# jjery2243542/adaptive_voice_conversion

Measured on AMD Instinct MI355X. Metric: mel-segments/sec (80x128) train step, higher is better.
Workload: dtype f32; 1 GPU; BASELINE configs[1]: recon+KL train step (fwd, loss, bwd, clip, Adam-amsgrad), 80-mel x 128-frame segments, batch 256/GPU, fp32; global_batch=256, parallelism=dp1, world_size=1

## Files before the change

### adaptive_voice_conversion_amd/_lib.py

```python
import ctypes
import os

_HERE = os.path.dirname(os.path.abspath(__file__))
LIB_PATH = os.path.join(_HERE, "csrc", "libavc_hip.so")
_lib = None

MAX_BLOCKS = 8
PLAN_INFERENCE, PLAN_SPEAKER_ONLY = 1, 2
GRADS_ALL, GRADS_DECODER, GRADS_ENCODERS, GRADS_SPEAKER, GRADS_CONTENT = 0, 1, 2, 3, 4


class EncoderCfg(ctypes.Structure):
    _fields_ = [(n, ctypes.c_int) for n in ("c_in", "c_h", "c_out", "kernel_size", "bank_size", "bank_scale", "c_bank",
                                            "n_conv_blocks", "n_dense_blocks")] + [("subsample", ctypes.c_int * MAX_BLOCKS), ("act", ctypes.c_int)]


class DecoderCfg(ctypes.Structure):
    _fields_ = [(n, ctypes.c_int) for n in ("c_in", "c_cond", "c_h", "c_out", "kernel_size", "n_conv_blocks")] + \
               [("upsample", ctypes.c_int * MAX_BLOCKS), ("act", ctypes.c_int)]


class ModelCfg(ctypes.Structure):
    _fields_ = [("spk", EncoderCfg), ("enc", EncoderCfg), ("dec", DecoderCfg)]

# ... 46 lines not shown
    lib.avc_tuning_init.argtypes = [ctypes.POINTER(Tuning)]
    lib.avc_tuning_init.restype = None
    lib.avc_get_op_tuning.argtypes = [ctypes.POINTER(Tuning)]
    lib.avc_get_op_tuning.restype = None
    lib.avc_plan_create_tuned.argtypes = [ctypes.POINTER(ModelCfg), c_int, c_int, c_int, c_int, ctypes.POINTER(Tuning), ctypes.POINTER(c_void_p)]
    lib.avc_plan_set_single_stream.argtypes = [c_void_p, c_int]
    lib.avc_plan_create_ragged.argtypes = [ctypes.POINTER(ModelCfg), c_int, ctypes.POINTER(c_int), ctypes.POINTER(c_int), ctypes.POINTER(Tuning),
                                           ctypes.POINTER(c_void_p)]
    lib.avc_plan_ragged_out.argtypes = [c_void_p, ctypes.POINTER(c_int), ctypes.POINTER(c_long)]
    lib.avc_forward_ragged.argtypes = [c_void_p, c_void_p, c_void_p, c_void_p, c_void_p, c_void_p]
    if hasattr(lib, "avc_plan_create_ragged_ex"):
        lib.avc_plan_create_ragged_ex.argtypes = [ctypes.POINTER(ModelCfg), c_int, ctypes.POINTER(c_int), ctypes.POINTER(c_int), c_int,
                                                  ctypes.POINTER(Tuning), ctypes.POINTER(c_void_p)]
        lib.avc_forward_ragged_emb.argtypes = [c_void_p, c_void_p, c_void_p, c_void_p, c_long, c_long, c_void_p, c_void_p]
    if hasattr(lib, "avc_plan_create_ragged_fanout"):
        lib.avc_plan_create_ragged_fanout.argtypes = [ctypes.POINTER(ModelCfg), c_int, ctypes.POINTER(c_int), c_int, ctypes.POINTER(c_int), c_int,
                                                      ctypes.POINTER(Tuning), ctypes.POINTER(c_void_p)]
        lib.avc_plan_ragged_latents.argtypes = [c_void_p, ctypes.POINTER(c_int), ctypes.POINTER(c_long)]
        lib.avc_decoder_forward_ragged.argtypes = [c_void_p, c_void_p, c_void_p, c_int, c_void_p, c_long, c_long, c_void_p, c_void_p]
    if hasattr(lib, "avc_backward_ragged"):
        lib.avc_backward_ragged.argtypes = [c_void_p, c_void_p, c_void_p, c_void_p, c_long, c_long, c_void_p, c_void_p]
    if hasattr(lib, "avc_plan_create_ragged_content_grads"):
        lib.avc_plan_create_ragged_content_grads.argtypes = [ctypes.POINTER(ModelCfg), c_int, ctypes.POINTER(c_int), ctypes.POINTER(Tuning),
                                                             ctypes.POINTER(c_void_p)]
        lib.avc_content_backward_ragged.argtypes = [c_void_p, c_void_p, c_void_p, c_void_p, c_void_p, c_void_p]
    lib.avc_gather_segments.argtypes = [c_void_p, c_long, c_int, c_void_p, c_int, c_int, c_void_p, c_void_p]
    lib.avc_plan_destroy.argtypes = [c_void_p]
    lib.avc_plan_destroy.restype = None
    lib.avc_plan_num_params.argtypes = [c_void_p]
    lib.avc_plan_param_floats.argtypes = [c_void_p]
    lib.avc_plan_param_floats.restype = c_long
    lib.avc_plan_param_info.argtypes = [c_void_p, c_int, ctypes.POINTER(c_long), ctypes.POINTER(c_long), ctypes.POINTER(c_int * 3)]
    lib.avc_plan_workspace_floats.argtypes = [c_void_p]
    lib.avc_plan_workspace_floats.restype = c_long
    lib.avc_plan_buffer.argtypes = [c_void_p, ctypes.c_char_p]
    lib.avc_plan_buffer.restype = c_long
    lib.avc_plan_num_relu_sites.argtypes = [c_void_p]
    lib.avc_plan_relu_site.argtypes = [c_void_p, c_int, ctypes.POINTER(ReluSite)]
    lib.avc_plan_set_compute_dtype.argtypes = [c_void_p, c_int]
    lib.avc_plan_compute_dtype.argtypes = [c_void_p]
    lib.avc_plan_out_len.argtypes = [c_void_p]
    lib.avc_plan_latent_len.argtypes = [c_void_p]
    lib.avc_forward.argtypes = [c_void_p, c_void_p, c_void_p, c_long, c_long, c_int, c_void_p, c_long, c_long, c_int,
                                c_void_p, c_void_p, c_void_p]
    lib.avc_forward_ex.argtypes = [c_void_p, c_void_p, c_void_p, c_long, c_long, c_int, c_void_p, c_long, c_long, c_int,
                                   c_void_p, c_void_p, c_int, c_void_p]
    lib.avc_plan_pack_weights.argtypes = [c_void_p, c_void_p, c_void_p, c_void_p]
    if hasattr(lib, "avc_decoder_forward"):
        lib.avc_decoder_forward.argtypes = [c_void_p, c_void_p, c_void_p, c_long, c_long, c_int, c_void_p, c_long, c_long, c_void_p, c_int, c_void_p]
        lib.avc_decoder_backward.argtypes = [c_void_p, c_void_p, c_void_p, c_long, c_long, c_int, c_void_p, c_long, c_long, c_void_p, c_void_p,
                                             c_void_p, c_void_p]
    lib.avc_loss.argtypes = [c_void_p, c_void_p, c_long, c_long, c_int, c_float, c_void_p, c_void_p]
    lib.avc_backward.argtypes = [c_void_p, c_void_p, c_void_p, c_long, c_long, c_int, c_void_p, c_long, c_long, c_int,
                                 c_void_p, c_void_p, c_void_p, c_void_p, c_float, c_void_p, c_void_p, c_void_p]
    lib.avc_clip_adam_ws_floats.argtypes = [c_long]
    lib.avc_clip_adam_ws_floats.restype = c_long
    lib.avc_clip_adam_step.argtypes = [c_void_p] * 5 + [c_long, c_int] + [c_float] * 5 + [c_int, c_float, c_float, c_int,
                                                                                        c_void_p, c_void_p, c_void_p]
    lib.avc_packed_weight_floats.argtypes = [c_int] * 4
    lib.avc_packed_weight_floats.restype = c_long
    lib.avc_packed_weight_floats_x3.argtypes = [c_int] * 4
    lib.avc_packed_weight_floats_x3.restype = c_long
    lib.avc_pack_weight_x3.argtypes = [c_void_p, c_int, c_int, c_int, c_int, c_void_p, c_void_p]
    lib.avc_pack_weight.argtypes = [c_void_p, c_int, c_int, c_int, c_int, c_int, c_int, c_void_p, c_void_p]
    lib.avc_conv1d_fwd.argtypes = [c_void_p, c_long, c_long, c_int, c_int, c_int, c_int, c_void_p, c_void_p, c_int, c_int,
                                   c_int, c_int, c_void_p, c_long, c_long, c_int, c_int, c_void_p, c_int, c_long, c_long,
                                   c_int, c_int, c_void_p, c_int, c_void_p]
    lib.avc_conv1d_dgrad.argtypes = [c_void_p, c_long, c_long, c_int, c_int, c_int, c_int, c_int, c_void_p, c_int, c_int,
                                     c_int, c_int, c_void_p, c_long, c_long, c_int, c_void_p, c_int, c_long, c_long, c_int,
                                     c_int, c_void_p, c_void_p, c_int, c_void_p]
    lib.avc_conv1d_wgrad_ws_floats.argtypes = [c_int] * 5
    lib.avc_conv1d_wgrad_ws_floats.restype = c_long
    lib.avc_conv1d_wgrad.argtypes = [c_void_p, c_long, c_long, c_int, c_void_p, c_long, c_long, c_int, c_int, c_int, c_int,
                                     c_int, c_int, c_int, c_int, c_int, c_void_p, c_void_p, c_void_p, c_void_p]
    lib.avc_instnorm_fwd.argtypes = [c_void_p, c_int, c_int, c_int, c_void_p, c_long, c_int, c_int, c_void_p, c_int, c_int,
                                     c_void_p, c_void_p, c_void_p, c_void_p]
    lib.avc_instnorm_bwd.argtypes = [c_void_p, c_void_p, c_void_p, c_void_p, c_int, c_int, c_int, c_void_p, c_long, c_int,
                                     c_int, c_void_p, c_void_p, c_long, c_int, c_void_p]
    lib.avc_conv1d_in_fwd.argtypes = [c_void_p, c_long, c_long, c_int, c_int, c_int, c_int, c_void_p, c_void_p, c_int, c_int, c_int, c_int,
                                      c_void_p, c_void_p, c_long, c_int, c_int, c_void_p, c_int, c_int, c_void_p, c_void_p, c_void_p, c_void_p, c_void_p]
    lib.avc_conv1d_dgrad_in_bwd.argtypes = [c_void_p, c_long, c_long, c_int, c_int, c_int, c_int, c_int, c_void_p, c_int, c_int, c_int, c_int,
                                            c_void_p, c_void_p, c_int, c_int, c_void_p, c_void_p, c_void_p, c_void_p, c_long, c_int, c_int,
                                            c_void_p, c_void_p, c_long, c_int, c_void_p, c_void_p]
    lib.avc_instnorm_fwd_pairs.argtypes = [c_void_p, c_int, c_int, c_int, c_void_p, c_long, c_int, c_int, c_void_p, c_int, c_int, c_int,
                                           c_void_p, c_void_p, c_void_p, c_void_p]
    lib.avc_instnorm_bwd_pairs.argtypes = [c_void_p, c_void_p, c_void_p, c_void_p, c_int, c_int, c_int, c_void_p, c_long, c_int, c_int, c_int,
                                           c_void_p, c_void_p, c_long, c_int, c_void_p]
    lib.avc_to_pairs.argtypes = [c_void_p, c_long, c_long, c_long, c_int, c_int, c_int, c_void_p, c_void_p]
    lib.avc_dsp_num_frames.argtypes = [c_long, c_int]
    lib.avc_dsp_basis_floats.argtypes = [c_int, c_int, c_int]
    lib.avc_dsp_basis_floats.restype = c_long
    lib.avc_dsp_basis_scratch_floats.argtypes = [c_int, c_int]
    lib.avc_dsp_basis_scratch_floats.restype = c_long
    lib.avc_dsp_make_basis.argtypes = [c_int, c_int, c_int, c_int, c_void_p, c_void_p, c_void_p]
    lib.avc_dsp_stft.argtypes = [c_void_p, c_long, c_int, c_int, c_int, c_void_p, c_void_p, c_void_p, c_void_p]
    lib.avc_dsp_istft.argtypes = [c_void_p, c_int, c_int, c_int, c_int, c_void_p, c_void_p, c_void_p, c_void_p]
    lib.avc_dsp_griffin_lim_ws_floats.argtypes = [c_int, c_int, c_int, c_int]
    lib.avc_dsp_griffin_lim_ws_floats.restype = c_long
    lib.avc_dsp_griffin_lim.argtypes = [c_void_p, c_int, c_int, c_int, c_int, c_int, c_void_p, c_void_p, c_void_p, c_void_p, c_void_p]
    lib.avc_dsp_stft_batch.argtypes = [c_void_p, c_long, c_int, c_int, c_int, c_int, c_void_p, c_void_p, c_void_p, c_void_p]
    lib.avc_dsp_istft_batch.argtypes = [c_void_p, c_int, c_int, c_int, c_int, c_int, c_void_p, c_void_p, c_void_p, c_void_p]
    lib.avc_dsp_griffin_lim_batch.argtypes = [c_void_p, c_int, c_int, c_int, c_int, c_int, c_int, c_void_p, c_void_p, c_void_p, c_void_p, c_void_p]
    lib.avc_dsp_griffin_lim_ragged.argtypes = [c_void_p, c_void_p, c_void_p, c_int, c_int, c_int, c_int, c_int, c_int, c_void_p, c_void_p, c_void_p, c_void_p, c_void_p]
    lib.avc_dsp_magnitude.argtypes = [c_void_p, c_int, c_int, c_void_p, c_void_p]
    lib.avc_dsp_db_normalize.argtypes = [c_void_p, c_int, c_int, c_float, c_float, c_void_p, c_void_p]
    lib.avc_dsp_denormalize_amp.argtypes = [c_void_p, c_int, c_int, c_float, c_float, c_void_p, c_void_p]
    lib.avc_dsp_preemphasis.argtypes = [c_void_p, c_long, c_float, c_void_p, c_void_p]
    lib.avc_dsp_deemphasis.argtypes = [c_void_p, c_long, c_float, c_void_p, c_void_p]
    lib.avc_dsp_frame_power.argtypes = [c_void_p, c_long, c_int, c_int, c_void_p, c_void_p]
    lib.avc_prof_end.argtypes = [c_void_p, c_void_p, c_void_p, c_void_p]
    lib.avc_prof_class_name.argtypes = [c_int]
    lib.avc_prof_class_name.restype = ctypes.c_char_p
    return lib


def load():
    global _lib, LIB_PATH
    if _lib is None:
        LIB_PATH = os.environ.get("AVC_HIP_LIB", LIB_PATH)
        if not os.path.exists(LIB_PATH):
            raise RuntimeError(
                f"{LIB_PATH} is missing: build the HIP extension first "
                "(python -c 'import __graft_entry__ as g; g.build()' or adaptive_voice_conversion_amd/csrc/build.sh)")
        import torch
        try:
            _lib = declare(ctypes.CDLL(LIB_PATH))
        except OSError as e:
            raise RuntimeError(f"cannot load {LIB_PATH}: {e}") from e
    return _lib
```

### adaptive_voice_conversion_amd/csrc/conv_gemm.hip

```cpp
#include <hip/hip_runtime.h>
#include <stdlib.h>

#include "avc_common.h"
#include "avc_internal.h"

#include "conv_shared.h"
#include "conv_x3_shared.h"

#ifndef AVC_CONV_STAGES
#define AVC_CONV_STAGES 2
#endif
#ifndef AVC_CONV_STAGES_BH
#define AVC_CONV_STAGES_BH 2
#endif

static __device__ __forceinline__ void conv_wait_dma(int n) {
#define AVC_WAIT_VM(k) __builtin_amdgcn_s_waitcnt(((k) & 15) | (((k) >> 4) << 14) | (7 << 4) | (15 << 8))
    switch (n) {
        case 0: AVC_WAIT_VM(0); break;
        case 1: AVC_WAIT_VM(1); break;
        case 2: AVC_WAIT_VM(2); break;
        case 3: AVC_WAIT_VM(3); break;
        case 4: AVC_WAIT_VM(4); break;
        case 5: AVC_WAIT_VM(5); break;
// ... 323 lines not shown
        load_a(kg + KG, 1);
        load_x(xtile, kg + KG, 1);
    }
    __syncthreads();

    const int a_lane4 = (wave_m * (32 * WM) + li) * 4;
    const int nit = (nchunk + KG - 1) / KG;
    int st = 0;
    for (int wk = 0; wk < walk_n; ++wk) {
    f32x16 acc[WM][WN];
#pragma unroll
    for (int wm = 0; wm < WM; ++wm)
#pragma unroll
        for (int wn = 0; wn < WN; ++wn)
#pragma unroll
            for (int r = 0; r < 16; ++r) acc[wm][wn][r] = 0.f;
    const bool walk_more = WALK && wk + 1 < walk_n;
    for (int it = 0; it < nit; ++it) {
        const int chunk = it * KG + kg;
        const bool more = (chunk + DIST * KG < nchunk) && !((a.dbg & 1) && (DIST == 2 || it >= 1));
        const bool last_of_tile = walk_more && it == nit - 1;
        int issued = 0;
        if (more) {
            const int stn = (st + DIST) % NS;
            load_a(chunk + DIST * KG, stn);
            load_x(xtile, chunk + DIST * KG, stn);
            if (DIST == 2) issued = dma_count(chunk + DIST * KG);
        } else if (last_of_tile && !(a.dbg & 1)) {
            const int stn = (st + 1) % NS;
            load_a(0, stn);
            load_x(xtile + walk_dx, 0, stn);
        }
        const float* Ab = As + st * AS;
        const float* Xb = Xs + st * XS;
        if ((a.dbg & 2) || chunk >= nchunk) {
        } else if constexpr (PAR) {
            if (wave_n == 0) {
                if (MIRROR && use_mirror && one_window) conv_chunk_mma<WM, WN, 1, KSC, GRC, BF, 1>(acc, Ab, Xb, KS, CK, ROW, h, a_lane4, cb4, cbl4, cbr4);
                else if (MIRROR && use_mirror) conv_chunk_mma<WM, WN, 2, KSC, GRC, BF, 1>(acc, Ab, Xb, KS, CK, ROW, h, a_lane4, cb4, cbl4, cbr4);
                else conv_chunk_mma<WM, WN, 0, KSC, GRC, BF, 1>(acc, Ab, Xb, KS, CK, ROW, h, a_lane4, cb4, cbl4, cbr4);
            } else {
                if (MIRROR && use_mirror && one_window) conv_chunk_mma<WM, WN, 1, KSC, GRC, BF, 2>(acc, Ab, Xb, KS, CK, ROW, h, a_lane4, cb4, cbl4, cbr4);
                else if (MIRROR && use_mirror) conv_chunk_mma<WM, WN, 2, KSC, GRC, BF, 2>(acc, Ab, Xb, KS, CK, ROW, h, a_lane4, cb4, cbl4, cbr4);
                else conv_chunk_mma<WM, WN, 0, KSC, GRC, BF, 2>(acc, Ab, Xb, KS, CK, ROW, h, a_lane4, cb4, cbl4, cbr4);
            }
        } else if (MIRROR && use_mirror && one_window)
            conv_chunk_mma<WM, WN, 1, KSC, GRC, BF>(acc, Ab, Xb, KS, CK, ROW, h, a_lane4, cb4, cbl4, cbr4);
        else if (MIRROR && use_mirror)
            conv_chunk_mma<WM, WN, 2, KSC, GRC, BF>(acc, Ab, Xb, KS, CK, ROW, h, a_lane4, cb4, cbl4, cbr4);
        else if constexpr (KSC < 0) {
            switch (KS * 8 + GR) {
                case 1 * 8 + 4: conv_chunk_mma<WM, WN, 0, 1, 4, BF>(acc, Ab, Xb, KS, CK, ROW, h, a_lane4, cb4, cbl4, cbr4); break;
                case 2 * 8 + 2: conv_chunk_mma<WM, WN, 0, 2, 2, BF>(acc, Ab, Xb, KS, CK, ROW, h, a_lane4, cb4, cbl4, cbr4); break;
                case 3 * 8 + 2: conv_chunk_mma<WM, WN, 0, 3, 2, BF>(acc, Ab, Xb, KS, CK, ROW, h, a_lane4, cb4, cbl4, cbr4); break;
                case 4 * 8 + 1: conv_chunk_mma<WM, WN, 0, 4, 1, BF>(acc, Ab, Xb, KS, CK, ROW, h, a_lane4, cb4, cbl4, cbr4); break;
                case 5 * 8 + 1: conv_chunk_mma<WM, WN, 0, 5, 1, BF>(acc, Ab, Xb, KS, CK, ROW, h, a_lane4, cb4, cbl4, cbr4); break;
                case 6 * 8 + 1: conv_chunk_mma<WM, WN, 0, 6, 1, BF>(acc, Ab, Xb, KS, CK, ROW, h, a_lane4, cb4, cbl4, cbr4); break;
                case 7 * 8 + 1: conv_chunk_mma<WM, WN, 0, 7, 1, BF>(acc, Ab, Xb, KS, CK, ROW, h, a_lane4, cb4, cbl4, cbr4); break;
                case 8 * 8 + 1: conv_chunk_mma<WM, WN, 0, 8, 1, BF>(acc, Ab, Xb, KS, CK, ROW, h, a_lane4, cb4, cbl4, cbr4); break;
                default: conv_chunk_mma<WM, WN, 0, 0, 0, BF>(acc, Ab, Xb, KS, CK, ROW, h, a_lane4, cb4, cbl4, cbr4);
            }
        } else
            conv_chunk_mma<WM, WN, 0, KSC, GRC, BF>(acc, Ab, Xb, KS, CK, ROW, h, a_lane4, cb4, cbl4, cbr4);
        if (last_of_tile) {
            conv_wait_dma(0);
        } else if (!(a.dbg & 4)) {
            conv_wait_dma(issued);
            conv_bare_barrier();
        }
        st = st == NS - 1 ? 0 : st + 1;
    }

    if (KG > 1) {
        float* red = smem + ((kg > 0 ? kg - 1 : 0) * 4 + wave) * (WM * WN * 16 * 64) + lane;
        if (kg > 0) {
#pragma unroll
            for (int wm = 0; wm < WM; ++wm)
#pragma unroll
                for (int wn = 0; wn < WN; ++wn)
#pragma unroll
                    for (int r = 0; r < 16; ++r) red[((wm * WN + wn) * 16 + r) * 64] = acc[wm][wn][r];
        }
        __syncthreads();
        if (kg > 0) return;
#pragma unroll
        for (int k2 = 1; k2 < KG; ++k2) {
            const float* rk = smem + ((k2 - 1) * 4 + wave) * (WM * WN * 16 * 64) + lane;
#pragma unroll
            for (int wm = 0; wm < WM; ++wm)
#pragma unroll
                for (int wn = 0; wn < WN; ++wn)
#pragma unroll
                    for (int r = 0; r < 16; ++r) acc[wm][wn][r] += rk[((wm * WN + wn) * 16 + r) * 64];
        }
    }

    if constexpr (INF) {
        static_assert(WM == 1 && WN == 1 && (BF == 0 || BF == 2) && !PAR && !RAG && !WALK && !MIRROR, "fused InstanceNorm epilogue: forward, 64 x 64 tiles, fp32 or bf16 pairs");
        if (KG > 1) __syncthreads();
        if constexpr (BF == 2) conv_epilogue_in_pairs(a, g, acc[0][0], smem, tid, wave_m, wave_n, li, h, m_tile0, q.b0);
        else conv_epilogue_in(a, g, acc[0][0], smem, tid, wave_m, wave_n, li, h, m_tile0, q.b0);
        return;
    }
    if constexpr (INB) {
        static_assert(WM == 1 && WN == 1 && (BF == 0 || BF == 2) && !RAG && !WALK && !INF, "fused InstanceNorm-backward epilogue: input gradient on 64 x 64 tiles, fp32 or bf16 pairs");
        if (KG > 1) __syncthreads();
        if constexpr (BF == 2) conv_epilogue_in_bwd_pairs(a, g, acc[0][0], smem, tid, wave_m, h, m_tile0, q.b0, q.t0, colb[0] - q.b0, colt[0], colv[0]);
        else conv_epilogue_in_bwd(a, g, acc[0][0], smem, tid, wave_m, h, m_tile0, q.b0, q.t0, colb[0] - q.b0, colt[0], colv[0]);
        return;
    }
    if (!(a.dbg & 8)) {
        if constexpr (WALK) {
            ConvEpi epi_t;
            ConvGroup g_t;
#ifdef AVC_EMU
            const ConvArgs* ka = &a;
#else
            const __attribute__((address_space(4))) ConvArgs* ka = (const __attribute__((address_space(4))) ConvArgs*)__builtin_amdgcn_kernarg_segment_ptr();
            asm volatile("" : "+s"(ka));
#endif
            epi_t.ob = ka->ob; epi_t.oc = ka->oc; epi_t.rb = ka->rb; epi_t.rc = ka->rc; epi_t.obase = 0; epi_t.rbase = 0;
            epi_t.ot = ka->ot; epi_t.ops = ka->ops; epi_t.rt = ka->rt; epi_t.Tres = ka->Tres; epi_t.Tout = ka->Tout; epi_t.M = ka->M;
            epi_t.act = ka->act; epi_t.res_mode = ka->res_mode; epi_t.res_to_primary = ka->res_to_primary; epi_t.slope = ka->slope;
            epi_t.pairs = ka->pairs;
            const int z = blockIdx.z;
            g_t.wp = nullptr; g_t.bias = ka->g[z].bias; g_t.out = ka->g[z].out; g_t.out2 = ka->g[z].out2; g_t.res = ka->g[z].res;
            g_t.mask = ka->g[z].mask; g_t.KS = 0; g_t.padL = 0; g_t.padR = 0; g_t.nchunk = 0; g_t.CK = 0; g_t.out_c0 = 0;
#pragma unroll
            for (int wn = 0; wn < WN; ++wn) {
                if (!colv[wn]) continue;
#pragma unroll
                for (int wm = 0; wm < WM; ++wm) {
                    int tcol = colt[wn], bcol = b0_cur + colb[wn], mb = m_tile0 + wave_m * (32 * WM) + wm * 32;
#ifndef AVC_EMU
                    asm volatile("" : "+v"(tcol), "+v"(bcol));
                    asm volatile("" : "+s"(mb));
#endif
                    if (BF == 2 && epi_t.pairs) conv_store_frag_pairs(epi_t, g_t, acc[wm][wn], mb, h, bcol, tcol);
                    else conv_store_frag(epi_t, g_t, acc[wm][wn], mb, h, bcol, tcol);
                }
            }
        } else {
#pragma unroll
            for (int wn = 0; wn < WN; ++wn) {
                if (!colv[wn]) continue;
#pragma unroll
                for (int wm = 0; wm < WM; ++wm) {
                    if (BF == 2 && epi.pairs) conv_store_frag_pairs(epi, g, acc[wm][wn], m_tile0 + wave_m * (32 * WM) + wm * 32, h, colb[wn], colt[wn]);
                    else conv_store_frag(epi, g, acc[wm][wn], m_tile0 + wave_m * (32 * WM) + wm * 32, h, colb[wn], colt[wn]);
                }
            }
        }
    }
    if (walk_more) {
        conv_bare_barrier();
        xtile += walk_dx;
        b0_cur += a.walk_db;
    }
    }
}


struct PackBatch {
    PackArgs a[AVC_PACK_BATCH];
};

static __device__ __forceinline__ void pack_one(const PackArgs& p, long first, long stride, long limit = (1L << 62));

__global__ void __launch_bounds__(AVC_THREADS) pack_weight_batch_kernel(const PackBatch b) {
    pack_one(b.a[blockIdx.y], (long)blockIdx.x * AVC_THREADS + threadIdx.x, (long)gridDim.x * AVC_THREADS);
}

static __device__ __forceinline__ void pack_staged(const PackArgs* __restrict__ gp, const float* __restrict__ params, float* __restrict__ ws, int piece, float* stage) {
    const int tid = threadIdx.x;
    const int MB = gp->mb, Mp = gp->Mp, M = gp->M, KS = gp->KS, CK = gp->CK, Cin = gp->Cin, Cout = gp->Cout, img = gp->img;
    const int nsrc = gp->nsrc, rows_per_src = gp->rows_per_src;
    const bool dgrad = gp->dgrad != 0;
    float* dst = (float*)((char*)ws + (size_t)gp->dst);
    const char* pbase = (const char*)params;
    const int nmb = (Mp + MB - 1) / MB;
    const int chunk = piece / nmb, m0 = (piece - chunk * nmb) * MB;
    const bool pairs = img == AVC_IMG_K4H;
    const int CKr = pairs ? 2 * CK : CK, c0 = chunk * CKr;
    const int seglen = dgrad ? MB * KS : CKr * KS, nseg = dgrad ? CKr : MB;
    const int pitch = seglen | 1;
    const int n = nseg * seglen;
    const float inv_seglen = 1.0f / (float)seglen, inv_rows = 1.0f / (float)rows_per_src;
    const int row0 = dgrad ? c0 : m0, col0 = dgrad ? m0 : c0;
    const int row_end = dgrad ? Cout : M, off_end = ((dgrad ? M : Cin) - col0) * KS;
    constexpr int U = 16;
    for (int e0 = tid; e0 < n; e0 += U * AVC_THREADS) {
// ... 210 lines not shown
    return ck;
}

static size_t conv_lds_bytes(const ConvArgs& a, int BM, int BN) {
    size_t worst = 0;
    for (int gi = 0; gi < a.ngroups; ++gi) {
        ConvGeom q = conv_geom(a.mode, a.stride, a.Tout, a.g[gi].KS, BN, 0);
        size_t AS = (size_t)a.g[gi].KS * a.g[gi].CK * BM, XS = (size_t)a.g[gi].CK * q.ROW;
        size_t bytes = (size_t)(a.bf16 == AVC_COMPUTE_BF16S ? AVC_CONV_STAGES_BH : AVC_CONV_STAGES) * (AS + XS) * 4;
        worst = bytes > worst ? bytes : worst;
    }
    return worst + 16;
}

static int conv_ntiles_n(const ConvArgs& a, int BN) {
    if (a.Tout >= BN) return a.B * avc_cdiv(a.Tout, BN);
    int worst = 1;
    for (int gi = 0; gi < a.ngroups; ++gi) {
        const int n = avc_cdiv(a.B, conv_geom(a.mode, a.stride, a.Tout, a.g[gi].KS, BN, 0).SPT);
        worst = n > worst ? n : worst;
    }
    return worst;
}

template <int WM, int BF>
static void conv_launch_rag(const ConvArgs& a, int fast, dim3 grid, dim3 block, size_t lds, hipStream_t stream) {
    if (fast == 1) hipLaunchKernelGGL((conv_gemm_kernel<WM, 1, false, 5, 1, 1, BF, false, true>), grid, block, lds, stream, a);
    else if (fast == -1) hipLaunchKernelGGL((conv_gemm_kernel<WM, 1, false, -1, 0, 1, BF, false, true>), grid, block, lds, stream, a);
    else if (fast == 14) hipLaunchKernelGGL((conv_gemm_kernel<WM, 1, false, 1, 4, 1, BF, false, true>), grid, block, lds, stream, a);
    else hipLaunchKernelGGL((conv_gemm_kernel<WM, 1, false, 0, 0, 1, BF, false, true>), grid, block, lds, stream, a);
}

static void conv_launch_rag_dgrad(const ConvArgs& a, int fast, dim3 grid, dim3 block, size_t lds, hipStream_t stream) {
    if (a.par && fast == 1) hipLaunchKernelGGL((conv_gemm_kernel<1, 1, true, 5, 1, 1, 0, true, true>), grid, block, lds, stream, a);
    else if (fast == 1) hipLaunchKernelGGL((conv_gemm_kernel<1, 1, true, 5, 1, 1, 0, false, true>), grid, block, lds, stream, a);
    else hipLaunchKernelGGL((conv_gemm_kernel<1, 1, true, 0, 0, 1, 0, false, true>), grid, block, lds, stream, a);
}

template <int WM, int KG, int BF>
static void conv_launch_variant(const ConvArgs& a, bool mir, int fast, dim3 grid, dim3 block, size_t lds, hipStream_t stream) {
    if (mir && fast == 1) hipLaunchKernelGGL((conv_gemm_kernel<WM, 1, true, 5, 1, KG, BF>), grid, block, lds, stream, a);
    else if (mir && fast == 2) hipLaunchKernelGGL((conv_gemm_kernel<WM, 1, true, 5, 2, KG, BF>), grid, block, lds, stream, a);
    else if (mir) hipLaunchKernelGGL((conv_gemm_kernel<WM, 1, true, 0, 0, KG, BF>), grid, block, lds, stream, a);
    else if (fast == 1) hipLaunchKernelGGL((conv_gemm_kernel<WM, 1, false, 5, 1, KG, BF>), grid, block, lds, stream, a);
    else if (fast == 2) hipLaunchKernelGGL((conv_gemm_kernel<WM, 1, false, 5, 2, KG, BF>), grid, block, lds, stream, a);
    else if (fast == 4 && KG == 1) hipLaunchKernelGGL((conv_gemm_kernel<WM, 1, false, 5, 4, 1, BF>), grid, block, lds, stream, a);
    else if (fast == -1 && KG == 1) hipLaunchKernelGGL((conv_gemm_kernel<WM, 1, false, -1, 0, 1, BF>), grid, block, lds, stream, a);
    else if (fast == 14) hipLaunchKernelGGL((conv_gemm_kernel<WM, 1, false, 1, 4, KG, BF>), grid, block, lds, stream, a);
    else hipLaunchKernelGGL((conv_gemm_kernel<WM, 1, false, 0, 0, KG, BF>), grid, block, lds, stream, a);
}

static bool conv_launch_walk(const ConvArgs& a, int tile, bool mir, int fast, dim3 grid, dim3 block, size_t lds, hipStream_t stream) {
    if (tile == 11 && fast == 1 && mir) hipLaunchKernelGGL((conv_gemm_kernel<1, 1, true, 5, 1, 1, 0, false, false, true>), grid, block, lds, stream, a);
    else if (tile == 11 && fast == 1) hipLaunchKernelGGL((conv_gemm_kernel<1, 1, false, 5, 1, 1, 0, false, false, true>), grid, block, lds, stream, a);
    else if (tile == 11 && fast == -1 && !mir) hipLaunchKernelGGL((conv_gemm_kernel<1, 1, false, -1, 0, 1, 0, false, false, true>), grid, block, lds, stream, a);
    else if (tile == 11 && fast == 14 && !mir) hipLaunchKernelGGL((conv_gemm_kernel<1, 1, false, 1, 4, 1, 0, false, false, true>), grid, block, lds, stream, a);
    else if (tile == 21 && fast == 14 && !mir) hipLaunchKernelGGL((conv_gemm_kernel<2, 1, false, 1, 4, 1, 0, false, false, true>), grid, block, lds, stream, a);
    else return false;
    return true;
}
template <int KG, int BF>
static void conv_launch_inf(const ConvArgs& a, int fast, dim3 grid, dim3 block, size_t lds, hipStream_t stream) {
    if (fast == 1) hipLaunchKernelGGL((conv_gemm_kernel<1, 1, false, 5, 1, KG, BF, false, false, false, true>), grid, block, lds, stream, a);
    else if (fast == 2) hipLaunchKernelGGL((conv_gemm_kernel<1, 1, false, 5, 2, KG, BF, false, false, false, true>), grid, block, lds, stream, a);
    else if (fast == 14) hipLaunchKernelGGL((conv_gemm_kernel<1, 1, false, 1, 4, KG, BF, false, false, false, true>), grid, block, lds, stream, a);
    else hipLaunchKernelGGL((conv_gemm_kernel<1, 1, false, 0, 0, KG, BF, false, false, false, true>), grid, block, lds, stream, a);
}
template <int KG, int BF>
static void conv_launch_inb(const ConvArgs& a, bool mir, int fast, dim3 grid, dim3 block, size_t lds, hipStream_t stream) {
    if (a.par && mir && fast == 1) hipLaunchKernelGGL((conv_gemm_kernel<1, 1, true, 5, 1, KG, BF, true, false, false, false, true>), grid, block, lds, stream, a);
    else if (a.par && mir) hipLaunchKernelGGL((conv_gemm_kernel<1, 1, true, 5, 2, KG, BF, true, false, false, false, true>), grid, block, lds, stream, a);
    else if (a.par && fast == 1) hipLaunchKernelGGL((conv_gemm_kernel<1, 1, false, 5, 1, KG, BF, true, false, false, false, true>), grid, block, lds, stream, a);
    else if (a.par) hipLaunchKernelGGL((conv_gemm_kernel<1, 1, false, 5, 2, KG, BF, true, false, false, false, true>), grid, block, lds, stream, a);
    else if (mir && fast == 1) hipLaunchKernelGGL((conv_gemm_kernel<1, 1, true, 5, 1, KG, BF, false, false, false, false, true>), grid, block, lds, stream, a);
    else if (mir && fast == 2) hipLaunchKernelGGL((conv_gemm_kernel<1, 1, true, 5, 2, KG, BF, false, false, false, false, true>), grid, block, lds, stream, a);
    else if (mir) hipLaunchKernelGGL((conv_gemm_kernel<1, 1, true, 0, 0, KG, BF, false, false, false, false, true>), grid, block, lds, stream, a);
    else if (fast == 14) hipLaunchKernelGGL((conv_gemm_kernel<1, 1, false, 1, 4, KG, BF, false, false, false, false, true>), grid, block, lds, stream, a);
    else hipLaunchKernelGGL((conv_gemm_kernel<1, 1, false, 0, 0, KG, BF, false, false, false, false, true>), grid, block, lds, stream, a);
}
static bool conv_walk_instance(int tile, bool mir, int fast) {
    return (tile == 11 && (fast == 1 || ((fast == -1 || fast == 14) && !mir))) || (tile == 21 && fast == 14 && !mir);
}

template <int BF>
static void conv_launch_wide(const ConvArgs& a, bool mir, dim3 grid, dim3 block, size_t lds, hipStream_t stream) {
    if (mir) hipLaunchKernelGGL((conv_gemm_kernel<1, 2, true, 5, 1, 1, BF>), grid, block, lds, stream, a);
    else hipLaunchKernelGGL((conv_gemm_kernel<1, 2, false, 5, 1, 1, BF>), grid, block, lds, stream, a);
}

template <int KG, int BF>
static void conv_launch_par(const ConvArgs& a, bool mir, int fast, dim3 grid, dim3 block, size_t lds, hipStream_t stream) {
    if (mir && fast == 1) hipLaunchKernelGGL((conv_gemm_kernel<1, 1, true, 5, 1, KG, BF, true>), grid, block, lds, stream, a);
    else if (mir) hipLaunchKernelGGL((conv_gemm_kernel<1, 1, true, 5, 2, KG, BF, true>), grid, block, lds, stream, a);
    else if (fast == 1) hipLaunchKernelGGL((conv_gemm_kernel<1, 1, false, 5, 1, KG, BF, true>), grid, block, lds, stream, a);
    else hipLaunchKernelGGL((conv_gemm_kernel<1, 1, false, 5, 2, KG, BF, true>), grid, block, lds, stream, a);
}

bool avc_conv_in_fusable(const ConvArgs& a, const avc_tuning& tun, int res_mode, int Tres) {
    const int Tn_ = a.Tout * a.ops;
    if (res_mode != AVC_RES_NONE && !((res_mode == AVC_RES_IDENTITY && Tres == Tn_) || (res_mode == AVC_RES_UP2 && 2 * Tres == Tn_) ||
                                      (res_mode == AVC_RES_AVGPOOL2 && Tres == 2 * Tn_))) return false;
    if (!tun.conv_in_fuse || a.mode != 0 || a.ngroups != 1 || a.rag.tile) return false;
    const bool bh = a.bf16 == AVC_COMPUTE_BF16S;
    if (bh ? (a.img != AVC_IMG_K4H || !a.pairs || a.ops != 1 || (a.M & 1) || a.x.ps != 1 || a.x.st != 1) : (a.bf16 != AVC_COMPUTE_F32 || a.img != AVC_IMG_K4 || a.pairs)) return false;
    if (a.Tout != 16 && a.Tout != 32 && a.Tout != 64) return false;
    if (a.ops != 1 && a.ops != 2) return false;
    if (a.ops == 2 && (a.M & 1)) return false;
    if (a.act || a.res_mode != AVC_RES_NONE || a.g[0].out2 || a.g[0].mask) return false;
    const int C = (bh ? a.M / 2 : a.M) / a.ops, Tn = a.Tout * a.ops;
    if (a.ot != 1 || a.oc != Tn || a.ob != (long)C * Tn) return false;
    if (conv_geom(0, a.stride, a.Tout, a.g[0].KS, 64, 0).SPT != 64 / a.Tout) return false;
    return avc_conv_pick_tile(tun, a.Mp, a.B, a.Tout, 1, a.Cred * a.g[0].KS * (bh ? 2 : 1)) == 11;
}

bool avc_conv_inb_fusable(const ConvArgs& a, const avc_tuning& tun) {
    if (!tun.conv_in_fuse || a.mode != 1 || a.ngroups != 1 || a.rag.tile) return false;
    const bool bh = a.bf16 == AVC_COMPUTE_BF16S;
    if (bh ? (a.img != AVC_IMG_K4H || !a.pairs || (a.M & 1) || a.x.ps != 1 || a.x.st != 1) : (a.bf16 != AVC_COMPUTE_F32 || a.img != AVC_IMG_K4 || a.pairs)) return false;
    if (a.Tout != 16 && a.Tout != 32 && a.Tout != 64) return false;
    if (a.ops != 1 || a.act || a.g[0].out2 || a.g[0].mask || a.g[0].bias) return false;
    const long Mr = bh ? a.M / 2 : a.M;
    if (a.ot != 1 || a.oc != a.Tout || a.ob != Mr * a.Tout) return false;
    if (a.res_mode != AVC_RES_NONE) {
        if (!a.res_to_primary || a.rt != 1 || a.rc != a.Tres || a.rb != Mr * a.Tres) return false;
        if (!((a.res_mode == AVC_RES_IDENTITY && a.Tres == a.Tout) || (a.res_mode == AVC_RES_POOLT && 2 * a.Tres == a.Tout) ||
              (a.res_mode == AVC_RES_UPT && a.Tres == 2 * a.Tout))) return false;
    }
    if (conv_geom(1, a.stride, a.Tout, a.g[0].KS, 64, 0).SPT != 64 / a.Tout) return false;
    return avc_conv_pick_tile(tun, a.Mp, a.B, a.Tout, 1, a.Cred * a.g[0].KS * (bh ? 2 : 1)) == 11;
}

int avc_launch_conv(const ConvArgs& a_in, hipStream_t stream, int force_tile, const avc_tuning& tun) {
    if (a_in.img == AVC_IMG_X3 || force_tile == 97) return avc_launch_conv_x3(a_in, stream, tun);
    ConvArgs a = a_in;
    a.dbg = tun.conv_ablation;
    if (a.ngroups < 1 || a.ngroups > AVC_MAX_GROUPS) return -1;
    if (a.Mp % 128 != 0) return -2;
    if (a.x.ps != 1 && a.x.ps != 2) return -2;
    for (int gi = 0; gi < a.ngroups; ++gi)
        if (a.mode == 0 && (a.g[gi].padL >= a.Tsrc || a.g[gi].padR >= a.Tsrc)) return -6;
    int tile = force_tile == 22 ? 21 : force_tile;
    if (tile == 98) return -8;
    const bool wide_ok = a.ngroups == 1 && a.g[0].KS == 5 && a.g[0].CK == 8 && a.stride == 1 && a.Tout >= 64 && !a.rag.tile && a.x.ps == 1;
    if (tile == 0) {
        tile = avc_conv_pick_tile(tun, a.Mp, a.B, a.Tout, a.ngroups, a.Cred * a.g[0].KS * (a.bf16 == AVC_COMPUTE_BF16S ? 2 : 1));
        if (tile == 11 && wide_ok && tun.tile12_wgs > 0 && !a.in.out && !a.inb.dy) {
            const long ntn = a.Tout >= 128 ? (long)a.B * avc_cdiv(a.Tout, 128) : (long)avc_cdiv(a.B, 128 / a.Tout);
            if ((long)(a.Mp / 64) * ntn >= tun.tile12_wgs) tile = 12;
        }
    }
    if (a.in.out) {
        if (!avc_conv_in_fusable(a, tun, a.in.res ? a.in.res_mode : AVC_RES_NONE, a.in.Tres) || (force_tile != 0 && force_tile != 11) || tile != 11) return -2;
        if (!a.in.mean || !a.in.rstd || a.in.C != a.M / a.ops) return -2;
    }
    if (a.inb.dy) {
        if (a.in.out || !avc_conv_inb_fusable(a, tun) || (force_tile != 0 && force_tile != 11) || tile != 11) return -2;
        if (!a.inb.y || !a.inb.mean || !a.inb.rstd || a.inb.C != a.M) return -2;
    }
    if (tile == 12 && !wide_ok) return -2;
    if (tile != 11 && tile != 21 && tile != 12) return -2;
    const int BM = (tile == 21) ? 128 : 64, BN = (tile == 12) ? 128 : 64;
    for (int gi = 0; gi < a.ngroups; ++gi) {
        ConvGeom q = conv_geom(a.mode, a.stride, a.Tout, a.g[gi].KS, BN, 0);
        if (a.g[gi].CK % 8 != 0) return -2;
        if (q.ROW > 16 * AVC_CONV_NJ4) return -3;
    }
    size_t lds = conv_lds_bytes(a, BM, BN);
    const bool rag = a.rag.tile != nullptr;
    if (rag && (a.Tout < BN || a.rag.ntiles < 1)) return -2;
    if (rag && a.mode == 1 && (a.bf16 != AVC_COMPUTE_F32 || tile == 12 || a.ngroups != 1)) return -2;
    dim3 grid(rag ? a.rag.ntiles : conv_ntiles_n(a, BN), a.Mp / BM, a.ngroups);
    int kgroups = 1;
    if (!rag && a.bf16 != AVC_COMPUTE_BF16S && tile == 11 && a.ngroups == 1 && (long)grid.x * grid.y <= tun.kg_wgs && a.g[0].nchunk >= 4 && 2 * lds <= 160 * 1024 && !a.dbg) kgroups = 2;
    lds *= kgroups;
    if ((a.in.out || a.inb.dy) && lds < AVC_IN_LDS_BYTES) lds = AVC_IN_LDS_BYTES;
    if (lds > 160 * 1024) return -5;
    if (tun.conv_min_lds > 0 && (size_t)tun.conv_min_lds > lds && tun.conv_min_lds <= 160 * 1024) lds = (size_t)tun.conv_min_lds;
    dim3 block(AVC_THREADS * kgroups);
    double flops = 0;
    for (int gi = 0; gi < a.ngroups; ++gi)
        flops += 2.0 * a.M * a.Cred * (a.bf16 == AVC_COMPUTE_BF16S ? 2 : 1) * a.g[gi].KS * (double)a.B * (a.mode == 0 ? a.Tout : a.Tsrc);
    ProfScope ps(a.mode == 0 ? AVC_K_CONV_FWD : AVC_K_CONV_DGRAD, flops, 0.0, stream);
    const bool mir = a.mode == 1 && a.mirror;
    const int fast = (a.ngroups == 1 && a.g[0].KS == 5) ? (a.g[0].CK == 8 ? 1 : (a.g[0].CK == 16 ? 2 : (a.g[0].CK == 32 ? 4 : 0)))
                     : ((a.ngroups > 1 && a.mode == 0 && tun.bank_switch) ? -1
                        : ((a.ngroups == 1 && a.g[0].KS == 1 && a.g[0].CK == 32 && tun.bank_switch) ? 14 : 0));
    const int bf = a.bf16 == AVC_COMPUTE_BF16 ? 1 : (a.bf16 == AVC_COMPUTE_BF16S ? 2 : 0);
    if (bf == 2 && (a.img != AVC_IMG_K4H || a.x.ps != 1 || a.x.st != 1)) return -2;
    if (a.pairs && (bf != 2 || a.ops != 1 || a.ot != 1 || (a.M & 1) || (a.res_mode != AVC_RES_NONE && a.rt != 1))) return -2;
    a.par = tun.dgrad_par && a.mode == 1 && a.stride == 2 && tile == 11 && a.ngroups == 1 && (fast == 1 || fast == 2) && !a.dbg &&
            a.g[0].padL == 2 && (a.Tout >= 64 || (a.Tout % 2 == 0 && 64 % a.Tout == 0)) && !(rag && fast != 1);
    a.walk_n = 1;
    a.walk_rem = (int)grid.x;
    a.walk_db = 0;
    bool walk = false;
    if (tun.conv_walk != 0 && !a.in.out && !a.inb.dy && !rag && !a.par && bf == 0 && kgroups == 1 && AVC_CONV_STAGES == 2 && conv_walk_instance(tile, mir, fast)) {
        const int ntn = (int)grid.x;
        const int tps = a.Tout >= BN ? avc_cdiv(a.Tout, BN) : 1;
        const int SPT = a.Tout >= BN ? 1 : conv_geom(a.mode, a.stride, a.Tout, a.g[0].KS, BN, 0).SPT;
        const bool geom_ok = a.Tout >= BN || (a.ngroups == 1 && a.B % SPT == 0);
        long per_cu = (long)(160 * 1024) / (long)lds;
        const long reg_cu = BM == 128 ? 3 : 4;
        per_cu = per_cu < reg_cu ? per_cu : reg_cu;
        per_cu = per_cu < tun.conv_walk ? per_cu : tun.conv_walk;
        long W = 256 * per_cu / ((long)grid.y * grid.z);
        const bool forced = tun.conv_walk < 0;
        if (forced) W = -tun.conv_walk < tps ? tps : -tun.conv_walk;
        W = W / tps * tps;
        if (geom_ok && W >= tps && W < ntn && (forced || (long)ntn >= (tun.conv_walk_min > 1 ? tun.conv_walk_min : 2) * W)) {
            a.walk_n = avc_cdiv(ntn, (int)W);
            a.walk_rem = ntn - (a.walk_n - 1) * (int)W;
            a.walk_db = a.Tout >= BN ? (int)W / tps : (int)W * SPT;
            grid.x = (unsigned)W;
            walk = true;
        }
    }
#define AVC_BF3(CALL_)                       \
    do {                                     \
        if (bf == 2) { CALL_(2); }           \
        else if (bf == 1) { CALL_(1); }      \
        else { CALL_(0); }                   \
    } while (0)
    if (a.inb.dy) {
        if (bf == 2) conv_launch_inb<1, 2>(a, mir, fast, grid, block, lds, stream);
        else if (kgroups == 2) conv_launch_inb<2, 0>(a, mir, fast, grid, block, lds, stream);
        else conv_launch_inb<1, 0>(a, mir, fast, grid, block, lds, stream);
    } else if (a.in.out) {
        const int f = (fast == 1 || fast == 2 || fast == 14) ? fast : 0;
        if (bf == 2) conv_launch_inf<1, 2>(a, f, grid, block, lds, stream);
        else if (kgroups == 2) conv_launch_inf<2, 0>(a, f, grid, block, lds, stream);
        else conv_launch_inf<1, 0>(a, f, grid, block, lds, stream);
    } else if (walk) {
        if (!conv_launch_walk(a, tile, mir, fast, grid, block, lds, stream)) return -2;
    } else if (rag) {
        if (bf == 2) return -2;
        if (mir) {
            if (tile != 11) return -2;
            conv_launch_rag_dgrad(a, fast, grid, block, lds, stream);
            return (int)hipGetLastError();
        }
        const int f = (fast == 1 || fast == -1 || fast == 14) ? fast : 0;
#define AVC_C_RAG2(BF_) conv_launch_rag<2, BF_>(a, f, grid, block, lds, stream)
#define AVC_C_RAG1(BF_) conv_launch_rag<1, BF_>(a, f, grid, block, lds, stream)
        if (tile == 21) { if (bf) AVC_C_RAG2(1); else AVC_C_RAG2(0); }
        else { if (bf) AVC_C_RAG1(1); else AVC_C_RAG1(0); }
    } else if (a.par) {
#define AVC_C_PAR2(BF_) conv_launch_par<2, BF_>(a, mir, fast, grid, block, lds, stream)
#define AVC_C_PAR1(BF_) conv_launch_par<1, BF_>(a, mir, fast, grid, block, lds, stream)
        if (kgroups == 2) AVC_BF3(AVC_C_PAR2);
        else AVC_BF3(AVC_C_PAR1);
    } else if (tile == 12) {
#define AVC_C_WIDE(BF_) conv_launch_wide<BF_>(a, mir, grid, block, lds, stream)
        AVC_BF3(AVC_C_WIDE);
    } else if (tile == 21) {
#define AVC_C_V21(BF_) conv_launch_variant<2, 1, BF_>(a, mir, fast, grid, block, lds, stream)
        AVC_BF3(AVC_C_V21);
    } else if (kgroups == 2) {
#define AVC_C_V12(BF_) conv_launch_variant<1, 2, BF_>(a, mir, fast, grid, block, lds, stream)
        AVC_BF3(AVC_C_V12);
    } else {
#define AVC_C_V11(BF_) conv_launch_variant<1, 1, BF_>(a, mir, fast, grid, block, lds, stream)
        AVC_BF3(AVC_C_V11);
    }
#undef AVC_BF3
    return (int)hipGetLastError();
}

long avc_pack_total(const PackArgs& p) {
    if (p.img == AVC_IMG_X3) return (long)p.nchunk * x3_arows(p.KS) * p.Mp * 4;
    return (long)p.nchunk * p.KS * p.CK * p.Mp;
}

int avc_launch_pack_batch(const PackArgs* ps, int n, hipStream_t stream) {
    for (int i = 0; i < n; i += AVC_PACK_BATCH) {
        PackBatch b;
        int m = n - i < AVC_PACK_BATCH ? n - i : AVC_PACK_BATCH;
        long maxtotal = 1, bytes = 0;
        for (int k = 0; k < m; ++k) {
            b.a[k] = ps[i + k];
            long t = avc_pack_total(ps[i + k]);
            maxtotal = t > maxtotal ? t : maxtotal;
            bytes += 8 * t;
        }
        int blocks = (int)((maxtotal + AVC_THREADS * 4 - 1) / (AVC_THREADS * 4));
        if (blocks > 256) blocks = 256;
        ProfScope ps_(AVC_K_PACK, 0.0, (double)bytes, stream);
        hipLaunchKernelGGL(pack_weight_batch_kernel, dim3(blocks, m), dim3(AVC_THREADS), 0, stream, b);
    }
    return (int)hipGetLastError();
}

int avc_launch_pack_table(const PackArgs* dev_tab, const void* dev_blk, int nblk, double bytes, const float* params, float* ws, hipStream_t stream) {
    ProfScope ps_(AVC_K_PACK, 0.0, bytes, stream);
    hipLaunchKernelGGL(pack_weight_table_kernel, dim3(nblk), dim3(AVC_THREADS), 0, stream, dev_tab, (const int2*)dev_blk, params, ws);
    return (int)hipGetLastError();
}

int avc_launch_pack(const PackArgs& p, hipStream_t stream) {
    long total = avc_pack_total(p);
    int blocks = (int)((total + AVC_THREADS * 4 - 1) / (AVC_THREADS * 4));
    if (blocks < 1) blocks = 1;
    if (blocks > 4096) blocks = 4096;
    ProfScope ps(AVC_K_PACK, 0.0, 8.0 * total, stream);
    hipLaunchKernelGGL(pack_weight_kernel, dim3(blocks), dim3(AVC_THREADS), 0, stream, p);
    return (int)hipGetLastError();
}
// ... 1 lines not shown
```

### adaptive_voice_conversion_amd/csrc/conv_shared.h

```cpp
#pragma once
#include "avc_common.h"
#include "bf16_pairs.h"

#define AVC_CONV_NJ 6
#define AVC_CONV_NJ4 10
#define AVC_CONV_MAXROW4 (16 * AVC_CONV_NJ4)

struct ConvGeom {
    int b0, t0, SPT, ncols, SEG, seg_p0, ROWDATA, ROW;
};

static inline __host__ __device__ ConvGeom conv_geom(int mode, int stride, int Tout, int KS, int BN, int tile) {
    ConvGeom q;
    if (Tout >= BN) {
        int tps = avc_cdiv(Tout, BN);
        q.b0 = tile / tps;
        q.t0 = (tile % tps) * BN;
        q.SPT = 1;
        q.ncols = BN;
    } else {
        q.SPT = BN / Tout;
        if (BN == 64) {
            const int seg = (mode == 0) ? (Tout - 1) * stride + KS : Tout + 3 * (KS - 1);
            const int fit = (AVC_CONV_MAXROW4 - KS) / seg;
// ... 61 lines not shown
        case AVC_RES_POOLT: i0 = (long)(t >> 1) * a.rt; break;
        case AVC_RES_UPT: i0 = (long)(2 * t) * a.rt; i1 = (long)(2 * t + 1) * a.rt; break;
        default: i0 = 0;
    }
}
static inline __device__ float conv_load_res(const ConvEpi& a, const float* res, int b, int m, int t) {
    const float* base = res + a.rbase + (long)b * a.rb + (long)m * a.rc;
    long i0, i1;
    conv_res_index(a, t, i0, i1);
    return conv_res_value(a, base[i0], i1 >= 0 ? base[i1] : 0.f, t);
}


static __device__ __forceinline__ void conv_store_frag(const ConvEpi& a, const ConvGroup& g, const f32x16& acc, int m_base, int h,
                                                       int b, int t) {
    const bool has_res = a.res_mode != AVC_RES_NONE;
    const bool has_mask = g.out2 && g.mask;
    const bool res_two = a.res_mode == AVC_RES_AVGPOOL2 || a.res_mode == AVC_RES_UPT;
    long ri0 = 0, ri1 = -1;
    if (has_res) conv_res_index(a, t, ri0, ri1);
#pragma unroll
    for (int half = 0; half < 2; ++half) {
        float bs[8], q0[8], q1[8], mk[8];
        long o[8];
#pragma unroll
        for (int e = 0; e < 8; ++e) {
            const int r = 8 * half + e;
            const int m = m_base + (r & 3) + 8 * (r >> 2) + 4 * h;
            const int mc = m < a.M ? m : a.M - 1;
            if (a.ops == 1)
                o[e] = a.obase + (long)b * a.ob + (long)mc * a.oc + (long)t * a.ot;
            else
                o[e] = a.obase + (long)b * a.ob + (long)(mc / a.ops) * a.oc + (long)(t * a.ops + (mc % a.ops)) * a.ot;
            bs[e] = q0[e] = q1[e] = mk[e] = 0.f;
        }
        if (g.bias) {
#pragma unroll
            for (int e = 0; e < 8; ++e) {
                const int r = 8 * half + e;
                const int m = m_base + (r & 3) + 8 * (r >> 2) + 4 * h;
                bs[e] = g.bias[m < a.M ? m : a.M - 1];
            }
        }
        if (has_res) {
#pragma unroll
            for (int e = 0; e < 8; ++e) {
                const int r = 8 * half + e;
                const int m = m_base + (r & 3) + 8 * (r >> 2) + 4 * h;
                const float* base = g.res + a.rbase + (long)b * a.rb + (long)(m < a.M ? m : a.M - 1) * a.rc;
                q0[e] = base[ri0];
                if (res_two) q1[e] = base[ri1];
            }
        }
        if (has_mask) {
#pragma unroll
            for (int e = 0; e < 8; ++e) mk[e] = g.mask[o[e]];
        }
        float v[8], v2[8];
#pragma unroll
        for (int e = 0; e < 8; ++e) {
            float x = g.bias ? acc[8 * half + e] + bs[e] : acc[8 * half + e];
            if (a.act == 1) x = avc_act(x, a.slope);
            const float rr = has_res ? conv_res_value(a, q0[e], q1[e], t) : 0.f;
            if (a.res_to_primary) x += rr;
            float y = a.res_to_primary ? x : x + rr;
            if (has_mask) y = avc_act_grad(y, mk[e] > 0.f, a.slope);
            v[e] = x;
            v2[e] = y;
        }
#pragma unroll
        for (int e = 0; e < 8; ++e) {
            const int r = 8 * half + e;
            const int m = m_base + (r & 3) + 8 * (r >> 2) + 4 * h;
            if (m < a.M) {
                if (g.out) g.out[o[e]] = v[e];
                if (g.out2) g.out2[o[e]] = v2[e];
            }
        }
    }
}

#define AVC_IN_LDT 68
#define AVC_IN_LDS_BYTES (64 * AVC_IN_LDT * 4)
static __device__ __forceinline__ float4 conv_in_res4(const float* rrow, int mode, int t, int Tres) {
    float4 r = make_float4(0.f, 0.f, 0.f, 0.f);
    if (mode == AVC_RES_IDENTITY) {
        r = *(const float4*)(rrow + t);
    } else if (mode == AVC_RES_UP2) {
        float2 ab = *(const float2*)(rrow + (t >> 1));
        r = make_float4(ab.x, ab.x, ab.y, ab.y);
    } else if (mode == AVC_RES_AVGPOOL2) {
        float4 p = *(const float4*)(rrow + 2 * t), q = *(const float4*)(rrow + 2 * t + 4);
        r = make_float4((p.x + p.y) * 0.5f, (p.z + p.w) * 0.5f, (q.x + q.y) * 0.5f, (q.z + q.w) * 0.5f);
    }
    return r;
}
static __device__ void conv_epilogue_in(const ConvArgs& a, const ConvGroup& g, const f32x16& acc, float* tile, int tid, int wave_m, int wave_n,
                                        int li, int h, int m_tile0, int b0) {
    const ConvINFuse& f = a.in;
    const int col = wave_n * 32 + li;
#pragma unroll
    for (int r = 0; r < 16; ++r) {
        const int row = wave_m * 32 + (r & 3) + 8 * (r >> 2) + 4 * h;
        const int m = m_tile0 + row;
        const float bs = g.bias ? g.bias[m < a.M ? m : a.M - 1] : 0.f;
        tile[row * AVC_IN_LDT + col] = acc[r] + bs;
    }
    __syncthreads();
    const int r = tid >> 2, qd = tid & 3;
    const int m = m_tile0 + r;
    const int Tout = a.Tout, lpr = Tout >> 4;
    const int bl = (16 * qd) / Tout, t0 = 16 * qd - bl * Tout;
    const int b = b0 + bl;
    const bool valid = m < a.M && b < a.B;
    float v[16];
#pragma unroll
    for (int k = 0; k < 4; ++k) {
        const float4 x = *(const float4*)(tile + r * AVC_IN_LDT + 16 * qd + 4 * k);
        v[4 * k] = x.x; v[4 * k + 1] = x.y; v[4 * k + 2] = x.z; v[4 * k + 3] = x.w;
    }
    const int ops = a.ops;
    const int c = ops == 2 ? m >> 1 : m, j = ops == 2 ? (m & 1) : 0;
    const int Tn = Tout * ops;
    const float invT = 1.0f / (float)Tn;
    float s = 0.f;
#pragma unroll
    for (int k = 0; k < 4; ++k) s += (v[4 * k] + v[4 * k + 1]) + (v[4 * k + 2] + v[4 * k + 3]);
    for (int o = 1; o < lpr; o <<= 1) s += __shfl_xor(s, o);
    if (ops == 2) s += __shfl_xor(s, 4);
    const float mean = s * invT;
    float ss = 0.f;
#pragma unroll
    for (int k = 0; k < 4; ++k) {
        const float dx = v[4 * k] - mean, dy = v[4 * k + 1] - mean, dz = v[4 * k + 2] - mean, dw = v[4 * k + 3] - mean;
        ss += (dx * dx + dy * dy) + (dz * dz + dw * dw);
    }
    for (int o = 1; o < lpr; o <<= 1) ss += __shfl_xor(ss, o);
    if (ops == 2) ss += __shfl_xor(ss, 4);
    const float rstd = 1.0f / sqrtf(ss * invT + AVC_IN_EPS);
    int fbase = t0;
    if (ops == 2) {
        float w[16];
#pragma unroll
        for (int i = 0; i < 8; ++i) {
            const float rcv = __shfl_xor(j ? v[i] : v[8 + i], 4);
            w[2 * i] = j ? rcv : v[i];
            w[2 * i + 1] = j ? v[8 + i] : rcv;
        }
#pragma unroll
        for (int i = 0; i < 16; ++i) v[i] = w[i];
        fbase = 2 * t0 + 16 * j;
    }
    if (!valid) return;
    const long rowi = (long)b * f.C + c;
    if (qd % lpr == 0 && j == 0) {
        f.mean[rowi] = mean;
        f.rstd[rowi] = rstd;
    }
    float gamma = 1.f, beta = 0.f;
    if (f.cond) {
        const float* cr = f.cond + (long)b * f.cond_sb + f.cond_off;
        beta = cr[c];
        gamma = cr[f.C + c];
    }
    float4 rv[4];
    const float* rrow = f.res ? f.res + rowi * f.Tres : nullptr;
#pragma unroll
    for (int k = 0; k < 4; ++k) rv[k] = rrow ? conv_in_res4(rrow, f.res_mode, fbase + 4 * k, f.Tres) : make_float4(0.f, 0.f, 0.f, 0.f);
    float* yrow = g.out + rowi * Tn + fbase;
    float* orow = f.out + rowi * Tn + fbase;
#pragma unroll
    for (int k = 0; k < 4; ++k) *(float4*)(yrow + 4 * k) = make_float4(v[4 * k], v[4 * k + 1], v[4 * k + 2], v[4 * k + 3]);
#pragma unroll
    for (int k = 0; k < 4; ++k) {
        float o[4];
#pragma unroll
        for (int e = 0; e < 4; ++e) {
            const float w = in_preact(in_xhat(v[4 * k + e], mean, rstd), gamma, beta);
            o[e] = f.relu ? avc_act(w, a.slope) : w;
        }
        *(float4*)(orow + 4 * k) = make_float4(o[0] + rv[k].x, o[1] + rv[k].y, o[2] + rv[k].z, o[3] + rv[k].w);
    }
}

static __device__ void conv_epilogue_in_bwd(const ConvArgs& a, const ConvGroup& g, const f32x16& acc, float* tile, int tid, int wave_m, int h,
                                            int m_tile0, int b0, int t0_tile, int bl_lane, int t_lane, bool col_valid) {
    const ConvINBwd& f = a.inb;
    const int Tout = a.Tout, lpr = Tout >> 4;
    if (col_valid) {
        const int col = bl_lane * Tout + (t_lane - t0_tile);
#pragma unroll
        for (int r = 0; r < 16; ++r) {
            const int row = wave_m * 32 + (r & 3) + 8 * (r >> 2) + 4 * h;
            tile[row * AVC_IN_LDT + col] = acc[r];
        }
    }
    __syncthreads();
    const int r = tid >> 2, qd = tid & 3;
    const int m = m_tile0 + r;
    const int bl = (16 * qd) / Tout, t0 = 16 * qd - bl * Tout;
    const int b = b0 + bl;
    const bool valid = m < a.M && b < a.B;
    const int mc = m < a.M ? m : a.M - 1, bc = b < a.B ? b : a.B - 1;
    float gv[16];
#pragma unroll
    for (int k = 0; k < 4; ++k) {
        const float4 x = *(const float4*)(tile + r * AVC_IN_LDT + 16 * qd + 4 * k);
        gv[4 * k] = x.x; gv[4 * k + 1] = x.y; gv[4 * k + 2] = x.z; gv[4 * k + 3] = x.w;
    }
    const long rowi = (long)bc * f.C + mc;
    float yv[16];
    const float* yrow = f.y + rowi * Tout + t0;
#pragma unroll
    for (int k = 0; k < 4; ++k) {
        const float4 x = *(const float4*)(yrow + 4 * k);
        yv[4 * k] = x.x; yv[4 * k + 1] = x.y; yv[4 * k + 2] = x.z; yv[4 * k + 3] = x.w;
    }
    const float mean = f.mean[rowi], rstd = f.rstd[rowi];
    float gamma = 1.f, beta = 0.f;
    if (f.cond) {
        const float* cr = f.cond + (long)bc * f.cond_sb + f.cond_off;
        beta = cr[mc];
        gamma = cr[f.C + mc];
    }
    if (a.res_mode != AVC_RES_NONE) {
        const float* rrow = g.res + ((long)bc * a.M + mc) * a.Tres;
        if (a.res_mode == AVC_RES_IDENTITY) {
#pragma unroll
            for (int k = 0; k < 4; ++k) {
                const float4 x = *(const float4*)(rrow + t0 + 4 * k);
                gv[4 * k] += x.x; gv[4 * k + 1] += x.y; gv[4 * k + 2] += x.z; gv[4 * k + 3] += x.w;
            }
        } else if (a.res_mode == AVC_RES_POOLT) {
#pragma unroll
            for (int k = 0; k < 2; ++k) {
                const float4 x = *(const float4*)(rrow + (t0 >> 1) + 4 * k);
                gv[8 * k] += x.x * 0.5f; gv[8 * k + 1] += x.x * 0.5f; gv[8 * k + 2] += x.y * 0.5f; gv[8 * k + 3] += x.y * 0.5f;
                gv[8 * k + 4] += x.z * 0.5f; gv[8 * k + 5] += x.z * 0.5f; gv[8 * k + 6] += x.w * 0.5f; gv[8 * k + 7] += x.w * 0.5f;
            }
        } else {
#pragma unroll
            for (int k = 0; k < 8; ++k) {
                const float4 x = *(const float4*)(rrow + 2 * t0 + 4 * k);
                gv[2 * k] += x.x + x.y;
                gv[2 * k + 1] += x.z + x.w;
            }
        }
    }
    if (valid && g.out) {
        float* grow = g.out + ((long)b * a.M + m) * Tout + t0;
#pragma unroll
        for (int k = 0; k < 4; ++k) *(float4*)(grow + 4 * k) = make_float4(gv[4 * k], gv[4 * k + 1], gv[4 * k + 2], gv[4 * k + 3]);
    }
    float xh[16], s1 = 0.f, s2 = 0.f;
#pragma unroll
    for (int i = 0; i < 16; ++i) {
        const float hh = in_xhat(yv[i], mean, rstd);
        const float w = in_preact(hh, gamma, beta);
        const float gme = avc_act_grad(gv[i], !f.relu || w > 0.f, a.slope);
        xh[i] = hh;
        gv[i] = gme;
        s1 += gme;
        s2 += gme * hh;
    }
    for (int o = 1; o < lpr; o <<= 1) {
        s1 += __shfl_xor(s1, o);
        s2 += __shfl_xor(s2, o);
    }
    if (!valid) return;
    if (f.dcond && qd % lpr == 0) {
        float* dc = f.dcond + (long)b * f.dcond_sb + f.dcond_off;
        dc[m] = s1;
        dc[f.C + m] = s2;
    }
    const float invT = 1.0f / (float)Tout;
    const float m1 = gamma * s1 * invT, m2 = gamma * s2 * invT;
    float* drow = f.dy + rowi * Tout + t0;
#pragma unroll
    for (int k = 0; k < 4; ++k) {
        float4 o;
        o.x = rstd * (gv[4 * k] * gamma - m1 - xh[4 * k] * m2);
        o.y = rstd * (gv[4 * k + 1] * gamma - m1 - xh[4 * k + 1] * m2);
        o.z = rstd * (gv[4 * k + 2] * gamma - m1 - xh[4 * k + 2] * m2);
        o.w = rstd * (gv[4 * k + 3] * gamma - m1 - xh[4 * k + 3] * m2);
        *(float4*)(drow + 4 * k) = o;
    }
}

typedef unsigned conv_u32x4 __attribute__((ext_vector_type(4)));
typedef unsigned conv_u32x2 __attribute__((ext_vector_type(2)));
static __device__ __forceinline__ void conv_in_res_pairs4(const unsigned* rrow, int mode, int t, float (&lo)[4], float (&hi)[4]) {
    if (mode == AVC_RES_IDENTITY) {
        const conv_u32x4 v = *(const conv_u32x4*)(rrow + t);
#pragma unroll
        for (int k = 0; k < 4; ++k) { lo[k] = bh_lo(v[k]); hi[k] = bh_hi(v[k]); }
    } else if (mode == AVC_RES_UP2) {
        const conv_u32x2 v = *(const conv_u32x2*)(rrow + (t >> 1));
        lo[0] = lo[1] = bh_lo(v[0]); hi[0] = hi[1] = bh_hi(v[0]);
        lo[2] = lo[3] = bh_lo(v[1]); hi[2] = hi[3] = bh_hi(v[1]);
    } else if (mode == AVC_RES_AVGPOOL2) {
        const conv_u32x4 p = *(const conv_u32x4*)(rrow + 2 * t), q = *(const conv_u32x4*)(rrow + 2 * t + 4);
        lo[0] = (bh_lo(p[0]) + bh_lo(p[1])) * 0.5f; hi[0] = (bh_hi(p[0]) + bh_hi(p[1])) * 0.5f;
        lo[1] = (bh_lo(p[2]) + bh_lo(p[3])) * 0.5f; hi[1] = (bh_hi(p[2]) + bh_hi(p[3])) * 0.5f;
        lo[2] = (bh_lo(q[0]) + bh_lo(q[1])) * 0.5f; hi[2] = (bh_hi(q[0]) + bh_hi(q[1])) * 0.5f;
        lo[3] = (bh_lo(q[2]) + bh_lo(q[3])) * 0.5f; hi[3] = (bh_hi(q[2]) + bh_hi(q[3])) * 0.5f;
    } else {
#pragma unroll
        for (int k = 0; k < 4; ++k) lo[k] = hi[k] = 0.f;
    }
}
static __device__ void conv_epilogue_in_pairs(const ConvArgs& a, const ConvGroup& g, const f32x16& acc, float* tile, int tid, int wave_m, int wave_n,
                                              int li, int h, int m_tile0, int b0) {
    const ConvINFuse& f = a.in;
    const int col = wave_n * 32 + li;
#pragma unroll
    for (int r = 0; r < 16; ++r) {
        const int row = wave_m * 32 + (r & 3) + 8 * (r >> 2) + 4 * h;
        const int m = m_tile0 + row;
        const float bs = g.bias ? g.bias[m < a.M ? m : a.M - 1] : 0.f;
        tile[row * AVC_IN_LDT + col] = acc[r] + bs;
    }
    __syncthreads();
    const int r = tid >> 2, qd = tid & 3;
    const int m = m_tile0 + r, odd = m & 1;
    const int Tout = a.Tout, lpr = Tout >> 4;
    const int bl = (16 * qd) / Tout, t0 = 16 * qd - bl * Tout;
    const int b = b0 + bl;
    const bool valid = m < a.M && b < a.B;
    float v[16];
#pragma unroll
    for (int k = 0; k < 4; ++k) {
        const float4 x = *(const float4*)(tile + r * AVC_IN_LDT + 16 * qd + 4 * k);
        v[4 * k] = bh_lo(bh_pack(x.x, 0.f)); v[4 * k + 1] = bh_lo(bh_pack(x.y, 0.f));
        v[4 * k + 2] = bh_lo(bh_pack(x.z, 0.f)); v[4 * k + 3] = bh_lo(bh_pack(x.w, 0.f));
    }
    const float invT = 1.0f / (float)Tout;
    float s = 0.f;
#pragma unroll
    for (int k = 0; k < 4; ++k) s += (v[4 * k] + v[4 * k + 1]) + (v[4 * k + 2] + v[4 * k + 3]);
    for (int o = 1; o < lpr; o <<= 1) s += __shfl_xor(s, o);
    const float mean = s * invT;
    float ss = 0.f;
#pragma unroll
    for (int i = 0; i < 16; ++i) {
        const float d = v[i] - mean;
        ss += d * d;
    }
    for (int o = 1; o < lpr; o <<= 1) ss += __shfl_xor(ss, o);
    const float rstd = 1.0f / sqrtf(ss * invT + AVC_IN_EPS);
    const int mc = m < a.M ? m : a.M - 1;
    float gamma = 1.f, beta = 0.f;
    if (f.cond) {
        const float* cr = f.cond + (long)(b < a.B ? b : a.B - 1) * f.cond_sb + f.cond_off;
        beta = cr[mc];
        gamma = cr[f.C + mc];
    }
    if (valid && qd % lpr == 0) {
        f.mean[(long)b * f.C + m] = mean;
        f.rstd[(long)b * f.C + m] = rstd;
    }
    float lo[8], hi[8];
#pragma unroll
    for (int i = 0; i < 8; ++i) {
        const float rcv = __shfl_xor(odd ? v[i] : v[8 + i], 4);
        lo[i] = odd ? rcv : v[i];
        hi[i] = odd ? v[8 + i] : rcv;
    }
    const float pmean = __shfl_xor(mean, 4), prstd = __shfl_xor(rstd, 4), pgamma = __shfl_xor(gamma, 4), pbeta = __shfl_xor(beta, 4);
    const float mean0 = odd ? pmean : mean, mean1 = odd ? mean : pmean, rstd0 = odd ? prstd : rstd, rstd1 = odd ? rstd : prstd;
    const float g0 = odd ? pgamma : gamma, g1 = odd ? gamma : pgamma, be0 = odd ? pbeta : beta, be1 = odd ? beta : pbeta;
    if (!valid) return;
    const int fb = t0 + 8 * odd;
    const long prow = (long)b * (f.C >> 1) + (m >> 1);
    unsigned* yrow = (unsigned*)g.out + prow * Tout + fb;
    unsigned* orow = (unsigned*)f.out + prow * Tout + fb;
    const unsigned* rrow = f.res ? (const unsigned*)f.res + prow * f.Tres : nullptr;
#pragma unroll
    for (int k = 0; k < 2; ++k) {
        float rl[4], rh[4];
        if (rrow) conv_in_res_pairs4(rrow, f.res_mode, fb + 4 * k, rl, rh);
        else { rl[0] = rl[1] = rl[2] = rl[3] = rh[0] = rh[1] = rh[2] = rh[3] = 0.f; }
        conv_u32x4 yv, ov;
#pragma unroll
        for (int e = 0; e < 4; ++e) {
            const float y0 = lo[4 * k + e], y1 = hi[4 * k + e];
            yv[e] = bh_pack(y0, y1);
            const float w0 = in_preact(in_xhat(y0, mean0, rstd0), g0, be0), w1 = in_preact(in_xhat(y1, mean1, rstd1), g1, be1);
            ov[e] = bh_pack((f.relu ? avc_act(w0, a.slope) : w0) + rl[e], (f.relu ? avc_act(w1, a.slope) : w1) + rh[e]);
        }
        *(conv_u32x4*)(yrow + 4 * k) = yv;
        *(conv_u32x4*)(orow + 4 * k) = ov;
    }
}

static __device__ void conv_epilogue_in_bwd_pairs(const ConvArgs& a, const ConvGroup& g, const f32x16& acc, float* tile, int tid, int wave_m, int h,
                                                  int m_tile0, int b0, int t0_tile, int bl_lane, int t_lane, bool col_valid) {
    const ConvINBwd& f = a.inb;
    const int Tout = a.Tout, lpr = Tout >> 4;
    if (col_valid) {
        const int col = bl_lane * Tout + (t_lane - t0_tile);
#pragma unroll
        for (int r = 0; r < 16; ++r) {
            const int row = wave_m * 32 + (r & 3) + 8 * (r >> 2) + 4 * h;
            tile[row * AVC_IN_LDT + col] = acc[r];
        }
    }
    __syncthreads();
    const int r = tid >> 2, qd = tid & 3;
    const int m = m_tile0 + r, odd = m & 1;
    const int bl = (16 * qd) / Tout, t0 = 16 * qd - bl * Tout;
    const int b = b0 + bl;
    const bool valid = m < a.M && b < a.B;
    const int mc = m < a.M ? m : a.M - 1, bc = b < a.B ? b : a.B - 1;
    float gv[16];
#pragma unroll
    for (int k = 0; k < 4; ++k) {
        const float4 x = *(const float4*)(tile + r * AVC_IN_LDT + 16 * qd + 4 * k);
        gv[4 * k] = x.x; gv[4 * k + 1] = x.y; gv[4 * k + 2] = x.z; gv[4 * k + 3] = x.w;
    }
    const int C2 = f.C >> 1;
    const long prow = (long)bc * C2 + (mc >> 1);
    const long rowi = (long)bc * f.C + mc;
    float yv[16];
    const unsigned* yrow = (const unsigned*)f.y + prow * Tout + t0;
#pragma unroll
    for (int k = 0; k < 4; ++k) {
        const conv_u32x4 v = *(const conv_u32x4*)(yrow + 4 * k);
#pragma unroll
        for (int e = 0; e < 4; ++e) yv[4 * k + e] = odd ? bh_hi(v[e]) : bh_lo(v[e]);
    }
    const float mean = f.mean[rowi], rstd = f.rstd[rowi];
    float gamma = 1.f, beta = 0.f;
    if (f.cond) {
        const float* cr = f.cond + (long)bc * f.cond_sb + f.cond_off;
        beta = cr[mc];
        gamma = cr[f.C + mc];
    }
    if (a.res_mode != AVC_RES_NONE) {
        const unsigned* rrow = (const unsigned*)g.res + ((long)bc * (a.M >> 1) + (mc >> 1)) * a.Tres;
        if (a.res_mode == AVC_RES_IDENTITY) {
#pragma unroll
            for (int k = 0; k < 4; ++k) {
                const conv_u32x4 v = *(const conv_u32x4*)(rrow + t0 + 4 * k);
#pragma unroll
                for (int e = 0; e < 4; ++e) gv[4 * k + e] += odd ? bh_hi(v[e]) : bh_lo(v[e]);
            }
        } else if (a.res_mode == AVC_RES_POOLT) {
#pragma unroll
            for (int k = 0; k < 2; ++k) {
                const conv_u32x4 v = *(const conv_u32x4*)(rrow + (t0 >> 1) + 4 * k);
#pragma unroll
                for (int e = 0; e < 4; ++e) {
                    const float x = (odd ? bh_hi(v[e]) : bh_lo(v[e])) * 0.5f;
                    gv[8 * k + 2 * e] += x;
                    gv[8 * k + 2 * e + 1] += x;
                }
            }
        } else {
#pragma unroll
            for (int k = 0; k < 8; ++k) {
                const conv_u32x4 v = *(const conv_u32x4*)(rrow + 2 * t0 + 4 * k);
                gv[2 * k] += odd ? bh_hi(v[0]) + bh_hi(v[1]) : bh_lo(v[0]) + bh_lo(v[1]);
                gv[2 * k + 1] += odd ? bh_hi(v[2]) + bh_hi(v[3]) : bh_lo(v[2]) + bh_lo(v[3]);
            }
        }
    }
#pragma unroll
    for (int i = 0; i < 16; ++i) gv[i] = bh_lo(bh_pack(gv[i], 0.f));
    auto store_pairs = [&](unsigned* base, const float (&v)[16]) {
        float lo[8], hi[8];
#pragma unroll
        for (int i = 0; i < 8; ++i) {
            const float rcv = __shfl_xor(odd ? v[i] : v[8 + i], 4);
            lo[i] = odd ? rcv : v[i];
            hi[i] = odd ? v[8 + i] : rcv;
        }
        if (!valid) return;
        unsigned* drow = base + prow * Tout + t0 + 8 * odd;
#pragma unroll
        for (int k = 0; k < 2; ++k) {
            conv_u32x4 w;
#pragma unroll
            for (int e = 0; e < 4; ++e) w[e] = bh_pack(lo[4 * k + e], hi[4 * k + e]);
            *(conv_u32x4*)(drow + 4 * k) = w;
        }
    };
    if (g.out) store_pairs((unsigned*)g.out, gv);
    float xh[16], s1 = 0.f, s2 = 0.f;
#pragma unroll
    for (int i = 0; i < 16; ++i) {
        const float hh = in_xhat(yv[i], mean, rstd);
        const float w = in_preact(hh, gamma, beta);
        const float gme = avc_act_grad(gv[i], !f.relu || w > 0.f, a.slope);
        xh[i] = hh;
        gv[i] = gme;
        s1 += gme;
        s2 += gme * hh;
    }
    for (int o = 1; o < lpr; o <<= 1) {
        s1 += __shfl_xor(s1, o);
        s2 += __shfl_xor(s2, o);
    }
    if (valid && f.dcond && qd % lpr == 0) {
        float* dc = f.dcond + (long)b * f.dcond_sb + f.dcond_off;
        dc[m] = s1;
        dc[f.C + m] = s2;
    }
    const float invT = 1.0f / (float)Tout;
    const float m1 = gamma * s1 * invT, m2 = gamma * s2 * invT;
    float dv[16];
#pragma unroll
    for (int i = 0; i < 16; ++i) dv[i] = rstd * (gv[i] * gamma - m1 - xh[i] * m2);
    store_pairs((unsigned*)f.dy, dv);
}

static __device__ __forceinline__ void conv_res_index_pair(const ConvEpi& a, int t, int& i0, int& i1) {
    i1 = -1;
    switch (a.res_mode) {
        case AVC_RES_IDENTITY: i0 = t; break;
        case AVC_RES_AVGPOOL2: i0 = 2 * t; i1 = (2 * t + 1 < a.Tres) ? 2 * t + 1 : 2 * t; break;
        case AVC_RES_POOLT: i0 = t >> 1; break;
        case AVC_RES_UPT: i0 = 2 * t; i1 = 2 * t + 1; break;
        default: i0 = 0;
    }
}
static inline __device__ void conv_load_res_pair(const ConvEpi& a, const float* res, int b, int m, int t, float& r0, float& r1) {
    const unsigned* base = (const unsigned*)res + a.rbase + (long)b * a.rb + (long)(m >> 1) * a.rc;
    int i0, i1;
    conv_res_index_pair(a, t, i0, i1);
    const unsigned d0 = base[i0], d1 = i1 >= 0 ? base[i1] : 0u;
    r0 = conv_res_value(a, bh_lo(d0), bh_lo(d1), t);
    r1 = conv_res_value(a, bh_hi(d0), bh_hi(d1), t);
}

static __device__ __forceinline__ void conv_store_frag_pairs(const ConvEpi& a, const ConvGroup& g, const f32x16& acc, int m_base, int h,
                                                             int b, int t) {
    unsigned* out = (unsigned*)g.out;
    unsigned* out2 = (unsigned*)g.out2;
    const unsigned* mask = (const unsigned*)g.mask;
    const bool has_res = a.res_mode != AVC_RES_NONE;
    const bool has_mask = out2 && mask;
    const bool res_two = a.res_mode == AVC_RES_AVGPOOL2 || a.res_mode == AVC_RES_UPT;
    int ri0 = 0, ri1 = -1;
    if (has_res) conv_res_index_pair(a, t, ri0, ri1);
#pragma unroll
    for (int half = 0; half < 2; ++half) {
        float b0[4], b1[4];
        unsigned d0[4], d1[4], md[4];
        long o[4];
#pragma unroll
        for (int e = 0; e < 4; ++e) {
            const int r = 2 * (4 * half + e);
            const int m = m_base + (r & 3) + 8 * (r >> 2) + 4 * h;
            const int mc = m < a.M ? m : a.M - 2;
            o[e] = a.obase + (long)b * a.ob + (long)(mc >> 1) * a.oc + t;
            b0[e] = b1[e] = 0.f;
            d0[e] = d1[e] = md[e] = 0u;
        }
        if (g.bias) {
#pragma unroll
            for (int e = 0; e < 4; ++e) {
                const int r = 2 * (4 * half + e);
                const int m = m_base + (r & 3) + 8 * (r >> 2) + 4 * h;
                const int mc = m < a.M ? m : a.M - 2;
                b0[e] = g.bias[mc];
                b1[e] = g.bias[mc + 1];
            }
        }
        if (has_res) {
#pragma unroll
            for (int e = 0; e < 4; ++e) {
                const int r = 2 * (4 * half + e);
                const int m = m_base + (r & 3) + 8 * (r >> 2) + 4 * h;
                const int mc = m < a.M ? m : a.M - 2;
                const unsigned* base = (const unsigned*)g.res + a.rbase + (long)b * a.rb + (long)(mc >> 1) * a.rc;
                d0[e] = base[ri0];
                if (res_two) d1[e] = base[ri1];
            }
        }
        if (has_mask) {
#pragma unroll
            for (int e = 0; e < 4; ++e) md[e] = mask[o[e]];
        }
        unsigned w[4], w2[4];
#pragma unroll
        for (int e = 0; e < 4; ++e) {
            const int r = 2 * (4 * half + e);
            float v0 = acc[r], v1 = acc[r + 1];
            if (g.bias) { v0 += b0[e]; v1 += b1[e]; }
            if (a.act == 1) { v0 = avc_act(v0, a.slope); v1 = avc_act(v1, a.slope); }
            float r0 = 0.f, r1 = 0.f;
            if (has_res) {
                r0 = conv_res_value(a, bh_lo(d0[e]), bh_lo(d1[e]), t);
                r1 = conv_res_value(a, bh_hi(d0[e]), bh_hi(d1[e]), t);
            }
            if (a.res_to_primary) { v0 += r0; v1 += r1; }
// ... 20 lines not shown
```

### adaptive_voice_conversion_amd/csrc/engine.hip

```cpp
#include <hip/hip_runtime.h>
#include <math.h>
#include <stdio.h>
#include <stdlib.h>

#include <algorithm>
#include <map>
#include <string>
#include <vector>

#include "avc_common.h"
#include "avc_hip.h"
#include "avc_internal.h"

static thread_local std::string g_err;
static int fail(int rc, const char* what) {
    char buf[256];
    snprintf(buf, sizeof(buf), "%s (rc=%d)", what, rc);
    g_err = buf;
    return rc;
}
#define RUN(expr)                                  \
    do {                                           \
        int _rc = (expr);                          \
        if (_rc != 0) return fail(_rc, #expr);     \
// ... 935 lines not shown
    return avc_launch_wgrad_batch(L.data(), n, ls, c.p->tun.wgrad_ablation);
}

static int wgrad_layer(BwdCtx& c, const LayerP& L, const float* x, long xsb, long xsc, int xst, const float* dy, long ysb,
                       long ysc, int yst, int yps, int Bn, int Tin, int Tout) {
    BwdCtx::PendW pw;
    WgradArgs& a = pw.a;
    memset(&a, 0, sizeof(a));
    a.x.ptr = x; a.x.sb = xsb; a.x.sc = xsc; a.x.st = xst; a.x.ps = 1;
    a.dy.ptr = dy; a.dy.sb = ysb; a.dy.sc = ysc; a.dy.st = yst; a.dy.ps = yps;
    a.B = Bn; a.Cin = L.Cin; a.Cout = L.Cout; a.Tin = Tin; a.Tout = Tout;
    a.KS = L.KS; a.padL = L.KS / 2; a.stride = L.stride;
    a.bf16 = (L.bf16 == AVC_COMPUTE_F32 && c.p->tun.wgrad_x3) ? AVC_COMPUTE_F32X3 : L.bf16;
    a.cw8 = c.p->tun.wgrad_cw8 ? 1 : 0;
    pw.L = &L;
    avc_wgrad_geometry(a);
    c.pend_units += (long)a.tiles * a.total_chunks;
    c.pend.push_back(pw);
    if (!c.hold && ((int)c.pend.size() >= c.p->tun.wgrad_batch || c.pend_units >= c.p->tun.wgrad_batch_units)) return flush_wgrads(c);
    return 0;
}

static void pack_layer(const avc_plan* p, const LayerP& L, const float* params, float* ws, std::vector<PackArgs>& out) {
    PackArgs a;
    memset(&a, 0, sizeof(a));
    for (int i = 0; i < L.nsrc; ++i) a.src[i] = p->par(params, L.w[i]);
    a.src[0] += L.src_off;
    a.nsrc = L.nsrc; a.rows_per_src = L.rows;
    a.Cout = L.Cout; a.Cin = L.Cin; a.KS = L.KS;
    a.dgrad = 0; a.CK = L.CK; a.nchunk = L.nchunk_f; a.M = L.Cout; a.Mp = L.Mp_f;
    a.dst = ws + L.wpf;
    a.img = L.conv_path ? (L.bh ? AVC_IMG_K4H : AVC_IMG_K4) : AVC_IMG_PLAIN;
    if (L.wpf < 0) {
    } else if (L.x3_f) {
        PackArgs r;
        avc_pack_x3_args(r, p->par(params, L.w[0]), L.Cout, L.Cin, L.KS, 0, ws + L.wrs_f);
        out.push_back(r);
    } else {
        out.push_back(a);
    }
    if (L.wplain >= 0) {
        PackArgs b = a;
        b.img = AVC_IMG_PLAIN;
        b.dst = ws + L.wplain;
        out.push_back(b);
    }
    if (L.need_dgrad && L.x3_d) {
        PackArgs r;
        avc_pack_x3_args(r, p->par(params, L.w[0]), L.Cout, L.Cin, L.KS, 1, ws + L.wrs_d, L.dgM);
        out.push_back(r);
    } else if (L.need_dgrad) {
        a.dgrad = 1; a.CK = L.CKd; a.nchunk = L.nchunk_d; a.M = L.dgM; a.Mp = L.Mp_d;
        a.dst = ws + L.wpd;
        out.push_back(a);
    }
    if (L.nsrc > 1) {
        PackArgs b;
        memset(&b, 0, sizeof(b));
        for (int i = 0; i < L.nsrc; ++i) b.src[i] = p->par(params, L.b[i]);
        b.nsrc = L.nsrc; b.rows_per_src = L.rows;
        b.Cout = L.Cout; b.Cin = 1; b.KS = 1;
        b.dgrad = 0; b.CK = 32; b.nchunk = 1; b.M = L.Cout; b.Mp = L.Mp_f;
        b.dst = ws + L.bpk;
        b.img = AVC_IMG_PLAIN;
        out.push_back(b);
    }
}

static int in_fwd(float slope, const float* y, int Bn, int C, int T, const float* cond, long cond_sb, int cond_off, const float* res,
                  int res_mode, int Tres, float* out, float* stats, hipStream_t s, int Bfull = 0, int b0 = 0, bool pairs = false, int planar = 0, int nv = 0) {
    if (Bfull == 0) Bfull = Bn;
    INFwdArgs a;
    a.y = y; a.out = out; a.mean = stats + (long)b0 * C; a.rstd = stats + (long)Bfull * C + (long)b0 * C;
    a.cond = cond; a.cond_sb = cond_sb; a.cond_off = cond_off;
    a.res = res; a.res_mode = res ? res_mode : 0; a.Tres = Tres;
    a.R = Bn * C; a.C = C; a.T = T; a.relu = 1; a.slope = slope; a.planar = planar; a.nv_hint = nv;
    if (pairs) {
        a.R = Bn * (C / 2);
        return avc_launch_in_fwd_pairs(a, s);
    }
    return avc_launch_in_fwd(a, s);
}

static int conv_in_fwd(const avc_plan* p, ConvArgs& a, float slope, int Bn, int C, int T, const float* cond, long cond_sb, int cond_off,
                       const float* res, int res_mode, int Tres, float* out, float* stats, hipStream_t s, int Bfull = 0, int b0 = 0,
                       bool pairs = false, int planar = 0, int nv = 0) {
    if (Bfull == 0) Bfull = Bn;
    if (!planar && avc_conv_in_fusable(a, p->tun, res ? res_mode : AVC_RES_NONE, Tres)) {
        a.in.out = out;
        a.in.mean = stats + (long)b0 * C;
        a.in.rstd = stats + (long)Bfull * C + (long)b0 * C;
        a.in.cond = cond; a.in.cond_sb = cond_sb; a.in.cond_off = cond_off;
        a.in.res = res; a.in.res_mode = res ? res_mode : 0; a.in.Tres = Tres;
        a.in.C = C; a.in.relu = 1;
        return avc_launch_conv(a, s, 0, p->tun);
    }
    int rc = avc_launch_conv(a, s, 0, p->tun);
    if (rc) return rc;
    return in_fwd(slope, a.g[0].out, Bn, C, T, cond, cond_sb, cond_off, res, res_mode, Tres, out, stats, s, Bfull, b0, pairs, planar, nv);
}

static int in_bwd(float slope, const float* g, const float* y, const float* stats, int Bn, int C, int T, const float* cond,
                  long cond_sb, int cond_off, float* dy, float* dcond, hipStream_t s, bool pairs = false, int nv = 0) {
    INBwdArgs a;
    a.g = g; a.y = y; a.mean = stats; a.rstd = stats + (long)Bn * C;
    a.cond = cond; a.cond_sb = cond_sb; a.cond_off = cond_off;
    a.dy = dy; a.dcond = dcond; a.dcond_sb = cond_sb; a.dcond_off = cond_off;
    a.R = Bn * C; a.C = C; a.T = T; a.relu = 1; a.slope = slope; a.planar = 0; a.nv_hint = nv;
    if (pairs) {
        a.R = Bn * (C / 2);
        return avc_launch_in_bwd_pairs(a, s);
    }
    return avc_launch_in_bwd(a, s);
}

static int enc_front(const avc_plan* p, const EncNet& e, const float* params, float* ws, const float* x, long sxb,
                     long sxc, int sxt, hipStream_t s) {
    const int B = p->B, T0 = e.T[0];
    const float SL = e.slope;
    const bool bh = p->bh;
    const long CCr = bh ? e.CC / 2 : e.CC, Cbr = bh ? e.c.c_bank / 2 : e.c.c_bank;
    float* tail = ws + e.cat + (long)e.nb * Cbr * T0;
    if (bh) RUN(avc_launch_to_pairs(x, sxb, sxc, sxt, B, e.c.c_in, T0, tail, CCr * T0, T0, s));
    ConvArgs a;
    memset(&a, 0, sizeof(a));
    a.x.ptr = x; a.x.sb = sxb; a.x.sc = sxc; a.x.st = sxt; a.x.ps = 1;
    if (bh) { a.x.ptr = tail; a.x.sb = CCr * T0; a.x.sc = T0; a.x.st = 1; }
    a.B = B; a.Cred = bh ? e.c.c_in / 2 : e.c.c_in; a.Tsrc = T0;
    a.mode = 0; a.stride = 1; a.bf16 = p->compute;
    a.M = e.c.c_bank; a.Mp = avc_cdiv(e.c.c_bank, 128) * 128; a.Tout = T0;
    a.ob = CCr * T0; a.oc = T0; a.ot = 1; a.ops = 1;
    a.act = 1;
    a.slope = SL;
    a.ngroups = e.nb;
    a.img = bh ? AVC_IMG_K4H : AVC_IMG_K4;
    a.pairs = bh ? 1 : 0;
    for (int g = 0; g < e.nb; ++g) {
        const LayerP& L = p->layers[e.bank[g]];
        set_group(a.g[g], ws + L.wpf, p->par(params, L.b[0]), L.KS, L.CK, L.nchunk_f);
        a.g[g].out = ws + e.cat + (long)g * Cbr * T0;
    }
    RUN(avc_launch_conv(a, s, 0, p->tun));
    if (!bh) RUN(avc_launch_copy_rows(x, sxb, sxc, sxt, B, e.c.c_in, T0, tail, (long)e.CC * T0, T0, s));
    return 0;
}

static bool side_ready(const avc_plan* p);
static int pack_all(const avc_plan* p, const float* params, float* ws, hipStream_t s) {
    if (p->pack_tab_dev && !(p->tun.dbg_streams & 16)) {
        return avc_launch_pack_table(p->pack_tab_dev, p->pack_blk_dev, p->pack_nblk, p->pack_tab_bytes, params, ws, s);
    }
    std::vector<PackArgs> all;
    for (size_t i = 0; i < p->layers.size(); ++i)
        if (p->layers[i].wpf >= 0 || p->layers[i].wpd >= 0) pack_layer(p, p->layers[i], params, ws, all);
    return avc_launch_pack_batch(all.data(), (int)all.size(), s);
}

extern "C" int avc_plan_pack_weights(const avc_plan* p, const float* params, float* ws, void* stream) {
    if (!p || !params || !ws) return fail(-1, "avc_plan_pack_weights: null argument");
    RUN(pack_all(p, params, ws, (hipStream_t)stream));
    return 0;
}

static int forward_impl(const avc_plan* p, const float* params, const float* x, long sxb, long sxc, int sxt,
                        const float* xc, long scb, long scc, int sct, const float* eps, float* ws, hipStream_t s, bool packed = false,
                        const DecIn* din = nullptr) {
    const int B = p->B;
    const bool bh = p->bh;
    const int NV = (int)p->tun.in_pairs_nv;
    if (!packed) RUN(pack_all(p, params, ws, s));

    const bool do_spk = has_spk(p->flags), do_enc = has_enc(p->flags), do_dec = has_dec(p->flags);
    auto content_front = [&]() -> int {
        if (!do_enc) return 0;
        const EncNet& e = p->enc;
        const float SL = e.slope;
        const int Cc = e.c.c_h;
        const long C = bh ? Cc / 2 : Cc, CCr = bh ? e.CC / 2 : e.CC;
        RUN(enc_front(p, e, params, ws, x, sxb, sxc, sxt, s));
        ConvArgs a = mk_fwd(p, SL, p->layers[e.in_conv], params, ws, ws + e.cat, CCr * e.T[0], e.T[0], 1, B, e.T[0], ws + e.h0, (long)C * e.T[0], e.T[0], 1, 0);
        RUN(conv_in_fwd(p, a, SL, B, Cc, e.T[0], nullptr, 0, 0, nullptr, 0, 0, ws + e.out[0], ws + e.st0, s, 0, 0, bh, 0, NV));
        return 0;
    };
    const hipStream_t mainS = s;
    const hipStream_t sideS = do_spk ? fork_side(p, mainS) : mainS;
    if (!do_spk) RUN(content_front());
    if (do_spk) {
        const hipStream_t s = sideS;
        const EncNet& e = p->spk;
        const float SL = e.slope;
        const int Cc = e.c.c_h;
        const long C = bh ? Cc / 2 : Cc;
        const long CCr = bh ? e.CC / 2 : e.CC;
        RUN(enc_front(p, e, params, ws, xc, scb, scc, sct, s));
        RUN(content_front());
        {
            const LayerP& L = p->layers[e.in_conv];
            ConvArgs a = mk_fwd(p, SL, L, params, ws, ws + e.cat, CCr * e.T[0], e.T[0], 1, B, e.T[0], ws + e.h0, (long)C * e.T[0], e.T[0], 1, 1);
            RUN(avc_launch_conv(a, s, 0, p->tun));
        }
        for (int l = 0; l < e.n; ++l) {
            const int Ti = e.T[l], To = e.T[l + 1];
            ConvArgs a = mk_fwd(p, SL, p->layers[e.c1[l]], params, ws, ws + e.out[l], (long)C * Ti, Ti, 1, B, Ti, ws + e.a1[l], (long)C * Ti, Ti, 1, 1);
            RUN(avc_launch_conv(a, s, 0, p->tun));
            ConvArgs b = mk_fwd(p, SL, p->layers[e.c2[l]], params, ws, ws + e.a1[l], (long)C * Ti, Ti, 1, B, Ti, ws + e.a2[l], (long)C * To, To, 1, 1);
            b.g[0].out2 = ws + e.out[l + 1];
            set_res(b, ws + e.out[l], e.c.subsample[l] > 1 ? AVC_RES_AVGPOOL2 : AVC_RES_IDENTITY, (long)C * Ti, Ti, 1, Ti);
            RUN(avc_launch_conv(b, s, 0, p->tun));
        }
        const int Tn = e.T[e.n];
        if (bh) RUN(avc_launch_timepool_fwd_pairs(ws + e.out[e.n], B, Cc, Tn, ws + e.pooled, s));
        else RUN(avc_launch_timepool_fwd(ws + e.out[e.n], B, Cc, Tn, ws + e.pooled, s));
        {
            DenseArgs da;
            memset(&da, 0, sizeof(da));
            da.nlayers = 2 * e.nd + 1;
            da.B = B; da.C = Cc; da.slope = SL;
            da.in = ws + e.hd[0];
            da.emb = ws + p->emb;
            for (int l = 0; l < da.nlayers; ++l) {
                const bool last = (l == da.nlayers - 1);
                const LayerP& L = p->layers[last ? e.outl : ((l & 1) ? e.dn2[l / 2] : e.dn1[l / 2])];
                DenseLayer& D = da.layer[l];
                D.wp = ws + L.wpf;
                D.bias = p->par(params, L.b[0]);
                D.Cin = L.Cin; D.Cout = L.Cout; D.Kp = L.nchunk_f * L.CK; D.Mp = L.Mp_f;
                if (!last) {
                    D.act = ws + ((l & 1) ? e.d2[l / 2] : e.d1[l / 2]);
                    D.out2 = (l & 1) ? ws + e.hd[l / 2 + 1] : nullptr;
                }
                da.Kmax = D.Kp > da.Kmax ? D.Kp : da.Kmax;
                da.Wmax = D.Kp * D.Mp > da.Wmax ? D.Kp * D.Mp : da.Wmax;
            }
            RUN(avc_launch_dense(da, 0, s));
        }
    }

    if (do_enc) {
        const EncNet& e = p->enc;
        const float SL = e.slope;
        const int Cc = e.c.c_h;
        const long C = bh ? Cc / 2 : Cc, CCr = bh ? e.CC / 2 : e.CC;
        for (int l = 0; l < e.n; ++l) {
            const int Ti = e.T[l], To = e.T[l + 1];
            ConvArgs a = mk_fwd(p, SL, p->layers[e.c1[l]], params, ws, ws + e.out[l], (long)C * Ti, Ti, 1, B, Ti, ws + e.y1[l], (long)C * Ti, Ti, 1, 0);
            RUN(conv_in_fwd(p, a, SL, B, Cc, Ti, nullptr, 0, 0, nullptr, 0, 0, ws + e.a1[l], ws + e.st1[l], s, 0, 0, bh, 0, NV));
            ConvArgs b = mk_fwd(p, SL, p->layers[e.c2[l]], params, ws, ws + e.a1[l], (long)C * Ti, Ti, 1, B, Ti, ws + e.y2[l], (long)C * To, To, 1, 0);
            const int rmode = e.c.subsample[l] > 1 ? AVC_RES_AVGPOOL2 : AVC_RES_IDENTITY;
            RUN(conv_in_fwd(p, b, SL, B, Cc, To, nullptr, 0, 0, ws + e.out[l], rmode, Ti, ws + e.out[l + 1], ws + e.st2[l], s, 0, 0, bh, 0, NV));
        }
        const int Tb = p->Tb;
        ConvArgs h = mk_fwd(p, SL, p->layers[e.heads], params, ws, ws + e.out[e.n], (long)C * Tb, Tb, 1, B, Tb, ws + p->muls, (long)2 * e.c.c_out * Tb, Tb, 1, 0);
        h.pairs = 0;
        RUN(avc_launch_conv(h, s, 0, p->tun));
    }

    join_side(p, mainS, sideS);
    if (do_dec) {
        const DecNet& d = p->dec;
        const float SL = d.slope;
        const int Cc = d.c.c_h, Czc = d.c.c_in, Tb = p->Tb;
        const long C = bh ? Cc / 2 : Cc, Cz = bh ? Czc / 2 : Czc;
        const float* zs = ws + d.z;
        long zsb = Cz * Tb, zsc = Tb;
        int zst = 1;
        if (din && !bh) {
            zs = din->z; zsb = din->szb; zsc = din->szc; zst = din->szt;
        } else if (din) {
            RUN(avc_launch_to_pairs(din->z, din->szb, din->szc, din->szt, B, Czc, Tb, ws + d.z, Cz * Tb, Tb, s));
        } else if (bh) {
            RUN(avc_launch_reparam_fwd_pairs(ws + p->muls, eps, B, Czc, Tb, ws + d.z, s));
        } else {
            RUN(avc_launch_reparam_fwd(ws + p->muls, eps, B, Czc, Tb, ws + d.z, s));
        }
        const float* es = din ? din->emb : ws + p->emb;
        const long esb = din ? din->seb : d.c.c_cond, esc = din ? din->sec : 1;
        const long csb = (long)2 * d.n * 2 * Cc;
        {
            ConvArgs a = mk_fwd(p, SL, p->layers[d.affine], params, ws, es, 0, esc, (int)esb, 1, B, ws + d.cond, 0, 1, (int)csb, 0);
            RUN(avc_launch_conv(a, s, 0, p->tun));
        }
        auto dec_phase = [&](int b0, int Bn, hipStream_t s, int ph) -> int {
            const long ob0 = (long)b0 * C * Tb;
            const float* cond = ws + d.cond + (long)b0 * csb;
            if (ph == 0) {
                ConvArgs a = mk_fwd(p, SL, p->layers[d.in_conv], params, ws, zs + (long)b0 * zsb, zsb, zsc, zst, Bn, Tb, ws + d.y0 + ob0, (long)C * Tb, Tb, 1, 0);
                RUN(conv_in_fwd(p, a, SL, Bn, Cc, Tb, nullptr, 0, 0, nullptr, 0, 0, ws + d.out[0] + ob0, ws + d.st0, s, B, b0, bh, 0, NV));
                return 0;
            }
            if (ph == 2 * d.n + 1) {
                const int To = p->Tout;
                ConvArgs o = mk_fwd(p, SL, p->layers[d.out_conv], params, ws, ws + d.out[d.n] + (long)b0 * C * To, (long)C * To, To, 1, Bn, To,
                                    ws + p->decb + (long)b0 * p->M * To, (long)p->M * To, To, 1, 0);
                o.pairs = 0;
                RUN(avc_launch_conv(o, s, 0, p->tun));
                return 0;
            }
            const int l = (ph - 1) / 2;
            const int Ti = d.T[l], To = d.T[l + 1], up = d.c.upsample[l];
            const long oi = (long)b0 * C * Ti, oo = (long)b0 * C * To;
            if ((ph - 1) % 2 == 0) {
                ConvArgs a = mk_fwd(p, SL, p->layers[d.c1[l]], params, ws, ws + d.out[l] + oi, (long)C * Ti, Ti, 1, Bn, Ti, ws + d.y1[l] + oi, (long)C * Ti, Ti, 1, 0);
                RUN(conv_in_fwd(p, a, SL, Bn, Cc, Ti, cond, csb, (2 * l) * 2 * Cc, nullptr, 0, 0, ws + d.a1[l] + oi, ws + d.st1[l], s, B, b0, bh, 0, NV));
                return 0;
            }
            ConvArgs b = mk_fwd(p, SL, p->layers[d.c2[l]], params, ws, ws + d.a1[l] + oi, (long)C * Ti, Ti, 1, Bn, Ti, ws + d.y2[l] + oo, (long)C * To, To, 1, 0);
            b.ops = up;
            if (bh) {
                b.ops = 1;
                b.ob = (long)C * To; b.oc = Ti;
            }
            RUN(conv_in_fwd(p, b, SL, Bn, Cc, To, cond, csb, (2 * l + 1) * 2 * Cc, ws + d.out[l] + oi, up > 1 ? AVC_RES_UP2 : AVC_RES_IDENTITY, Ti,
                            ws + d.out[l + 1] + oo, ws + d.st2[l], s, B, b0, bh, (bh && up > 1) ? 1 : 0, NV));
            return 0;
        };
        const int nph = 2 * d.n + 2;
        if (B >= p->tun.dec_split_min && side_ready(p)) {
            const int Bh = B / 2;
            const hipStream_t s2 = fork_side(p, s);
            for (int ph = 0; ph < nph; ++ph) {
                RUN(dec_phase(0, Bh, s, ph));
                RUN(dec_phase(Bh, B - Bh, s2, ph));
            }
            join_side(p, s, s2);
        } else {
            for (int ph = 0; ph < nph; ++ph) RUN(dec_phase(0, B, s, ph));
        }
    }
    return 0;
}

extern "C" int avc_forward(const avc_plan* p, const float* params, const float* x, long sxb, long sxc, int sxt,
                           const float* x_cond, long scb, long scc, int sct, const float* eps, float* ws, void* stream) {
    if (!p || !params || !x || !ws) return fail(-1, "avc_forward: null argument");
    if (p->flags & AVC_PLAN_RAGGED) return fail(-8, "avc_forward: ragged plans run through avc_forward_ragged");
    if (p->flags & AVC_PLAN_DECODER_ONLY) return fail(-8, "avc_forward: decoder part plans run through avc_decoder_forward");
    if (!x_cond) {
        x_cond = x; scb = sxb; scc = sxc; sct = sxt;
    }
    return forward_impl(p, params, x, sxb, sxc, sxt, x_cond, scb, scc, sct, eps, ws, (hipStream_t)stream);
}

extern "C" int avc_forward_ex(const avc_plan* p, const float* params, const float* x, long sxb, long sxc, int sxt,
                              const float* x_cond, long scb, long scc, int sct, const float* eps, float* ws, int flags, void* stream) {
    if (!p || !params || !x || !ws) return fail(-1, "avc_forward_ex: null argument");
    if (p->flags & AVC_PLAN_RAGGED) return fail(-8, "avc_forward_ex: ragged plans run through avc_forward_ragged");
    if (p->flags & AVC_PLAN_DECODER_ONLY) return fail(-8, "avc_forward_ex: decoder part plans run through avc_decoder_forward");
    if (flags & ~AVC_FWD_WEIGHTS_PACKED) return fail(-1, "avc_forward_ex: unknown flag");
    if (!x_cond) {
        x_cond = x; scb = sxb; scc = sxc; sct = sxt;
    }
    return forward_impl(p, params, x, sxb, sxc, sxt, x_cond, scb, scc, sct, eps, ws, (hipStream_t)stream, (flags & AVC_FWD_WEIGHTS_PACKED) != 0);
}

extern "C" int avc_decoder_forward(const avc_plan* p, const float* params, const float* z, long szb, long szc, int szt, const float* emb,
                                   long seb, long sec, float* ws, int flags, void* stream) {
    if (!p || !params || !z || !emb || !ws) return fail(-1, "avc_decoder_forward: null argument");
    if (!(p->flags & AVC_PLAN_DECODER_ONLY)) return fail(-8, "avc_decoder_forward: the plan was not created with AVC_PLAN_DECODER_ONLY");
    if (p->flags & AVC_PLAN_RAGGED) return fail(-8, "avc_decoder_forward: ragged decoder plans run through avc_decoder_forward_ragged");
    if (flags & ~AVC_FWD_WEIGHTS_PACKED) return fail(-1, "avc_decoder_forward: unknown flag");
    const DecIn din = {z, szb, szc, szt, emb, seb, sec};
    return forward_impl(p, params, nullptr, 0, 0, 0, nullptr, 0, 0, 0, nullptr, ws, (hipStream_t)stream, (flags & AVC_FWD_WEIGHTS_PACKED) != 0,
                        &din);
}

extern "C" int avc_loss(const avc_plan* p, const float* x, long sxb, long sxc, int sxt, float lambda_rec, float* ws,
                        void* stream) {
    if (!p) return fail(-1, "avc_loss: null plan");
    if (p->flags & AVC_PLAN_PARTS) return fail(-8, "avc_loss: part plans have no loss (the caller's autograd takes the losses of solver.py:84-88)");
    if (p->flags & AVC_PLAN_INFERENCE) return fail(-8, "avc_loss: the plan was created with AVC_PLAN_INFERENCE");
    if (p->Tout != p->T) return fail(-7, "avc_loss: L1Loss needs dec and x of equal length (T % 8 == 0 for the stock config)");
    RUN(avc_launch_loss(ws + p->decb, x, sxb, sxc, sxt, p->B, p->M, p->T, ws + p->muls, p->dec.c.c_in, p->Tb, lambda_rec,
                        ws + p->ddec, ws + p->loss_partial, ws + p->losses, (hipStream_t)stream));
    return 0;
}

static int enc_back_front(BwdCtx& c, const EncNet& e, const float* x, long sxb, long sxc, int sxt, const float* dy_in) {
    const avc_plan* p = c.p;
    const bool bh = p->bh;
    const int B = p->B, T0 = e.T[0];
    const long C = bh ? e.c.c_h / 2 : e.c.c_h, CCr = bh ? e.CC / 2 : e.CC, Cbr = bh ? e.c.c_bank / 2 : e.c.c_bank;
    const float SL = e.slope;
    float* ws = c.ws;
    const LayerP& L = p->layers[e.in_conv];
    RUN(wgrad_layer(c, L, ws + e.cat, CCr * T0, T0, 1, dy_in, (long)C * T0, T0, 1, 1, B, T0, T0));
    if (!c.dry) {
        ConvArgs a = mk_dgrad(SL, L, ws, dy_in, (long)C * T0, T0, 1, 1, B, T0, T0, nullptr, CCr * T0, T0, 1);
        a.g[0].out2 = ws + e.dcat;
        a.g[0].mask = ws + e.cat;
        RUN(avc_launch_conv(a, c.s, 0, p->tun));
    }
    if (!c.dry && e.in_pass >= 0) {
        const long M = e.c.c_in;
        float* dx = ws + e.dx;
        ConvArgs a = mk_dgrad(SL, p->layers[e.in_pass], ws, dy_in, (long)C * T0, T0, 1, 1, B, T0, T0, dx, M * T0, T0, 1);
// ... 6 lines not shown
            RUN(avc_launch_conv(b, c.s, 0, p->tun));
        }
    }
    for (int g = 0; g < e.nb; ++g) {
        const LayerP& Lb = p->layers[e.bank[g]];
        if (bh)
            RUN(wgrad_layer(c, Lb, ws + e.cat + (long)e.nb * Cbr * T0, CCr * T0, T0, 1, ws + e.dcat + (long)g * Cbr * T0, CCr * T0, T0, 1, 1, B, T0, T0));
        else
            RUN(wgrad_layer(c, Lb, x, sxb, sxc, sxt, ws + e.dcat + (long)g * e.c.c_bank * T0, (long)e.CC * T0, T0, 1, 1, B, T0, T0));
    }
    return 0;
}

int avc_backward_impl(const avc_plan* p, const float* params, const float* x, long sxb, long sxc, int sxt, const float* xc,
                      long scb, long scc, int sct, const float* eps, const float* d_dec, const float* d_muls_up,
                      const float* d_emb_up, float lambda_kl, float* grads, float* ws, hipStream_t s, bool dry,
                      long* slab_need, const DecIn* din) {
    BwdCtx c;
    c.p = p; c.params = params; c.grads = grads; c.ws = ws; c.s = s; c.dry = dry; c.slab_used = 0;
    if (!dry) avc_prof_mark(0, s);
    c.nev = 0; c.dy_used = 0; c.pend_units = 0;
    const bool overlap = !dry && side_ready(p) && !(p->tun.dbg_streams & 1);
    const bool use_side = !dry && !(p->tun.dbg_streams & 2);
    c.wstream = overlap ? p->wstream[0] : s;
    const int B = p->B;
    const bool bh = p->bh;
    const int NV = (int)p->tun.in_pairs_nv;
    float* gA = ws + p->gA;
    float* gB = ws + p->gB;
    float* gC = ws + p->gC;
    float* dyA = nullptr;
    float* dyB = nullptr;
    auto rot = [&]() { float* t = gA; gA = gC; gC = t; };
    const bool do_spk = has_spk(p->flags), do_enc = has_enc(p->flags), do_dec = has_dec(p->flags);
    const bool dec_only = (p->flags & AVC_PLAN_DECODER_ONLY) != 0;

    if (do_dec) {
        const DecNet& d = p->dec;
        const float SL = d.slope;
        const int Cc = d.c.c_h, Czc = d.c.c_in, Tb = p->Tb, To = p->Tout;
        const long C = bh ? Cc / 2 : Cc, Cz = bh ? Czc / 2 : Czc;
        const long Mr = bh ? p->M / 2 : p->M;
        const long csb = (long)2 * d.n * 2 * Cc;
        const float* ddec = d_dec ? d_dec : ws + p->ddec;
        const float* zs = ws + d.z;
        long zsb = Cz * Tb, zsc = Tb;
        int zst = 1;
        if (din && !bh) { zs = din->z; zsb = din->szb; zsc = din->szc; zst = din->szt; }
        const float* es = din ? din->emb : ws + p->emb;
        const long esb = din ? din->seb : d.c.c_cond, esc = din ? din->sec : 1;
        if (bh) {
            if (!dry) RUN(avc_launch_to_pairs(ddec, (long)p->M * To, To, 1, B, p->M, To, ws + p->ddecp, Mr * To, To, s));
            ddec = ws + p->ddecp;
        }
        const LayerP& Lo = p->layers[d.out_conv];
        const LayerP& Li = p->layers[d.in_conv];
        float* dy2[AVC_MAX_BLOCKS];
        float* dy1[AVC_MAX_BLOCKS];
        for (int l = d.n - 1; l >= 0; --l) {
            dy2[l] = c.fresh((long)B * C * d.T[l + 1]);
            dy1[l] = c.fresh((long)B * C * d.T[l]);
        }
        float* dy0 = c.fresh((long)B * C * Tb);
        struct ChainSt {
            float *gA, *gB, *gC;
            bool fused;
        };
        auto chain_phase = [&](ChainSt& st, int b0, int Bn, hipStream_t s, int ph) -> int {
            auto half_in_bwd = [&](const float* g, long off, long yoff, long stoff, int T, int coff, bool cond, float* dy, int planar = 0) -> int {
                INBwdArgs a;
                a.g = g + off; a.y = ws + yoff + off;
                a.mean = ws + stoff + (long)b0 * Cc; a.rstd = ws + stoff + (long)B * Cc + (long)b0 * Cc;
                a.cond = cond ? ws + d.cond + (long)b0 * csb : nullptr; a.cond_sb = csb; a.cond_off = coff;
                a.dy = dy + off; a.dcond = cond ? ws + d.dcond + (long)b0 * csb : nullptr; a.dcond_sb = csb; a.dcond_off = coff;
                a.R = Bn * Cc; a.C = Cc; a.T = T; a.relu = 1; a.slope = SL; a.planar = planar; a.nv_hint = (int)p->tun.in_pairs_nv;
                if (bh) {
                    a.R = Bn * (Cc / 2);
                    return avc_launch_in_bwd_pairs(a, s);
                }
                return avc_launch_in_bwd(a, s);
            };
            auto dgrad_inb = [&](ConvArgs& a, bool keep_g, long off, long yoff, long stoff, int T, int coff, bool cond, float* dy, bool planar = false) -> int {
                st.fused = false;
                if (!planar && a.Tout == T && avc_conv_inb_fusable(a, p->tun)) {
                    a.inb.dy = dy + off; a.inb.y = ws + yoff + off;
                    a.inb.mean = ws + stoff + (long)b0 * Cc; a.inb.rstd = ws + stoff + (long)B * Cc + (long)b0 * Cc;
                    a.inb.cond = cond ? ws + d.cond + (long)b0 * csb : nullptr; a.inb.cond_sb = csb; a.inb.cond_off = coff;
                    a.inb.dcond = cond ? ws + d.dcond + (long)b0 * csb : nullptr; a.inb.dcond_sb = csb; a.inb.dcond_off = coff;
                    a.inb.C = Cc; a.inb.relu = 1;
                    if (!keep_g) a.g[0].out = nullptr;
                    st.fused = true;
                }
                return avc_launch_conv(a, s, 0, p->tun);
            };
            const bool was_fused = st.fused;
            if (ph == 0) {
                const long oi = (long)b0 * Mr * To, oo = (long)b0 * C * To;
                ConvArgs a = mk_dgrad(SL, Lo, ws, ddec + oi, Mr * To, To, 1, 1, Bn, To, To, st.gA + oo, (long)C * To, To, 1);
                const int ln = d.n - 1;
                RUN(dgrad_inb(a, true, oo, d.y2[ln], d.st2[ln], d.T[ln + 1], (2 * ln + 1) * 2 * Cc, true, dy2[ln], bh && d.c.upsample[ln] > 1));
                return 0;
            }
            if (ph == 2 * d.n + 1) {
                const long ob = (long)b0 * C * Tb;
                if (!was_fused) RUN(half_in_bwd(st.gA, ob, d.y0, d.st0, Tb, 0, false, dy0));
                st.fused = false;
                ConvArgs a = mk_dgrad(SL, Li, ws, dy0 + ob, (long)C * Tb, Tb, 1, 1, Bn, Tb, Tb, ws + p->dz + (long)b0 * Czc * Tb, (long)Czc * Tb, Tb, 1);
                a.pairs = 0;
                RUN(avc_launch_conv(a, s, 0, p->tun));
                return 0;
            }
            const int l = d.n - 1 - (ph - 1) / 2;
            const int Ti = d.T[l], T2 = d.T[l + 1], up = d.c.upsample[l];
            const long o2 = (long)b0 * C * T2, o1 = (long)b0 * C * Ti;
            if ((ph - 1) % 2 == 0) {
                if (!was_fused) RUN(half_in_bwd(st.gA, o2, d.y2[l], d.st2[l], T2, (2 * l + 1) * 2 * Cc, true, dy2[l], (bh && up > 1) ? 1 : 0));
                ConvArgs a = bh ? mk_dgrad(SL, p->layers[d.c2[l]], ws, dy2[l] + o2, (long)C * T2, Ti, 1, 1, Bn, Ti, Ti, st.gB + o1, (long)C * Ti, Ti, 1)
                                : mk_dgrad(SL, p->layers[d.c2[l]], ws, dy2[l] + o2, (long)C * T2, T2, up, up, Bn, Ti, Ti, st.gB + o1, (long)C * Ti, Ti, 1);
                RUN(dgrad_inb(a, false, o1, d.y1[l], d.st1[l], Ti, (2 * l) * 2 * Cc, true, dy1[l]));
                return 0;
            }
            if (!was_fused) RUN(half_in_bwd(st.gB, o1, d.y1[l], d.st1[l], Ti, (2 * l) * 2 * Cc, true, dy1[l]));
            ConvArgs a = mk_dgrad(SL, p->layers[d.c1[l]], ws, dy1[l] + o1, (long)C * Ti, Ti, 1, 1, Bn, Ti, Ti, st.gC + o1, (long)C * Ti, Ti, 1);
            set_res(a, st.gA + o2, up > 1 ? AVC_RES_UPT : AVC_RES_IDENTITY, (long)C * T2, T2, 1, T2);
            if (l > 0) RUN(dgrad_inb(a, true, o1, d.y2[l - 1], d.st2[l - 1], Ti, (2 * (l - 1) + 1) * 2 * Cc, true, dy2[l - 1], bh && d.c.upsample[l - 1] > 1));
            else RUN(dgrad_inb(a, true, o1, d.y0, d.st0, Tb, 0, false, dy0));
            float* t = st.gA; st.gA = st.gC; st.gC = t;
            return 0;
        };
        c.hold = true;
        const int early = p->tun.dec_wgrad_flush;
        auto rec_phase = [&](int ph) -> int {
            if (ph == 0) return wgrad_layer(c, Lo, ws + d.out[d.n], (long)C * To, To, 1, ddec, Mr * To, To, 1, 1, B, To, To);
            if (ph == 2 * d.n + 1) return wgrad_layer(c, Li, zs, zsb, zsc, zst, dy0, (long)C * Tb, Tb, 1, 1, B, Tb, Tb);
            const int l = d.n - 1 - (ph - 1) / 2;
            const int Ti = d.T[l], T2 = d.T[l + 1], up = d.c.upsample[l];
            if ((ph - 1) % 2 == 0) {
                if (bh) return wgrad_layer(c, p->layers[d.c2[l]], ws + d.a1[l], (long)C * Ti, Ti, 1, dy2[l], (long)C * T2, Ti, 1, 1, B, Ti, Ti);
                return wgrad_layer(c, p->layers[d.c2[l]], ws + d.a1[l], (long)C * Ti, Ti, 1, dy2[l], (long)C * T2, T2, up, up, B, Ti, Ti);
            }
            return wgrad_layer(c, p->layers[d.c1[l]], ws + d.out[l], (long)C * Ti, Ti, 1, dy1[l], (long)C * Ti, Ti, 1, 1, B, Ti, Ti);
        };
        {
            const int nph = 2 * d.n + 2;
            ChainSt st0 = {ws + p->gA, ws + p->gB, ws + p->gC, false}, st1 = st0;
            const bool split = use_side && B >= p->tun.dec_split_min && side_ready(p);
            const int Bh = B / 2;
            const hipStream_t s2 = split ? fork_side(p, s) : s;
            for (int ph = 0; ph < nph; ++ph) {
                if (!dry) {
                    if (split) {
                        RUN(chain_phase(st0, 0, Bh, s, ph));
                        RUN(chain_phase(st1, Bh, B - Bh, s2, ph));
                    } else {
                        RUN(chain_phase(st0, 0, B, s, ph));
                    }
                }
                RUN(rec_phase(ph));
                if (early > 0 && (int)c.pend.size() >= early && ph + 1 < nph) {
                    c.s_extra = s2;
                    c.target_wgs = (int)p->tun.dec_wgrad_wgs;
                    RUN(flush_wgrads(c, true));
                    c.s_extra = nullptr;
                    c.target_wgs = 0;
                }
            }
            if (split) join_side(p, s, s2);
        }
        const LayerP& La = p->layers[d.affine];
        RUN(wgrad_layer(c, La, es, 0, esc, (int)esb, ws + d.dcond, 0, 1, (int)csb, 1, 1, B, B));
        {
            WgradArgs w;
            memset(&w, 0, sizeof(w));
            w.x.ptr = ws + d.dcond; w.x.sb = 0; w.x.sc = csb; w.x.st = 1; w.x.ps = 1;
            w.dy.ptr = ws + La.wplain; w.dy.sb = 0; w.dy.sc = La.Mp_f; w.dy.st = 1; w.dy.ps = 1;
            w.B = 1; w.Cin = B; w.Cout = d.c.c_cond; w.Tin = La.Cout; w.Tout = La.Cout;
            w.KS = 1; w.padL = 0; w.stride = 1; w.bf16 = bh ? AVC_COMPUTE_BF16 : p->compute;
            w.rows_per_src = w.Cout;
            avc_wgrad_plan_batch(&w, 1, 256);
            const long off = c.slab_used;
            c.slab_used += (w.slab_need + 63) / 64 * 64;
            if (!dry) {
                w.slab = ws + p->slab + off;
                w.dbslab = nullptr;
                w.dw = ws + p->demb;
                w.db = nullptr;
                RUN(avc_launch_wgrad_batch(&w, 1, s, p->tun.wgrad_ablation));
                if (d_emb_up) RUN(avc_launch_add_transposed(ws + p->demb, d_emb_up, B, d.c.c_cond, s));
                if (dec_only) RUN(avc_launch_transpose(ws + p->demb_rm, ws + p->demb, d.c.c_cond, B, s));
            }
        }
        if (dec_only) {
            c.hold = false;
            RUN(flush_wgrads(c));
            if (!dry && p->side_state == 1) hipEventRecord(p->ev_dec_grads, c.wstream);
        }
        if (!dry && !dec_only) {
            float lk = lambda_kl / (float)((long)B * Czc * Tb);
            RUN(avc_launch_latent_bwd(ws + p->muls, eps, ws + p->dz, d_muls_up, B, Czc, Tb, lk, ws + p->dmuls, s));
            if (bh) RUN(avc_launch_to_pairs(ws + p->dmuls, (long)2 * Czc * Tb, Tb, 1, B, 2 * Czc, Tb, ws + p->dmulsp, (long)Czc * Tb, Tb, s));
        }
    }

    auto content_branch = [&]() -> int {
        const EncNet& e = p->enc;
        const float SL = e.slope;
        const int Cc = e.c.c_h, Tb = p->Tb;
        const long C = bh ? Cc / 2 : Cc, Co2 = bh ? e.c.c_out : 2 * e.c.c_out;
        const float* dmuls = ws + (bh ? p->dmulsp : p->dmuls);
        const LayerP& Lh = p->layers[e.heads];
        RUN(wgrad_layer(c, Lh, ws + e.out[e.n], (long)C * Tb, Tb, 1, dmuls, (long)Co2 * Tb, Tb, 1, 1, B, Tb, Tb));
        auto dgrad_inb = [&](ConvArgs& a, bool keep_g, const float* y, const float* st, int T, float* dy) -> bool {
            bool fused = false;
            if (a.Tout == T && avc_conv_inb_fusable(a, p->tun)) {
                a.inb.dy = dy; a.inb.y = y; a.inb.mean = st; a.inb.rstd = st + (long)B * Cc;
                a.inb.C = Cc; a.inb.relu = 1;
                if (!keep_g) a.g[0].out = nullptr;
                fused = true;
            }
            return fused;
        };
        bool fused = false;
        dyA = c.fresh((long)B * C * e.T[e.n]);
        {
            ConvArgs a = mk_dgrad(SL, Lh, ws, dmuls, (long)Co2 * Tb, Tb, 1, 1, B, Tb, Tb, gA, (long)C * Tb, Tb, 1);
            fused = dgrad_inb(a, true, ws + e.y2[e.n - 1], ws + e.st2[e.n - 1], e.T[e.n], dyA);
            if (!dry) RUN(avc_launch_conv(a, s, 0, p->tun));
        }
        for (int l = e.n - 1; l >= 0; --l) {
            const int Ti = e.T[l], T2 = e.T[l + 1], sub = e.c.subsample[l];
            const LayerP& L1 = p->layers[e.c1[l]];
            const LayerP& L2 = p->layers[e.c2[l]];
            if (!dry && !fused) RUN(in_bwd(SL, gA, ws + e.y2[l], ws + e.st2[l], B, Cc, T2, nullptr, 0, 0, dyA, nullptr, s, bh, NV));
            dyB = c.fresh((long)B * C * Ti);
            {
                ConvArgs a = mk_dgrad(SL, L2, ws, dyA, (long)C * T2, T2, 1, 1, B, T2, Ti, gB, (long)C * Ti, Ti, 1);
                fused = dgrad_inb(a, false, ws + e.y1[l], ws + e.st1[l], Ti, dyB);
                if (!dry) RUN(avc_launch_conv(a, s, 0, p->tun));
            }
            RUN(wgrad_layer(c, L2, ws + e.a1[l], (long)C * Ti, Ti, 1, dyA, (long)C * T2, T2, 1, 1, B, Ti, T2));
            if (!dry && !fused) RUN(in_bwd(SL, gB, ws + e.y1[l], ws + e.st1[l], B, Cc, Ti, nullptr, 0, 0, dyB, nullptr, s, bh, NV));
            dyA = c.fresh((long)B * C * Ti);
            {
                ConvArgs a = mk_dgrad(SL, L1, ws, dyB, (long)C * Ti, Ti, 1, 1, B, Ti, Ti, gC, (long)C * Ti, Ti, 1);
                set_res(a, gA, sub > 1 ? AVC_RES_POOLT : AVC_RES_IDENTITY, (long)C * T2, T2, 1, T2);
                fused = dgrad_inb(a, true, l > 0 ? ws + e.y2[l - 1] : ws + e.h0, l > 0 ? ws + e.st2[l - 1] : ws + e.st0, Ti, dyA);
                if (!dry) RUN(avc_launch_conv(a, s, 0, p->tun));
            }
            RUN(wgrad_layer(c, L1, ws + e.out[l], (long)C * Ti, Ti, 1, dyB, (long)C * Ti, Ti, 1, 1, B, Ti, Ti));
            rot();
        }
        if (!dry && !fused) RUN(in_bwd(SL, gA, ws + e.h0, ws + e.st0, B, Cc, e.T[0], nullptr, 0, 0, dyA, nullptr, s, bh, NV));
        RUN(enc_back_front(c, e, x, sxb, sxc, sxt, dyA));
        if (!dry) avc_prof_mark(3, s);
        RUN(flush_wgrads(c));
        return 0;
    };

    if (!do_dec && do_enc && !dry) {
        const int Czc = p->dec.c.c_in, Tb = p->Tb;
        float lk = lambda_kl / (float)((long)B * Czc * Tb);
        RUN(avc_launch_latent_bwd(ws + p->muls, nullptr, nullptr, d_muls_up, B, Czc, Tb, lk, ws + p->dmuls, s));
        if (bh) RUN(avc_launch_to_pairs(ws + p->dmuls, (long)2 * Czc * Tb, Tb, 1, B, 2 * Czc, Tb, ws + p->dmulsp, (long)Czc * Tb, Tb, s));
    }
    if (!do_dec && do_spk && !dry)
        RUN(avc_launch_transpose(ws + p->demb, d_emb_up, B, p->spk.c.c_out, s));

    const hipStream_t mainS = s;
    const hipStream_t sideS = (use_side && do_spk) ? fork_side(p, mainS) : mainS;
    if (!do_spk && do_enc) {
        c.s = mainS;
        c.wstream = overlap ? p->wstream[0] : mainS;
        RUN(content_branch());
    }
    if (do_spk) {
        const hipStream_t s = sideS;
        c.s = sideS;
        float* gA = ws + p->gA2;
        float* gB = ws + p->gB2;
        float* gC = ws + p->gC2;
        float* dyA = nullptr;
        float* dyB = nullptr;
        c.wstream = (overlap && sideS != mainS) ? p->wstream[1] : sideS;
        auto rot = [&]() { float* t = gA; gA = gC; gC = t; };
        const EncNet& e = p->spk;
        const float SL = e.slope;
        const int Cc = e.c.c_h;
        const long C = bh ? Cc / 2 : Cc;
        float* dhA = ws + p->dhA;
        const LayerP& Lo = p->layers[e.outl];
        {
            DenseArgs da;
            memset(&da, 0, sizeof(da));
            da.nlayers = 2 * e.nd + 1;
            da.B = B; da.C = Cc; da.slope = SL;
            da.in = ws + p->demb;
            da.in2 = nullptr;
            da.dpooled = dhA;
            float* dzl[AVC_DENSE_MAXL];
            for (int l = 0; l < da.nlayers; ++l) {
                const bool last = (l == da.nlayers - 1);
                const LayerP& L = p->layers[last ? e.outl : ((l & 1) ? e.dn2[l / 2] : e.dn1[l / 2])];
                DenseLayer& D = da.layer[l];
                D.wp = ws + L.wpd;
                D.Cin = L.Cin; D.Cout = L.Cout; D.Kp = L.nchunk_d * L.CKd; D.Mp = L.Mp_d;
                dzl[l] = last ? nullptr : c.fresh((long)Cc * B);
                if (!last) {
                    D.act = ws + ((l & 1) ? e.d2[l / 2] : e.d1[l / 2]);
                    D.dz = dzl[l];
                }
                da.Kmax = D.Kp > da.Kmax ? D.Kp : da.Kmax;
                da.Wmax = D.Kp * D.Mp > da.Wmax ? D.Kp * D.Mp : da.Wmax;
            }
            if (!dry) RUN(avc_launch_dense(da, 1, s));
            if (!dry) avc_prof_mark(1, s);
            {
                const hipStream_t ws0 = overlap ? p->wstream[0] : mainS;
                if (overlap && sideS != mainS) {
                    hipEventRecord(p->ev_dense, sideS);
                    hipStreamWaitEvent(ws0, p->ev_dense, 0);
                }
                c.s = mainS;
                c.wstream = ws0;
                c.hold = false;
                RUN(flush_wgrads(c));
                if (!dry && p->side_state == 1) hipEventRecord(p->ev_dec_grads, c.wstream);
                if (!dry) avc_prof_mark(5, c.wstream);
                c.s = sideS;
                c.wstream = (overlap && sideS != mainS) ? p->wstream[1] : sideS;
            }
// ... 878 lines not shown
```

### adaptive_voice_conversion_amd/csrc/ops_api.hip

```cpp
#include <hip/hip_runtime.h>
#include <math.h>

#include "avc_common.h"
#include "avc_internal.h"

#include <string.h>

static avc_tuning make_default_tuning() {
    avc_tuning t;
    memset(&t, 0, sizeof(t));
    t.struct_size = (int)sizeof(avc_tuning);
    t.dec_split_min = 128;
    t.dgrad_par = 1;
    t.side_prio = 1;
    t.bank_switch = 1;
    t.conv_ck5 = 8;
    t.wgrad_batch = 12;
    t.wgrad_batch_wgs = 256;
    t.wgrad_target_wgs = 256;
    t.wgrad_batch_units = 1L << 40;
    t.tile_thr11 = 8192;
    t.tile_thr21 = 4096;
    t.ck16_wgs = 256;
    t.ck32_wgs = 256;
    t.kg_wgs = 256;
    t.bh_ck5 = 8;
    t.in_pairs_nv = 1;
    t.wgrad_cw8 = 0;
    t.dec_wgrad_flush = 0;
    t.dec_wgrad_wgs = 128;
    t.conv_walk = 0;
    t.conv_walk_min = 2;
    t.conv_in_fuse = 1;
    return t;
}
const avc_tuning& avc_default_tuning() {
    static const avc_tuning t = make_default_tuning();
    return t;
}
avc_tuning& avc_op_tuning() {
    static thread_local avc_tuning t = make_default_tuning();
    return t;
}

extern "C" {
void avc_tuning_init(avc_tuning* t) {
    if (t) *t = avc_default_tuning();
}
void avc_get_op_tuning(avc_tuning* out) {
    if (out) *out = avc_op_tuning();
}
int avc_set_tuning(const char* name, int value) {
    if (!name) return -1;
    avc_tuning& t = avc_op_tuning();
#define AVC_TUNE_FIELD(f) if (!strcmp(name, #f)) { t.f = value; return 0; }
    AVC_TUNE_FIELD(single_stream) AVC_TUNE_FIELD(dec_split_min) AVC_TUNE_FIELD(conv_x3) AVC_TUNE_FIELD(wgrad_x3) AVC_TUNE_FIELD(dgrad_par)
    AVC_TUNE_FIELD(bank_switch) AVC_TUNE_FIELD(conv_ck5) AVC_TUNE_FIELD(wgrad_batch) AVC_TUNE_FIELD(wgrad_batch_wgs) AVC_TUNE_FIELD(wgrad_target_wgs)
    AVC_TUNE_FIELD(conv_ablation) AVC_TUNE_FIELD(wgrad_ablation) AVC_TUNE_FIELD(op_compute_dtype) AVC_TUNE_FIELD(tile12_wgs) AVC_TUNE_FIELD(side_prio) AVC_TUNE_FIELD(wgrad_batch_units)
    AVC_TUNE_FIELD(tile_thr11) AVC_TUNE_FIELD(tile_thr21) AVC_TUNE_FIELD(ck16_wgs) AVC_TUNE_FIELD(ck32_wgs) AVC_TUNE_FIELD(kg_wgs) AVC_TUNE_FIELD(bh_ck5) AVC_TUNE_FIELD(in_pairs_nv) AVC_TUNE_FIELD(conv_min_lds) AVC_TUNE_FIELD(wgrad_cw8) AVC_TUNE_FIELD(dec_wgrad_flush) AVC_TUNE_FIELD(dec_wgrad_wgs)
    AVC_TUNE_FIELD(conv_walk) AVC_TUNE_FIELD(conv_walk_min) AVC_TUNE_FIELD(conv_in_fuse) AVC_TUNE_FIELD(dbg_streams)
#undef AVC_TUNE_FIELD
    if (!strcmp(name, "compute")) { t.op_compute_dtype = (value == AVC_COMPUTE_BF16) ? AVC_COMPUTE_BF16 : AVC_COMPUTE_F32; return 0; }
    return -1;
}

long avc_packed_weight_floats_x3(int Cout, int Cin, int KS, int dgrad) {
    const int Cred = dgrad ? Cout : Cin;
    if (!((KS == 5 && Cred % 16 == 0) || (KS == 1 && Cred >= 32))) return -1;
    return avc_conv_x3_image_floats(dgrad ? Cin : Cout, Cred, KS);
}
int avc_pack_weight_x3(const float* w, int Cout, int Cin, int KS, int dgrad, float* dst, void* stream) {
    if (avc_packed_weight_floats_x3(Cout, Cin, KS, dgrad) < 0) return -2;
    PackArgs p;
    avc_pack_x3_args(p, w, Cout, Cin, KS, dgrad, dst);
    return avc_launch_pack(p, (hipStream_t)stream);
}

int avc_gather_segments(const float* corpus, long n_rows, int M, const long* starts, int B, int T, float* out, void* stream) {
    if (!corpus || !starts || !out) return -1;
    return avc_launch_gather_segments(corpus, n_rows, M, starts, B, T, out, (hipStream_t)stream);
}

static bool op_bh() { const int d = avc_op_tuning().op_compute_dtype; return d == AVC_COMPUTE_BF16S || d == 4; }
static void op_compute(ConvArgs& a) {
    const int d = avc_op_tuning().op_compute_dtype;
    a.bf16 = d == 4 ? AVC_COMPUTE_BF16S : d;
    a.pairs = d == AVC_COMPUTE_BF16S ? 1 : 0;
}

int avc_instnorm_fwd(const float* y, int B, int C, int T, const float* cond, long cond_sb, int cond_off, int relu, const float* res, int res_mode,
                     int Tres, float* out, float* mean, float* rstd, void* stream);
int avc_instnorm_fwd_pairs(const void* y, int B, int C, int T, const float* cond, long cond_sb, int cond_off, int relu, const void* res, int res_mode,
                           int Tres, int planar, void* out, float* mean, float* rstd, void* stream);
int avc_instnorm_bwd(const float* g, const float* y, const float* mean, const float* rstd, int B, int C, int T, const float* cond, long cond_sb,
                     int cond_off, int relu, float* dy, float* dcond, long dcond_sb, int dcond_off, void* stream);

long avc_packed_weight_floats(int Cout, int Cin, int KS, int dgrad) {
    int CK = avc_conv_ck(avc_op_tuning(), KS);
    int red = dgrad ? Cout : Cin, M = dgrad ? Cin : Cout;
    if (op_bh()) red = (red + 1) / 2;
    int nchunk = avc_cdiv(red, CK), Mp = avc_cdiv(M, 128) * 128;
    return (long)nchunk * KS * CK * Mp;
}

int avc_pack_weight(const float* const* srcs, int nsrc, int rows_per_src, int Cout, int Cin, int KS, int dgrad,
                    float* dst, void* stream) {
    if (nsrc < 1 || nsrc > 12 || nsrc * rows_per_src != Cout) return -1;
    PackArgs p;
    memset(&p, 0, sizeof(p));
    for (int i = 0; i < nsrc; ++i) p.src[i] = srcs[i];
    p.nsrc = nsrc;
    p.rows_per_src = rows_per_src;
    p.Cout = Cout;
    p.Cin = Cin;
    p.KS = KS;
    p.dgrad = dgrad;
    p.CK = avc_conv_ck(avc_op_tuning(), KS);
    p.img = AVC_IMG_K4;
    int red = dgrad ? Cout : Cin;
    if (op_bh()) { red = (red + 1) / 2; p.img = AVC_IMG_K4H; }
    p.M = dgrad ? Cin : Cout;
    p.nchunk = avc_cdiv(red, p.CK);
    p.Mp = avc_cdiv(p.M, 128) * 128;
    p.dst = dst;
// ... 67 lines not shown
    return avc_instnorm_fwd(y, B, C, T, cond, cond_sb, cond_off, relu, res, res_mode, Tres, out, mean, rstd, stream);
}

int avc_conv1d_dgrad(const float* dy, long syb, long syc, int syt, int yps, int B, int Cout, int Tdy, const float* wpd,
                     int Cin, int KS, int stride, int Tin, float* dx, long ob, long oc, int ot, const float* res,
                     int res_mode, long rb, long rc, int rt, int Tres, float* dx2, const float* mask, int tile,
                     void* stream) {
    ConvArgs a;
    memset(&a, 0, sizeof(a));
    op_compute(a);
    const bool bh = op_bh();
    if (bh && (Cout & 1)) return -2;
    a.x.ptr = dy; a.x.sb = syb; a.x.sc = syc; a.x.st = syt; a.x.ps = yps;
    a.B = B; a.Cred = bh ? Cout / 2 : Cout; a.Tsrc = Tdy;
    a.mode = 1; a.stride = stride;
    int padL = KS / 2, padR = (KS % 2 == 0) ? KS / 2 - 1 : KS / 2;
    a.mirror = (KS > 1) ? 1 : 0;
    a.M = Cin; a.Mp = avc_cdiv(Cin, 128) * 128;
    a.Tout = Tin;
    a.ob = ob; a.oc = oc; a.ot = ot; a.ops = 1;
    a.act = 0;
    a.res_mode = res_mode; a.res_to_primary = 1;
    a.rb = rb; a.rc = rc; a.rt = rt; a.Tres = Tres;
    a.ngroups = 1;
    a.g[0].CK = avc_conv_ck(avc_op_tuning(), KS);
    a.g[0].wp = wpd; a.g[0].bias = nullptr; a.g[0].out = dx; a.g[0].out2 = dx2; a.g[0].res = res; a.g[0].mask = mask;
    a.g[0].KS = KS; a.g[0].padL = padL; a.g[0].padR = padR; a.g[0].nchunk = avc_cdiv(a.Cred, a.g[0].CK);
    a.img = bh ? AVC_IMG_K4H : AVC_IMG_K4;
    if (tile == 97) { a.img = AVC_IMG_X3; a.g[0].CK = KS == 1 ? 32 : 16; a.g[0].nchunk = avc_cdiv(Cout, a.g[0].CK); }
    return avc_launch_conv(a, (hipStream_t)stream, tile, avc_op_tuning());
}

static void op_wgrad_args(WgradArgs& a, int B, int Cin, int Cout, int Tin, int Tout, int KS, int stride) {
    memset(&a, 0, sizeof(a));
    const avc_tuning& t = avc_op_tuning();
    a.bf16 = (t.op_compute_dtype == AVC_COMPUTE_F32 && t.wgrad_x3) ? AVC_COMPUTE_F32X3 : (op_bh() ? AVC_COMPUTE_BF16S : t.op_compute_dtype);
    a.B = B; a.Cin = Cin; a.Cout = Cout; a.Tin = Tin; a.Tout = Tout;
    a.KS = KS; a.padL = KS / 2; a.stride = stride;
    a.x.ps = 1; a.dy.ps = 1;
    a.cw8 = t.wgrad_cw8 ? 1 : 0;
}
int avc_conv1d_dgrad_in_bwd(const float* dy, long syb, long syc, int syt, int yps, int B, int Cout, int Tdy, const float* wpd, int Cin, int KS,
                            int stride, int Tin, float* g_out, const float* res, int res_mode, int Tres, const float* y, const float* mean,
                            const float* rstd, const float* cond, long cond_sb, int cond_off, int relu, float* dy_out, float* dcond,
                            long dcond_sb, int dcond_off, int* fused, void* stream) {
    const bool bh = op_bh();
    if (bh && (avc_op_tuning().op_compute_dtype != AVC_COMPUTE_BF16S || (Cin & 1) || (Cout & 1))) return -2;
    ConvArgs a;
    memset(&a, 0, sizeof(a));
    op_compute(a);
    a.x.ptr = dy; a.x.sb = syb; a.x.sc = syc; a.x.st = syt; a.x.ps = yps;
    a.B = B; a.Cred = bh ? Cout / 2 : Cout; a.Tsrc = Tdy;
    a.mode = 1; a.stride = stride;
    const int padL = KS / 2, padR = (KS % 2 == 0) ? KS / 2 - 1 : KS / 2;
    a.mirror = (KS > 1) ? 1 : 0;
    a.M = Cin; a.Mp = avc_cdiv(Cin, 128) * 128;
    a.Tout = Tin;
    const long Cr = bh ? Cin / 2 : Cin;
    a.ob = Cr * Tin; a.oc = Tin; a.ot = 1; a.ops = 1;
    a.slope = relu == 2 ? AVC_LRELU_SLOPE : 0.f;
    a.res_mode = res ? res_mode : AVC_RES_NONE; a.res_to_primary = 1;
    a.rb = Cr * Tres; a.rc = Tres; a.rt = 1; a.Tres = Tres;
    a.ngroups = 1;
    a.g[0].CK = avc_conv_ck(avc_op_tuning(), KS);
    a.g[0].wp = wpd; a.g[0].out = g_out; a.g[0].res = res;
    a.g[0].KS = KS; a.g[0].padL = padL; a.g[0].padR = padR; a.g[0].nchunk = avc_cdiv(a.Cred, a.g[0].CK);
    a.img = bh ? AVC_IMG_K4H : AVC_IMG_K4;
    const bool fuse = avc_conv_inb_fusable(a, avc_op_tuning());
    if (fused) *fused = fuse ? 1 : 0;
    if (fuse) {
        a.inb.dy = dy_out; a.inb.y = y; a.inb.mean = mean; a.inb.rstd = rstd;
        a.inb.cond = cond; a.inb.cond_sb = cond_sb; a.inb.cond_off = cond_off;
        a.inb.dcond = dcond; a.inb.dcond_sb = dcond_sb; a.inb.dcond_off = dcond_off;
        a.inb.C = Cin; a.inb.relu = relu ? 1 : 0;
        return avc_launch_conv(a, (hipStream_t)stream, 0, avc_op_tuning());
    }
    if (!g_out) return -1;
    int rc = avc_launch_conv(a, (hipStream_t)stream, 0, avc_op_tuning());
    if (rc) return rc;
    if (bh) return avc_instnorm_bwd_pairs(g_out, y, mean, rstd, B, Cin, Tin, cond, cond_sb, cond_off, relu, 0, dy_out, dcond, dcond_sb, dcond_off, stream);
    return avc_instnorm_bwd(g_out, y, mean, rstd, B, Cin, Tin, cond, cond_sb, cond_off, relu, dy_out, dcond, dcond_sb, dcond_off, stream);
}

long avc_conv1d_wgrad_ws_floats(int B, int Cin, int Cout, int Tout, int KS) {
    long need = 0;
    for (int stride = 1; stride <= 2; ++stride) {
        WgradArgs a;
        op_wgrad_args(a, B, Cin, Cout, Tout * stride, Tout, KS, stride);
        avc_wgrad_plan_batch(&a, 1, avc_op_tuning().wgrad_target_wgs);
        const long n = a.slab_need + a.dbslab_need + 64;
        need = n > need ? n : need;
    }
    return need;
}
int avc_conv1d_wgrad(const float* x, long sxb, long sxc, int sxt, const float* dy, long syb, long syc, int syt, int yps,
                     int B, int Cin, int Cout, int Tin, int Tout, int KS, int stride, float* dW, float* db, float* ws,
                     void* stream) {
    WgradArgs a;
    op_wgrad_args(a, B, Cin, Cout, Tin, Tout, KS, stride);
    a.x.ptr = x; a.x.sb = sxb; a.x.sc = sxc; a.x.st = sxt; a.x.ps = 1;
    a.dy.ptr = dy; a.dy.sb = syb; a.dy.sc = syc; a.dy.st = syt; a.dy.ps = yps;
    avc_wgrad_plan_batch(&a, 1, avc_op_tuning().wgrad_target_wgs);
    a.slab = ws;
    a.dbslab = db ? ws + a.slab_need : nullptr;
    a.dw = dW; a.db = db; a.rows_per_src = Cout;
    return avc_launch_wgrad_batch(&a, 1, (hipStream_t)stream, avc_op_tuning().wgrad_ablation);
}

int avc_instnorm_fwd(const float* y, int B, int C, int T, const float* cond, long cond_sb, int cond_off, int relu,
                     const float* res, int res_mode, int Tres, float* out, float* mean, float* rstd, void* stream) {
    INFwdArgs a;
    a.y = y; a.out = out; a.mean = mean; a.rstd = rstd;
    a.cond = cond; a.cond_sb = cond_sb; a.cond_off = cond_off;
    a.res = res; a.res_mode = res ? res_mode : 0; a.Tres = Tres;
    a.R = B * C; a.C = C; a.T = T; a.relu = relu ? 1 : 0;
    a.slope = relu == 2 ? AVC_LRELU_SLOPE : 0.f;
    a.planar = 0; a.nv_hint = 0;
    return avc_launch_in_fwd(a, (hipStream_t)stream);
}

int avc_instnorm_bwd(const float* g, const float* y, const float* mean, const float* rstd, int B, int C, int T,
                     const float* cond, long cond_sb, int cond_off, int relu, float* dy, float* dcond, long dcond_sb,
                     int dcond_off, void* stream) {
    INBwdArgs a;
    a.g = g; a.y = y; a.mean = mean; a.rstd = rstd;
    a.cond = cond; a.cond_sb = cond_sb; a.cond_off = cond_off;
    a.dy = dy; a.dcond = dcond; a.dcond_sb = dcond_sb; a.dcond_off = dcond_off;
    a.R = B * C; a.C = C; a.T = T; a.relu = relu ? 1 : 0;
    a.slope = relu == 2 ? AVC_LRELU_SLOPE : 0.f;
    a.planar = 0; a.nv_hint = 0;
    return avc_launch_in_bwd(a, (hipStream_t)stream);
}

int avc_instnorm_fwd_pairs(const void* y, int B, int C, int T, const float* cond, long cond_sb, int cond_off, int relu, const void* res, int res_mode,
                           int Tres, int planar, void* out, float* mean, float* rstd, void* stream) {
    INFwdArgs a;
    a.y = (const float*)y; a.out = (float*)out; a.mean = mean; a.rstd = rstd;
    a.cond = cond; a.cond_sb = cond_sb; a.cond_off = cond_off;
    a.res = (const float*)res; a.res_mode = res ? res_mode : 0; a.Tres = Tres;
    a.R = B * (C / 2); a.C = C; a.T = T; a.relu = relu ? 1 : 0;
    a.slope = relu == 2 ? AVC_LRELU_SLOPE : 0.f;
    a.planar = planar ? 1 : 0;
    a.nv_hint = (int)avc_op_tuning().in_pairs_nv;
    return avc_launch_in_fwd_pairs(a, (hipStream_t)stream);
}
int avc_instnorm_bwd_pairs(const void* g, const void* y, const float* mean, const float* rstd, int B, int C, int T, const float* cond, long cond_sb,
                           int cond_off, int relu, int planar, void* dy, float* dcond, long dcond_sb, int dcond_off, void* stream) {
    INBwdArgs a;
    a.g = (const float*)g; a.y = (const float*)y; a.mean = mean; a.rstd = rstd;
    a.cond = cond; a.cond_sb = cond_sb; a.cond_off = cond_off;
    a.dy = (float*)dy; a.dcond = dcond; a.dcond_sb = dcond_sb; a.dcond_off = dcond_off;
    a.R = B * (C / 2); a.C = C; a.T = T; a.relu = relu ? 1 : 0;
    a.slope = relu == 2 ? AVC_LRELU_SLOPE : 0.f;
    a.planar = planar ? 1 : 0;
    a.nv_hint = (int)avc_op_tuning().in_pairs_nv;
    return avc_launch_in_bwd_pairs(a, (hipStream_t)stream);
}
int avc_to_pairs(const float* x, long sxb, long sxc, long sxt, int B, int C, int T, void* dst, void* stream) {
    return avc_launch_to_pairs(x, sxb, sxc, sxt, B, C, T, (float*)dst, (long)(C / 2) * T, T, (hipStream_t)stream);
}

long avc_clip_adam_ws_floats(long n) { return avc_adam_blocks(n); }

int avc_clip_adam_step(float* p, float* g, float* m, float* v, float* vmax, long n, int step, float lr, float beta1,
                       float beta2, float eps, float weight_decay, int amsgrad, float max_norm, float grad_prescale,
                       int write_clipped, float* ws, float* gnorm_out, void* stream) {
// ... 15 lines not shown
```

### include/avc_hip.h

```cpp
#ifndef AVC_HIP_H
#define AVC_HIP_H
#ifdef __cplusplus
extern "C" {
#endif

#define AVC_MAX_BLOCKS 8

typedef struct avc_encoder_cfg {
    int c_in, c_h, c_out, kernel_size, bank_size, bank_scale, c_bank, n_conv_blocks, n_dense_blocks;
    int subsample[AVC_MAX_BLOCKS];
    int act;
} avc_encoder_cfg;

typedef struct avc_decoder_cfg {
    int c_in, c_cond, c_h, c_out, kernel_size, n_conv_blocks;
    int upsample[AVC_MAX_BLOCKS];
    int act;
} avc_decoder_cfg;

typedef struct avc_model_cfg {
    avc_encoder_cfg spk;
    avc_encoder_cfg enc;
    avc_decoder_cfg dec;
} avc_model_cfg;

typedef struct avc_plan avc_plan;

int avc_version(void);
const char* avc_last_error(void);

int avc_plan_create(const avc_model_cfg* cfg, int B, int T, int T_cond, avc_plan** out);
#define AVC_PLAN_INFERENCE 1
#define AVC_PLAN_SPEAKER_ONLY 2
#define AVC_PLAN_CONTENT_ONLY 32
#define AVC_PLAN_DECODER_ONLY 64
#define AVC_PLAN_PART_GRADS 128
#define AVC_PLAN_INPUT_GRADS 256
int avc_plan_create_ex(const avc_model_cfg* cfg, int B, int T, int T_cond, int flags, avc_plan** out);
int avc_plan_flags(const avc_plan* p);
int avc_plan_side_priority(const avc_plan* p);
void avc_plan_destroy(avc_plan* p);
int avc_plan_num_params(const avc_plan* p);
long avc_plan_param_floats(const avc_plan* p);
int avc_plan_param_info(const avc_plan* p, int i, long* offset, long* numel, int dims[3]);
long avc_plan_workspace_floats(const avc_plan* p);
long avc_plan_buffer(const avc_plan* p, const char* name);
int avc_plan_out_len(const avc_plan* p);
int avc_plan_latent_len(const avc_plan* p);

typedef struct avc_relu_site {
    int kind, B, C, T;
    long act_off, sb, sc, st;
    long y_off, stat_off, cond_off, cond_sb;
    long storage;
} avc_relu_site;
int avc_plan_num_relu_sites(const avc_plan* p);
int avc_plan_relu_site(const avc_plan* p, int i, avc_relu_site* out);

#define AVC_GRADS_ALL 0
#define AVC_GRADS_DECODER 1
#define AVC_GRADS_ENCODERS 2
#define AVC_GRADS_SPEAKER 3
#define AVC_GRADS_CONTENT 4
int avc_plan_param_range(const avc_plan* p, int part, long* offset, long* numel);
int avc_plan_stream_wait_grads(const avc_plan* p, int part, void* stream);

typedef struct avc_tuning {
    int struct_size;
    int single_stream;
    int dec_split_min;
    int conv_x3;
    int wgrad_x3;
    int dgrad_par;
    int bank_switch;
    int conv_ck5;
    int wgrad_batch;
    int wgrad_batch_wgs;
    int wgrad_target_wgs;
    int conv_ablation;
    int wgrad_ablation;
    int op_compute_dtype;
    int side_prio;
    int tile12_wgs;
    long wgrad_batch_units;
    long tile_thr11, tile_thr21, ck16_wgs, ck32_wgs, kg_wgs;
    long conv_min_lds;
    long in_pairs_nv;
    long bh_ck5;
    long wgrad_cw8;
    long dec_wgrad_flush;
    long dec_wgrad_wgs;
    long conv_walk;
    long conv_walk_min;
    long conv_in_fuse;
    long dbg_streams;
} avc_tuning;
void avc_tuning_init(avc_tuning* t);
#define AVC_PLAN_X3 4
#define AVC_PLAN_RAGGED 8
#define AVC_PLAN_BF16S 16
#define AVC_ERR_PAIR_SHAPE (-12)
int avc_plan_create_tuned(const avc_model_cfg* cfg, int B, int T, int T_cond, int flags, const avc_tuning* tuning, avc_plan** out);
int avc_plan_set_single_stream(avc_plan* p, int on);

int avc_plan_set_compute_dtype(avc_plan* p, int dtype);
int avc_plan_compute_dtype(const avc_plan* p);

int avc_forward(const avc_plan* p, const float* params, const float* x, long sxb, long sxc, int sxt,
                const float* x_cond, long scb, long scc, int sct, const float* eps, float* ws, void* stream);
#define AVC_FWD_WEIGHTS_PACKED 1
int avc_plan_pack_weights(const avc_plan* p, const float* params, float* ws, void* stream);
int avc_forward_ex(const avc_plan* p, const float* params, const float* x, long sxb, long sxc, int sxt,
                   const float* x_cond, long scb, long scc, int sct, const float* eps, float* ws, int flags, void* stream);

int avc_plan_create_ragged(const avc_model_cfg* cfg, int B, const int* T, const int* T_cond, const avc_tuning* tuning, avc_plan** out);
int avc_plan_ragged_out(const avc_plan* p, int* out_len, long* out_off);
int avc_forward_ragged(const avc_plan* p, const float* params, const float* x, const float* x_cond, float* ws, void* stream);
#define AVC_PLAN_EMB_INPUT 512
int avc_plan_create_ragged_ex(const avc_model_cfg* cfg, int B, const int* T, const int* T_cond, int flags, const avc_tuning* tuning,
                              avc_plan** out);
int avc_forward_ragged_emb(const avc_plan* p, const float* params, const float* x, const float* emb, long seb, long sec, float* ws,
                           void* stream);
#define AVC_PLAN_FANOUT 1024
int avc_plan_create_ragged_fanout(const avc_model_cfg* cfg, int S, const int* T, int N, const int* src_of, int flags,
                                  const avc_tuning* tuning, avc_plan** out);
int avc_plan_ragged_latents(const avc_plan* p, int* len, long* off);
int avc_decoder_forward_ragged(const avc_plan* p, const float* params, const float* z, int zc, const float* emb, long seb, long sec,
                               float* ws, void* stream);
int avc_backward_ragged(const avc_plan* p, const float* params, const float* x_cond, const float* d_emb, long seb, long sec, float* ws,
                        void* stream);
int avc_plan_create_ragged_content_grads(const avc_model_cfg* cfg, int S, const int* T, const avc_tuning* tuning, avc_plan** out);
int avc_content_backward_ragged(const avc_plan* p, const float* params, const float* x, const float* d_muls, float* ws, void* stream);

int avc_loss(const avc_plan* p, const float* x, long sxb, long sxc, int sxt, float lambda_rec, float* ws, void* stream);

int avc_backward(const avc_plan* p, const float* params, const float* x, long sxb, long sxc, int sxt,
                 const float* x_cond, long scb, long scc, int sct, const float* eps, const float* d_dec,
                 const float* d_muls_up, const float* d_emb_up, float lambda_kl, float* grads, float* ws, void* stream);

int avc_decoder_forward(const avc_plan* p, const float* params, const float* z, long szb, long szc, int szt, const float* emb, long seb,
                        long sec, float* ws, int flags, void* stream);
int avc_decoder_backward(const avc_plan* p, const float* params, const float* z, long szb, long szc, int szt, const float* emb, long seb,
                         long sec, const float* d_dec, float* grads, float* ws, void* stream);

int avc_instnorm_fwd_pairs(const void* y, int B, int C, int T, const float* cond, long cond_sb, int cond_off, int relu, const void* res, int res_mode,
                           int Tres, int planar, void* out, float* mean, float* rstd, void* stream);
int avc_instnorm_bwd_pairs(const void* g, const void* y, const float* mean, const float* rstd, int B, int C, int T, const float* cond, long cond_sb,
                           int cond_off, int relu, int planar, void* dy, float* dcond, long dcond_sb, int dcond_off, void* stream);
int avc_to_pairs(const float* x, long sxb, long sxc, long sxt, int B, int C, int T, void* dst, void* stream);

long avc_clip_adam_ws_floats(long n);
int avc_clip_adam_step(float* p, float* g, float* m, float* v, float* vmax, long n, int step, float lr, float beta1,
                       float beta2, float eps, float weight_decay, int amsgrad, float max_norm, float grad_prescale,
                       int write_clipped, float* ws, float* gnorm_out, void* stream);

int avc_set_tuning(const char* name, int value);
void avc_get_op_tuning(avc_tuning* out);

int avc_gather_segments(const float* corpus, long n_rows, int M, const long* starts, int B, int T, float* out,
                        void* stream);

int avc_dsp_num_frames(long L, int hop_length);
long avc_dsp_basis_floats(int n_fft, int win_length, int inverse);
long avc_dsp_basis_scratch_floats(int n_fft, int win_length);
int avc_dsp_make_basis(int n_fft, int hop_length, int win_length, int inverse, float* dense_scratch, float* packed, void* stream);
int avc_dsp_stft(const float* y, long L, int n_fft, int hop_length, int win_length, const float* basis_fwd, float* frames_ws,
                 float* spec, void* stream);
int avc_dsp_istft(const float* spec, int T, int n_fft, int hop_length, int win_length, const float* basis_inv, float* tf_ws, float* y,
                  void* stream);
long avc_dsp_griffin_lim_ws_floats(int T, int n_fft, int hop_length, int win_length);
int avc_dsp_griffin_lim(const float* S, int T, int n_fft, int hop_length, int win_length, int n_iter, const float* basis_fwd,
                        const float* basis_inv, float* ws, float* y, void* stream);
int avc_dsp_stft_batch(const float* y, long L, int B, int n_fft, int hop_length, int win_length, const float* basis_fwd, float* frames_ws,
                       float* spec, void* stream);
int avc_dsp_istft_batch(const float* spec, int B, int T, int n_fft, int hop_length, int win_length, const float* basis_inv, float* tf_ws,
                        float* y, void* stream);
int avc_dsp_griffin_lim_batch(const float* S, int B, int T, int n_fft, int hop_length, int win_length, int n_iter, const float* basis_fwd,
                              const float* basis_inv, float* ws, float* y, void* stream);
int avc_dsp_griffin_lim_ragged(const float* S, const int* toff, const int* toff_host, int B, int Ttot, int n_fft, int hop_length, int win_length,
                               int n_iter, const float* basis_fwd, const float* basis_inv, float* ws, float* y, void* stream);
int avc_dsp_magnitude(const float* spec, int n_fft, int T, float* mag, void* stream);
int avc_dsp_db_normalize(const float* in, int C, int T, float ref_db, float max_db, float* out, void* stream);
int avc_dsp_denormalize_amp(const float* in, int C, int T, float ref_db, float max_db, float* out, void* stream);
int avc_dsp_preemphasis(const float* y, long L, float a, float* out, void* stream);
int avc_dsp_deemphasis(const float* x, long L, float a, float* out, void* stream);
int avc_dsp_frame_power(const float* y, long L, int frame_length, int hop_length, float* out, void* stream);

long avc_packed_weight_floats(int Cout, int Cin, int KS, int dgrad);
int avc_pack_weight(const float* const* srcs, int nsrc, int rows_per_src, int Cout, int Cin, int KS, int dgrad,
                    float* dst, void* stream);
long avc_packed_weight_floats_x3(int Cout, int Cin, int KS, int dgrad);
int avc_pack_weight_x3(const float* w, int Cout, int Cin, int KS, int dgrad, float* dst, void* stream);
int avc_conv1d_fwd(const float* x, long sxb, long sxc, int sxt, int B, int Cin, int Tin, const float* wp,
                   const float* bias, int Cout, int KS, int stride, int act, float* out, long ob, long oc, int ot,
                   int ops, const float* res, int res_mode, long rb, long rc, int rt, int Tres, float* out2, int tile,
                   void* stream);
int avc_conv1d_dgrad(const float* dy, long syb, long syc, int syt, int yps, int B, int Cout, int Tdy, const float* wpd,
                     int Cin, int KS, int stride, int Tin, float* dx, long ob, long oc, int ot, const float* res,
                     int res_mode, long rb, long rc, int rt, int Tres, float* dx2, const float* mask, int tile,
                     void* stream);
long avc_conv1d_wgrad_ws_floats(int B, int Cin, int Cout, int Tout, int KS);
int avc_conv1d_wgrad(const float* x, long sxb, long sxc, int sxt, const float* dy, long syb, long syc, int syt, int yps,
                     int B, int Cin, int Cout, int Tin, int Tout, int KS, int stride, float* dW, float* db, float* ws,
                     void* stream);
int avc_instnorm_fwd(const float* y, int B, int C, int T, const float* cond, long cond_sb, int cond_off, int relu,
                     const float* res, int res_mode, int Tres, float* out, float* mean, float* rstd, void* stream);
int avc_instnorm_bwd(const float* g, const float* y, const float* mean, const float* rstd, int B, int C, int T,
                     const float* cond, long cond_sb, int cond_off, int relu, float* dy, float* dcond, long dcond_sb,
                     int dcond_off, void* stream);
int avc_conv1d_in_fwd(const float* x, long sxb, long sxc, int sxt, int B, int Cin, int Tin, const float* wp, const float* bias, int Cout, int KS,
                      int stride, int ops, float* y, const float* cond, long cond_sb, int cond_off, int relu, const float* res, int res_mode,
                      int Tres, float* out, float* mean, float* rstd, int* fused, void* stream);
int avc_conv1d_dgrad_in_bwd(const float* dy, long syb, long syc, int syt, int yps, int B, int Cout, int Tdy, const float* wpd, int Cin, int KS,
                            int stride, int Tin, float* g_out, const float* res, int res_mode, int Tres, const float* y, const float* mean,
                            const float* rstd, const float* cond, long cond_sb, int cond_off, int relu, float* dy_out, float* dcond,
                            long dcond_sb, int dcond_off, int* fused, void* stream);

#ifdef __cplusplus
}
#endif
#endif
```

Before: 43550 mel-segments/sec.

## Extend fused conv+InstanceNorm epilogue to 128-frame rows with 64x128 tiles

Extends the fused convolution + InstanceNorm forward/backward epilogue to handle Tout=128 by using 64x128 wide tiles (WN=2), with optional K-group split and a larger LDS staging tile. Per-path bit flags gate the wide fusion, and by default only encoder backward (dgrad + IN-backward) is enabled. The aim is to remove separate InstanceNorm kernel launches and the extra global round trips at full-length layers. In exchange the epilogue loops over two passes, uses more LDS per block, and adds extra barriers on the KG=2 path, which may lower occupancy.

New measurement: 43760 mel-segments/sec (median of 6 runs). About the same (+0.5%).

```diff
diff --git a/adaptive_voice_conversion_amd/_lib.py b/adaptive_voice_conversion_amd/_lib.py
--- a/adaptive_voice_conversion_amd/_lib.py
+++ b/adaptive_voice_conversion_amd/_lib.py
@@ -152,6 +152,8 @@
     lib.avc_conv1d_dgrad_in_bwd.argtypes = [c_void_p, c_long, c_long, c_int, c_int, c_int, c_int, c_int, c_void_p, c_int, c_int, c_int, c_int,
                                             c_void_p, c_void_p, c_int, c_int, c_void_p, c_void_p, c_void_p, c_void_p, c_long, c_int, c_int,
                                             c_void_p, c_void_p, c_long, c_int, c_void_p, c_void_p]
+    lib.avc_conv1d_in_fwd_mode.argtypes = lib.avc_conv1d_in_fwd.argtypes[:-1] + [c_long, c_void_p]
+    lib.avc_conv1d_dgrad_in_bwd_mode.argtypes = lib.avc_conv1d_dgrad_in_bwd.argtypes[:-1] + [c_long, c_void_p]
     lib.avc_instnorm_fwd_pairs.argtypes = [c_void_p, c_int, c_int, c_int, c_void_p, c_long, c_int, c_int, c_void_p, c_int, c_int, c_int,
                                            c_void_p, c_void_p, c_void_p, c_void_p]
     lib.avc_instnorm_bwd_pairs.argtypes = [c_void_p, c_void_p, c_void_p, c_void_p, c_int, c_int, c_int, c_void_p, c_long, c_int, c_int, c_int,
diff --git a/adaptive_voice_conversion_amd/csrc/conv_gemm.hip b/adaptive_voice_conversion_amd/csrc/conv_gemm.hip
--- a/adaptive_voice_conversion_amd/csrc/conv_gemm.hip
+++ b/adaptive_voice_conversion_amd/csrc/conv_gemm.hip
@@ -429,7 +429,13 @@
                     for (int r = 0; r < 16; ++r) red[((wm * WN + wn) * 16 + r) * 64] = acc[wm][wn][r];
         }
         __syncthreads();
-        if (kg > 0) return;
+        if constexpr ((INF || INB) && WN == 2) {
+            if (kg > 0) {
+                __syncthreads();
+                __syncthreads();
+                return;
+            }
+        } else if (kg > 0) return;
 #pragma unroll
         for (int k2 = 1; k2 < KG; ++k2) {
             const float* rk = smem + ((k2 - 1) * 4 + wave) * (WM * WN * 16 * 64) + lane;
@@ -443,17 +449,17 @@
     }
 
     if constexpr (INF) {
-        static_assert(WM == 1 && WN == 1 && (BF == 0 || BF == 2) && !PAR && !RAG && !WALK && !MIRROR, "fused InstanceNorm epilogue: forward, 64 x 64 tiles, fp32 or bf16 pairs");
+        static_assert(WM == 1 && (WN == 1 || WN == 2) && (BF == 0 || BF == 2) && !PAR && !RAG && !WALK && !MIRROR, "fused InstanceNorm epilogue: forward, 64 x 64 or 64 x 128 tiles, fp32 or bf16 pairs");
         if (KG > 1) __syncthreads();
-        if constexpr (BF == 2) conv_epilogue_in_pairs(a, g, acc[0][0], smem, tid, wave_m, wave_n, li, h, m_tile0, q.b0);
-        else conv_epilogue_in(a, g, acc[0][0], smem, tid, wave_m, wave_n, li, h, m_tile0, q.b0);
+        if constexpr (BF == 2) conv_epilogue_in_pairs<WN>(a, g, acc[0], smem, tid, wave_m, wave_n, li, h, m_tile0, q.b0);
+        else conv_epilogue_in<WN>(a, g, acc[0], smem, tid, wave_m, wave_n, li, h, m_tile0, q.b0);
         return;
     }
     if constexpr (INB) {
-        static_assert(WM == 1 && WN == 1 && (BF == 0 || BF == 2) && !RAG && !WALK && !INF, "fused InstanceNorm-backward epilogue: input gradient on 64 x 64 tiles, fp32 or bf16 pairs");
+        static_assert(WM == 1 && (WN == 1 || (WN == 2 && !PAR)) && (BF == 0 || BF == 2) && !RAG && !WALK && !INF, "fused InstanceNorm-backward epilogue: input gradient on 64 x 64 or 64 x 128 tiles, fp32 or bf16 pairs");
         if (KG > 1) __syncthreads();
-        if constexpr (BF == 2) conv_epilogue_in_bwd_pairs(a, g, acc[0][0], smem, tid, wave_m, h, m_tile0, q.b0, q.t0, colb[0] - q.b0, colt[0], colv[0]);
-        else conv_epilogue_in_bwd(a, g, acc[0][0], smem, tid, wave_m, h, m_tile0, q.b0, q.t0, colb[0] - q.b0, colt[0], colv[0]);
+        if constexpr (BF == 2) conv_epilogue_in_bwd_pairs<WN>(a, g, acc[0], smem, tid, wave_m, h, m_tile0, q.b0, q.t0, colb, colt, colv);
+        else conv_epilogue_in_bwd<WN>(a, g, acc[0], smem, tid, wave_m, h, m_tile0, q.b0, q.t0, colb, colt, colv);
         return;
     }
     if (!(a.dbg & 8)) {
@@ -830,8 +836,22 @@
     return (tile == 11 && (fast == 1 || ((fast == -1 || fast == 14) && !mir))) || (tile == 21 && fast == 14 && !mir);
 }
 
-template <int BF>
+template <int BF, int KG = 1>
 static void conv_launch_wide(const ConvArgs& a, bool mir, dim3 grid, dim3 block, size_t lds, hipStream_t stream) {
+    if constexpr (BF != 1) {
+        const bool ck16 = a.g[0].CK == 16;
+        if (a.in.out) {
+            if (ck16) hipLaunchKernelGGL((conv_gemm_kernel<1, 2, false, 5, 2, KG, BF, false, false, false, true>), grid, block, lds, stream, a);
+            else hipLaunchKernelGGL((conv_gemm_kernel<1, 2, false, 5, 1, KG, BF, false, false, false, true>), grid, block, lds, stream, a);
+            return;
+        }
+        if (a.inb.dy) {
+            if (ck16) hipLaunchKernelGGL((conv_gemm_kernel<1, 2, true, 5, 2, KG, BF, false, false, false, false, true>), grid, block, lds, stream, a);
+            else hipLaunchKernelGGL((conv_gemm_kernel<1, 2, true, 5, 1, KG, BF, false, false, false, false, true>), grid, block, lds, stream, a);
+            return;
+        }
+    }
+    if constexpr (KG != 1) return;
     if (mir) hipLaunchKernelGGL((conv_gemm_kernel<1, 2, true, 5, 1, 1, BF>), grid, block, lds, stream, a);
     else hipLaunchKernelGGL((conv_gemm_kernel<1, 2, false, 5, 1, 1, BF>), grid, block, lds, stream, a);
 }
@@ -844,6 +864,9 @@
     else hipLaunchKernelGGL((conv_gemm_kernel<1, 1, false, 5, 2, KG, BF, true>), grid, block, lds, stream, a);
 }
 
+static bool conv_in_wide_rows(const ConvArgs& a, long family_bits) {
+    return family_bits != 0 && a.Tout == 128 && a.ngroups == 1 && a.g[0].KS == 5 && (a.g[0].CK == 8 || a.g[0].CK == 16) && a.stride == 1 && a.x.ps == 1;
+}
 bool avc_conv_in_fusable(const ConvArgs& a, const avc_tuning& tun, int res_mode, int Tres) {
     const int Tn_ = a.Tout * a.ops;
     if (res_mode != AVC_RES_NONE && !((res_mode == AVC_RES_IDENTITY && Tres == Tn_) || (res_mode == AVC_RES_UP2 && 2 * Tres == Tn_) ||
@@ -851,13 +874,15 @@
     if (!tun.conv_in_fuse || a.mode != 0 || a.ngroups != 1 || a.rag.tile) return false;
     const bool bh = a.bf16 == AVC_COMPUTE_BF16S;
     if (bh ? (a.img != AVC_IMG_K4H || !a.pairs || a.ops != 1 || (a.M & 1) || a.x.ps != 1 || a.x.st != 1) : (a.bf16 != AVC_COMPUTE_F32 || a.img != AVC_IMG_K4 || a.pairs)) return false;
-    if (a.Tout != 16 && a.Tout != 32 && a.Tout != 64) return false;
+    const bool wide = conv_in_wide_rows(a, tun.conv_in_fuse & (AVC_IN_FUSE_T128_ENC_FWD | AVC_IN_FUSE_T128_DEC_FWD));
+    if (a.Tout != 16 && a.Tout != 32 && a.Tout != 64 && !wide) return false;
+    if (wide && a.ops != 1) return false;
     if (a.ops != 1 && a.ops != 2) return false;
     if (a.ops == 2 && (a.M & 1)) return false;
     if (a.act || a.res_mode != AVC_RES_NONE || a.g[0].out2 || a.g[0].mask) return false;
     const int C = (bh ? a.M / 2 : a.M) / a.ops, Tn = a.Tout * a.ops;
     if (a.ot != 1 || a.oc != Tn || a.ob != (long)C * Tn) return false;
-    if (conv_geom(0, a.stride, a.Tout, a.g[0].KS, 64, 0).SPT != 64 / a.Tout) return false;
+    if (!wide && conv_geom(0, a.stride, a.Tout, a.g[0].KS, 64, 0).SPT != 64 / a.Tout) return false;
     return avc_conv_pick_tile(tun, a.Mp, a.B, a.Tout, 1, a.Cred * a.g[0].KS * (bh ? 2 : 1)) == 11;
 }
 
@@ -865,7 +890,8 @@
     if (!tun.conv_in_fuse || a.mode != 1 || a.ngroups != 1 || a.rag.tile) return false;
     const bool bh = a.bf16 == AVC_COMPUTE_BF16S;
     if (bh ? (a.img != AVC_IMG_K4H || !a.pairs || (a.M & 1) || a.x.ps != 1 || a.x.st != 1) : (a.bf16 != AVC_COMPUTE_F32 || a.img != AVC_IMG_K4 || a.pairs)) return false;
-    if (a.Tout != 16 && a.Tout != 32 && a.Tout != 64) return false;
+    const bool wide = a.mirror && conv_in_wide_rows(a, tun.conv_in_fuse & (AVC_IN_FUSE_T128_ENC_BWD | AVC_IN_FUSE_T128_DEC_BWD));
+    if (a.Tout != 16 && a.Tout != 32 && a.Tout != 64 && !wide) return false;
     if (a.ops != 1 || a.act || a.g[0].out2 || a.g[0].mask || a.g[0].bias) return false;
     const long Mr = bh ? a.M / 2 : a.M;
     if (a.ot != 1 || a.oc != a.Tout || a.ob != Mr * a.Tout) return false;
@@ -874,7 +900,7 @@
         if (!((a.res_mode == AVC_RES_IDENTITY && a.Tres == a.Tout) || (a.res_mode == AVC_RES_POOLT && 2 * a.Tres == a.Tout) ||
               (a.res_mode == AVC_RES_UPT && a.Tres == 2 * a.Tout))) return false;
     }
-    if (conv_geom(1, a.stride, a.Tout, a.g[0].KS, 64, 0).SPT != 64 / a.Tout) return false;
+    if (!wide && conv_geom(1, a.stride, a.Tout, a.g[0].KS, 64, 0).SPT != 64 / a.Tout) return false;
     return avc_conv_pick_tile(tun, a.Mp, a.B, a.Tout, 1, a.Cred * a.g[0].KS * (bh ? 2 : 1)) == 11;
 }
 
@@ -897,15 +923,18 @@
             if ((long)(a.Mp / 64) * ntn >= tun.tile12_wgs) tile = 12;
         }
     }
+    const int in_tile = a.Tout == 128 ? 12 : 11;
     if (a.in.out) {
-        if (!avc_conv_in_fusable(a, tun, a.in.res ? a.in.res_mode : AVC_RES_NONE, a.in.Tres) || (force_tile != 0 && force_tile != 11) || tile != 11) return -2;
+        if (!avc_conv_in_fusable(a, tun, a.in.res ? a.in.res_mode : AVC_RES_NONE, a.in.Tres) || (force_tile != 0 && force_tile != in_tile) || (tile != 11 && tile != in_tile)) return -2;
         if (!a.in.mean || !a.in.rstd || a.in.C != a.M / a.ops) return -2;
+        tile = in_tile;
     }
     if (a.inb.dy) {
-        if (a.in.out || !avc_conv_inb_fusable(a, tun) || (force_tile != 0 && force_tile != 11) || tile != 11) return -2;
+        if (a.in.out || !avc_conv_inb_fusable(a, tun) || (force_tile != 0 && force_tile != in_tile) || (tile != 11 && tile != in_tile)) return -2;
         if (!a.inb.y || !a.inb.mean || !a.inb.rstd || a.inb.C != a.M) return -2;
-    }
-    if (tile == 12 && !wide_ok) return -2;
+        tile = in_tile;
+    }
+    if (tile == 12 && !wide_ok && !(a.in.out || a.inb.dy)) return -2;
     if (tile != 11 && tile != 21 && tile != 12) return -2;
     const int BM = (tile == 21) ? 128 : 64, BN = (tile == 12) ? 128 : 64;
     for (int gi = 0; gi < a.ngroups; ++gi) {
@@ -920,8 +949,11 @@
     dim3 grid(rag ? a.rag.ntiles : conv_ntiles_n(a, BN), a.Mp / BM, a.ngroups);
     int kgroups = 1;
     if (!rag && a.bf16 != AVC_COMPUTE_BF16S && tile == 11 && a.ngroups == 1 && (long)grid.x * grid.y <= tun.kg_wgs && a.g[0].nchunk >= 4 && 2 * lds <= 160 * 1024 && !a.dbg) kgroups = 2;
+    if ((a.in.out || a.inb.dy) && tile == 12 && a.bf16 != AVC_COMPUTE_BF16S && (long)(a.Mp / 64) * conv_ntiles_n(a, 64) <= tun.kg_wgs && a.g[0].nchunk >= 4 &&
+        2 * conv_lds_bytes(a, 64, 64) <= 160 * 1024 && 2 * lds <= 160 * 1024 && !a.dbg) kgroups = 2;
     lds *= kgroups;
-    if ((a.in.out || a.inb.dy) && lds < AVC_IN_LDS_BYTES) lds = AVC_IN_LDS_BYTES;
+    const size_t in_lds = tile == 12 ? AVC_IN_LDS_BYTES_WIDE : AVC_IN_LDS_BYTES;
+    if ((a.in.out || a.inb.dy) && lds < in_lds) lds = in_lds;
     if (lds > 160 * 1024) return -5;
     if (tun.conv_min_lds > 0 && (size_t)tun.conv_min_lds > lds && tun.conv_min_lds <= 160 * 1024) lds = (size_t)tun.conv_min_lds;
     dim3 block(AVC_THREADS * kgroups);
@@ -969,7 +1001,11 @@
         else if (bf == 1) { CALL_(1); }      \
         else { CALL_(0); }                   \
     } while (0)
-    if (a.inb.dy) {
+    if ((a.inb.dy || a.in.out) && tile == 12) {
+        if (bf == 2) conv_launch_wide<2>(a, mir, grid, block, lds, stream);
+        else if (kgroups == 2) conv_launch_wide<0, 2>(a, mir, grid, block, lds, stream);
+        else conv_launch_wide<0>(a, mir, grid, block, lds, stream);
+    } else if (a.inb.dy) {
         if (bf == 2) conv_launch_inb<1, 2>(a, mir, fast, grid, block, lds, stream);
         else if (kgroups == 2) conv_launch_inb<2, 0>(a, mir, fast, grid, block, lds, stream);
         else conv_launch_inb<1, 0>(a, mir, fast, grid, block, lds, stream);
diff --git a/adaptive_voice_conversion_amd/csrc/conv_shared.h b/adaptive_voice_conversion_amd/csrc/conv_shared.h
--- a/adaptive_voice_conversion_amd/csrc/conv_shared.h
+++ b/adaptive_voice_conversion_amd/csrc/conv_shared.h
@@ -167,6 +167,8 @@
 
 #define AVC_IN_LDT 68
 #define AVC_IN_LDS_BYTES (64 * AVC_IN_LDT * 4)
+#define AVC_IN_LDT_OF(WN_) (64 * (WN_) + 4)
+#define AVC_IN_LDS_BYTES_WIDE (64 * AVC_IN_LDT_OF(2) * 4)
 static __device__ __forceinline__ float4 conv_in_res4(const float* rrow, int mode, int t, int Tres) {
     float4 r = make_float4(0.f, 0.f, 0.f, 0.f);
     if (mode == AVC_RES_IDENTITY) {
@@ -180,19 +182,26 @@
     }
     return r;
 }
-static __device__ void conv_epilogue_in(const ConvArgs& a, const ConvGroup& g, const f32x16& acc, float* tile, int tid, int wave_m, int wave_n,
+template <int WN>
+static __device__ void conv_epilogue_in(const ConvArgs& a, const ConvGroup& g, const f32x16 (&acc)[WN], float* tile, int tid, int wave_m, int wave_n,
                                         int li, int h, int m_tile0, int b0) {
+    constexpr int LDT = AVC_IN_LDT_OF(WN), QPR = 4 * WN;
     const ConvINFuse& f = a.in;
-    const int col = wave_n * 32 + li;
-#pragma unroll
-    for (int r = 0; r < 16; ++r) {
-        const int row = wave_m * 32 + (r & 3) + 8 * (r >> 2) + 4 * h;
-        const int m = m_tile0 + row;
-        const float bs = g.bias ? g.bias[m < a.M ? m : a.M - 1] : 0.f;
-        tile[row * AVC_IN_LDT + col] = acc[r] + bs;
+#pragma unroll
+    for (int wn = 0; wn < WN; ++wn) {
+        const int col = wave_n * (32 * WN) + wn * 32 + li;
+#pragma unroll
+        for (int r = 0; r < 16; ++r) {
+            const int row = wave_m * 32 + (r & 3) + 8 * (r >> 2) + 4 * h;
+            const int m = m_tile0 + row;
+            const float bs = g.bias ? g.bias[m < a.M ? m : a.M - 1] : 0.f;
+            tile[row * LDT + col] = acc[wn][r] + bs;
+        }
     }
     __syncthreads();
-    const int r = tid >> 2, qd = tid & 3;
+#pragma unroll
+    for (int pass = 0; pass < WN; ++pass) {
+    const int r = pass * (64 / WN) + tid / QPR, qd = tid % QPR;
     const int m = m_tile0 + r;
     const int Tout = a.Tout, lpr = Tout >> 4;
     const int bl = (16 * qd) / Tout, t0 = 16 * qd - bl * Tout;
@@ -201,10 +210,10 @@
     float v[16];
 #pragma unroll
     for (int k = 0; k < 4; ++k) {
-        const float4 x = *(const float4*)(tile + r * AVC_IN_LDT + 16 * qd + 4 * k);
+        const float4 x = *(const float4*)(tile + r * LDT + 16 * qd + 4 * k);
         v[4 * k] = x.x; v[4 * k + 1] = x.y; v[4 * k + 2] = x.z; v[4 * k + 3] = x.w;
     }
-    const int ops = a.ops;
+    const int ops = WN == 1 ? a.ops : 1;
     const int c = ops == 2 ? m >> 1 : m, j = ops == 2 ? (m & 1) : 0;
     const int Tn = Tout * ops;
     const float invT = 1.0f / (float)Tn;
@@ -236,7 +245,7 @@
         for (int i = 0; i < 16; ++i) v[i] = w[i];
         fbase = 2 * t0 + 16 * j;
     }
-    if (!valid) return;
+    if (!valid) continue;
     const long rowi = (long)b * f.C + c;
     if (qd % lpr == 0 && j == 0) {
         f.mean[rowi] = mean;
@@ -266,22 +275,29 @@
         }
         *(float4*)(orow + 4 * k) = make_float4(o[0] + rv[k].x, o[1] + rv[k].y, o[2] + rv[k].z, o[3] + rv[k].w);
     }
-}
-
-static __device__ void conv_epilogue_in_bwd(const ConvArgs& a, const ConvGroup& g, const f32x16& acc, float* tile, int tid, int wave_m, int h,
-                                            int m_tile0, int b0, int t0_tile, int bl_lane, int t_lane, bool col_valid) {
+    }
+}
+
+template <int WN>
+static __device__ void conv_epilogue_in_bwd(const ConvArgs& a, const ConvGroup& g, const f32x16 (&acc)[WN], float* tile, int tid, int wave_m, int h,
+                                            int m_tile0, int b0, int t0_tile, const int (&colb)[WN], const int (&colt)[WN], const bool (&colv)[WN]) {
+    constexpr int LDT = AVC_IN_LDT_OF(WN), QPR = 4 * WN;
     const ConvINBwd& f = a.inb;
     const int Tout = a.Tout, lpr = Tout >> 4;
-    if (col_valid) {
-        const int col = bl_lane * Tout + (t_lane - t0_tile);
+#pragma unroll
+    for (int wn = 0; wn < WN; ++wn) {
+        if (!colv[wn]) continue;
+        const int col = (colb[wn] - b0) * Tout + (colt[wn] - t0_tile);
 #pragma unroll
         for (int r = 0; r < 16; ++r) {
             const int row = wave_m * 32 + (r & 3) + 8 * (r >> 2) + 4 * h;
-            tile[row * AVC_IN_LDT + col] = acc[r];
+            tile[row * LDT + col] = acc[wn][r];
         }
     }
     __syncthreads();
-    const int r = tid >> 2, qd = tid & 3;
+#pragma unroll
+    for (int pass = 0; pass < WN; ++pass) {
+    const int r = pass * (64 / WN) + tid / QPR, qd = tid % QPR;
     const int m = m_tile0 + r;
     const int bl = (16 * qd) / Tout, t0 = 16 * qd - bl * Tout;
     const int b = b0 + bl;
@@ -290,7 +306,7 @@
     float gv[16];
 #pragma unroll
     for (int k = 0; k < 4; ++k) {
-        const float4 x = *(const float4*)(tile + r * AVC_IN_LDT + 16 * qd + 4 * k);
+        const float4 x = *(const float4*)(tile + r * LDT + 16 * qd + 4 * k);
         gv[4 * k] = x.x; gv[4 * k + 1] = x.y; gv[4 * k + 2] = x.z; gv[4 * k + 3] = x.w;
     }
     const long rowi = (long)bc * f.C + mc;
@@ -352,7 +368,7 @@
         s1 += __shfl_xor(s1, o);
         s2 += __shfl_xor(s2, o);
     }
-    if (!valid) return;
+    if (!valid) continue;
     if (f.dcond && qd % lpr == 0) {
         float* dc = f.dcond + (long)b * f.dcond_sb + f.dcond_off;
         dc[m] = s1;
@@ -369,6 +385,7 @@
         o.z = rstd * (gv[4 * k + 2] * gamma - m1 - xh[4 * k + 2] * m2);
         o.w = rstd * (gv[4 * k + 3] * gamma - m1 - xh[4 * k + 3] * m2);
         *(float4*)(drow + 4 * k) = o;
+    }
     }
 }
 
@@ -394,19 +411,26 @@
         for (int k = 0; k < 4; ++k) lo[k] = hi[k] = 0.f;
     }
 }
-static __device__ void conv_epilogue_in_pairs(const ConvArgs& a, const ConvGroup& g, const f32x16& acc, float* tile, int tid, int wave_m, int wave_n,
+template <int WN>
+static __device__ void conv_epilogue_in_pairs(const ConvArgs& a, const ConvGroup& g, const f32x16 (&acc)[WN], float* tile, int tid, int wave_m, int wave_n,
                                               int li, int h, int m_tile0, int b0) {
+    constexpr int LDT = AVC_IN_LDT_OF(WN), QPR = 4 * WN;
     const ConvINFuse& f = a.in;
-    const int col = wave_n * 32 + li;
-#pragma unroll
-    for (int r = 0; r < 16; ++r) {
-        const int row = wave_m * 32 + (r & 3) + 8 * (r >> 2) + 4 * h;
-        const int m = m_tile0 + row;
-        const float bs = g.bias ? g.bias[m < a.M ? m : a.M - 1] : 0.f;
-        tile[row * AVC_IN_LDT + col] = acc[r] + bs;
+#pragma unroll
+    for (int wn = 0; wn < WN; ++wn) {
+        const int col = wave_n * (32 * WN) + wn * 32 + li;
+#pragma unroll
+        for (int r = 0; r < 16; ++r) {
+            const int row = wave_m * 32 + (r & 3) + 8 * (r >> 2) + 4 * h;
+            const int m = m_tile0 + row;
+            const float bs = g.bias ? g.bias[m < a.M ? m : a.M - 1] : 0.f;
+            tile[row * LDT + col] = acc[wn][r] + bs;
+        }
     }
     __syncthreads();
-    const int r = tid >> 2, qd = tid & 3;
+#pragma unroll
+    for (int pass = 0; pass < WN; ++pass) {
+    const int r = pass * (64 / WN) + tid / QPR, qd = tid % QPR;
     const int m = m_tile0 + r, odd = m & 1;
     const int Tout = a.Tout, lpr = Tout >> 4;
     const int bl = (16 * qd) / Tout, t0 = 16 * qd - bl * Tout;
@@ -415,7 +439,7 @@
     float v[16];
 #pragma unroll
     for (int k = 0; k < 4; ++k) {
-        const float4 x = *(const float4*)(tile + r * AVC_IN_LDT + 16 * qd + 4 * k);
+        const float4 x = *(const float4*)(tile + r * LDT + 16 * qd + 4 * k);
         v[4 * k] = bh_lo(bh_pack(x.x, 0.f)); v[4 * k + 1] = bh_lo(bh_pack(x.y, 0.f));
         v[4 * k + 2] = bh_lo(bh_pack(x.z, 0.f)); v[4 * k + 3] = bh_lo(bh_pack(x.w, 0.f));
     }
@@ -447,14 +471,14 @@
     float lo[8], hi[8];
 #pragma unroll
     for (int i = 0; i < 8; ++i) {
-        const float rcv = __shfl_xor(odd ? v[i] : v[8 + i], 4);
+        const float rcv = __shfl_xor(odd ? v[i] : v[8 + i], QPR);
         lo[i] = odd ? rcv : v[i];
         hi[i] = odd ? v[8 + i] : rcv;
     }
-    const float pmean = __shfl_xor(mean, 4), prstd = __shfl_xor(rstd, 4), pgamma = __shfl_xor(gamma, 4), pbeta = __shfl_xor(beta, 4);
+    const float pmean = __shfl_xor(mean, QPR), prstd = __shfl_xor(rstd, QPR), pgamma = __shfl_xor(gamma, QPR), pbeta = __shfl_xor(beta, QPR);
     const float mean0 = odd ? pmean : mean, mean1 = odd ? mean : pmean, rstd0 = odd ? prstd : rstd, rstd1 = odd ? rstd : prstd;
     const float g0 = odd ? pgamma : gamma, g1 = odd ? gamma : pgamma, be0 = odd ? pbeta : beta, be1 = odd ? beta : pbeta;
-    if (!valid) return;
+    if (!valid) continue;
     const int fb = t0 + 8 * odd;
     const long prow = (long)b * (f.C >> 1) + (m >> 1);
     unsigned* yrow = (unsigned*)g.out + prow * Tout + fb;
@@ -476,22 +500,29 @@
         *(conv_u32x4*)(yrow + 4 * k) = yv;
         *(conv_u32x4*)(orow + 4 * k) = ov;
     }
-}
-
-static __device__ void conv_epilogue_in_bwd_pairs(const ConvArgs& a, const ConvGroup& g, const f32x16& acc, float* tile, int tid, int wave_m, int h,
-                                                  int m_tile0, int b0, int t0_tile, int bl_lane, int t_lane, bool col_valid) {
+    }
+}
+
+template <int WN>
+static __device__ void conv_epilogue_in_bwd_pairs(const ConvArgs& a, const ConvGroup& g, const f32x16 (&acc)[WN], float* tile, int tid, int wave_m, int h,
+                                                  int m_tile0, int b0, int t0_tile, const int (&colb)[WN], const int (&colt)[WN], const bool (&colv)[WN]) {
+    constexpr int LDT = AVC_IN_LDT_OF(WN), QPR = 4 * WN;
     const ConvINBwd& f = a.inb;
     const int Tout = a.Tout, lpr = Tout >> 4;
-    if (col_valid) {
-        const int col = bl_lane * Tout + (t_lane - t0_tile);
+#pragma unroll
+    for (int wn = 0; wn < WN; ++wn) {
+        if (!colv[wn]) continue;
+        const int col = (colb[wn] - b0) * Tout + (colt[wn] - t0_tile);
 #pragma unroll
         for (int r = 0; r < 16; ++r) {
             const int row = wave_m * 32 + (r & 3) + 8 * (r >> 2) + 4 * h;
-            tile[row * AVC_IN_LDT + col] = acc[r];
+            tile[row * LDT + col] = acc[wn][r];
         }
     }
     __syncthreads();
-    const int r = tid >> 2, qd = tid & 3;
+#pragma unroll
+    for (int pass = 0; pass < WN; ++pass) {
+    const int r = pass * (64 / WN) + tid / QPR, qd = tid % QPR;
     const int m = m_tile0 + r, odd = m & 1;
     const int bl = (16 * qd) / Tout, t0 = 16 * qd - bl * Tout;
     const int b = b0 + bl;
@@ -500,7 +531,7 @@
     float gv[16];
 #pragma unroll
     for (int k = 0; k < 4; ++k) {
-        const float4 x = *(const float4*)(tile + r * AVC_IN_LDT + 16 * qd + 4 * k);
+        const float4 x = *(const float4*)(tile + r * LDT + 16 * qd + 4 * k);
         gv[4 * k] = x.x; gv[4 * k + 1] = x.y; gv[4 * k + 2] = x.z; gv[4 * k + 3] = x.w;
     }
     const int C2 = f.C >> 1;
@@ -556,7 +587,7 @@
         float lo[8], hi[8];
 #pragma unroll
         for (int i = 0; i < 8; ++i) {
-            const float rcv = __shfl_xor(odd ? v[i] : v[8 + i], 4);
+            const float rcv = __shfl_xor(odd ? v[i] : v[8 + i], QPR);
             lo[i] = odd ? rcv : v[i];
             hi[i] = odd ? v[8 + i] : rcv;
         }
@@ -597,6 +628,7 @@
 #pragma unroll
     for (int i = 0; i < 16; ++i) dv[i] = rstd * (gv[i] * gamma - m1 - xh[i] * m2);
     store_pairs((unsigned*)f.dy, dv);
+    }
 }
 
 static __device__ __forceinline__ void conv_res_index_pair(const ConvEpi& a, int t, int& i0, int& i1) {
diff --git a/adaptive_voice_conversion_amd/csrc/engine.hip b/adaptive_voice_conversion_amd/csrc/engine.hip
--- a/adaptive_voice_conversion_amd/csrc/engine.hip
+++ b/adaptive_voice_conversion_amd/csrc/engine.hip
@@ -1041,18 +1041,24 @@
     return avc_launch_in_fwd(a, s);
 }
 
-static int conv_in_fwd(const avc_plan* p, ConvArgs& a, float slope, int Bn, int C, int T, const float* cond, long cond_sb, int cond_off,
+static avc_tuning in_fuse_tun(const avc_plan* p, long family) {
+    avc_tuning t = p->tun;
+    t.conv_in_fuse = t.conv_in_fuse ? (1 | (t.conv_in_fuse & family)) : 0;
+    return t;
+}
+static int conv_in_fwd(const avc_plan* p, long family, ConvArgs& a, float slope, int Bn, int C, int T, const float* cond, long cond_sb, int cond_off,
                        const float* res, int res_mode, int Tres, float* out, float* stats, hipStream_t s, int Bfull = 0, int b0 = 0,
                        bool pairs = false, int planar = 0, int nv = 0) {
     if (Bfull == 0) Bfull = Bn;
-    if (!planar && avc_conv_in_fusable(a, p->tun, res ? res_mode : AVC_RES_NONE, Tres)) {
+    const avc_tuning tun = in_fuse_tun(p, family);
+    if (!planar && avc_conv_in_fusable(a, tun, res ? res_mode : AVC_RES_NONE, Tres)) {
         a.in.out = out;
         a.in.mean = stats + (long)b0 * C;
         a.in.rstd = stats + (long)Bfull * C + (long)b0 * C;
         a.in.cond = cond; a.in.cond_sb = cond_sb; a.in.cond_off = cond_off;
         a.in.res = res; a.in.res_mode = res ? res_mode : 0; a.in.Tres = Tres;
         a.in.C = C; a.in.relu = 1;
-        return avc_launch_conv(a, s, 0, p->tun);
+        return avc_launch_conv(a, s, 0, tun);
     }
     int rc = avc_launch_conv(a, s, 0, p->tun);
     if (rc) return rc;
@@ -1138,7 +1144,7 @@
         const long C = bh ? Cc / 2 : Cc, CCr = bh ? e.CC / 2 : e.CC;
         RUN(enc_front(p, e, params, ws, x, sxb, sxc, sxt, s));
         ConvArgs a = mk_fwd(p, SL, p->layers[e.in_conv], params, ws, ws + e.cat, CCr * e.T[0], e.T[0], 1, B, e.T[0], ws + e.h0, (long)C * e.T[0], e.T[0], 1, 0);
-        RUN(conv_in_fwd(p, a, SL, B, Cc, e.T[0], nullptr, 0, 0, nullptr, 0, 0, ws + e.out[0], ws + e.st0, s, 0, 0, bh, 0, NV));
+        RUN(conv_in_fwd(p, AVC_IN_FUSE_T128_ENC_FWD, a, SL, B, Cc, e.T[0], nullptr, 0, 0, nullptr, 0, 0, ws + e.out[0], ws + e.st0, s, 0, 0, bh, 0, NV));
         return 0;
     };
     const hipStream_t mainS = s;
@@ -1203,10 +1209,10 @@
         for (int l = 0; l < e.n; ++l) {
             const int Ti = e.T[l], To = e.T[l + 1];
             ConvArgs a = mk_fwd(p, SL, p->layers[e.c1[l]], params, ws, ws + e.out[l], (long)C * Ti, Ti, 1, B, Ti, ws + e.y1[l], (long)C * Ti, Ti, 1, 0);
-            RUN(conv_in_fwd(p, a, SL, B, Cc, Ti, nullptr, 0, 0, nullptr, 0, 0, ws + e.a1[l], ws + e.st1[l], s, 0, 0, bh, 0, NV));
+            RUN(conv_in_fwd(p, AVC_IN_FUSE_T128_ENC_FWD, a, SL, B, Cc, Ti, nullptr, 0, 0, nullptr, 0, 0, ws + e.a1[l], ws + e.st1[l], s, 0, 0, bh, 0, NV));
             ConvArgs b = mk_fwd(p, SL, p->layers[e.c2[l]], params, ws, ws + e.a1[l], (long)C * Ti, Ti, 1, B, Ti, ws + e.y2[l], (long)C * To, To, 1, 0);
             const int rmode = e.c.subsample[l] > 1 ? AVC_RES_AVGPOOL2 : AVC_RES_IDENTITY;
-            RUN(conv_in_fwd(p, b, SL, B, Cc, To, nullptr, 0, 0, ws + e.out[l], rmode, Ti, ws + e.out[l + 1], ws + e.st2[l], s, 0, 0, bh, 0, NV));
+            RUN(conv_in_fwd(p, AVC_IN_FUSE_T128_ENC_FWD, b, SL, B, Cc, To, nullptr, 0, 0, ws + e.out[l], rmode, Ti, ws + e.out[l + 1], ws + e.st2[l], s, 0, 0, bh, 0, NV));
         }
         const int Tb = p->Tb;
         ConvArgs h = mk_fwd(p, SL, p->layers[e.heads], params, ws, ws + e.out[e.n], (long)C * Tb, Tb, 1, B, Tb, ws + p->muls, (long)2 * e.c.c_out * Tb, Tb, 1, 0);
@@ -1244,7 +1250,7 @@
             const float* cond = ws + d.cond + (long)b0 * csb;
             if (ph == 0) {
                 ConvArgs a = mk_fwd(p, SL, p->layers[d.in_conv], params, ws, zs + (long)b0 * zsb, zsb, zsc, zst, Bn, Tb, ws + d.y0 + ob0, (long)C * Tb, Tb, 1, 0);
-                RUN(conv_in_fwd(p, a, SL, Bn, Cc, Tb, nullptr, 0, 0, nullptr, 0, 0, ws + d.out[0] + ob0, ws + d.st0, s, B, b0, bh, 0, NV));
+                RUN(conv_in_fwd(p, AVC_IN_FUSE_T128_DEC_FWD, a, SL, Bn, Cc, Tb, nullptr, 0, 0, nullptr, 0, 0, ws + d.out[0] + ob0, ws + d.st0, s, B, b0, bh, 0, NV));
                 return 0;
             }
             if (ph == 2 * d.n + 1) {
@@ -1260,7 +1266,7 @@
             const long oi = (long)b0 * C * Ti, oo = (long)b0 * C * To;
             if ((ph - 1) % 2 == 0) {
                 ConvArgs a = mk_fwd(p, SL, p->layers[d.c1[l]], params, ws, ws + d.out[l] + oi, (long)C * Ti, Ti, 1, Bn, Ti, ws + d.y1[l] + oi, (long)C * Ti, Ti, 1, 0);
-                RUN(conv_in_fwd(p, a, SL, Bn, Cc, Ti, cond, csb, (2 * l) * 2 * Cc, nullptr, 0, 0, ws + d.a1[l] + oi, ws + d.st1[l], s, B, b0, bh, 0, NV));
+                RUN(conv_in_fwd(p, AVC_IN_FUSE_T128_DEC_FWD, a, SL, Bn, Cc, Ti, cond, csb, (2 * l) * 2 * Cc, nullptr, 0, 0, ws + d.a1[l] + oi, ws + d.st1[l], s, B, b0, bh, 0, NV));
                 return 0;
             }
             ConvArgs b = mk_fwd(p, SL, p->layers[d.c2[l]], params, ws, ws + d.a1[l] + oi, (long)C * Ti, Ti, 1, Bn, Ti, ws + d.y2[l] + oo, (long)C * To, To, 1, 0);
@@ -1269,7 +1275,7 @@
                 b.ops = 1;
                 b.ob = (long)C * To; b.oc = Ti;
             }
-            RUN(conv_in_fwd(p, b, SL, Bn, Cc, To, cond, csb, (2 * l + 1) * 2 * Cc, ws + d.out[l] + oi, up > 1 ? AVC_RES_UP2 : AVC_RES_IDENTITY, Ti,
+            RUN(conv_in_fwd(p, AVC_IN_FUSE_T128_DEC_FWD, b, SL, Bn, Cc, To, cond, csb, (2 * l + 1) * 2 * Cc, ws + d.out[l] + oi, up > 1 ? AVC_RES_UP2 : AVC_RES_IDENTITY, Ti,
                             ws + d.out[l + 1] + oo, ws + d.st2[l], s, B, b0, bh, (bh && up > 1) ? 1 : 0, NV));
             return 0;
         };
@@ -1442,7 +1448,8 @@
             };
             auto dgrad_inb = [&](ConvArgs& a, bool keep_g, long off, long yoff, long stoff, int T, int coff, bool cond, float* dy, bool planar = false) -> int {
                 st.fused = false;
-                if (!planar && a.Tout == T && avc_conv_inb_fusable(a, p->tun)) {
+                const avc_tuning tun = in_fuse_tun(p, AVC_IN_FUSE_T128_DEC_BWD);
+                if (!planar && a.Tout == T && avc_conv_inb_fusable(a, tun)) {
                     a.inb.dy = dy + off; a.inb.y = ws + yoff + off;
                     a.inb.mean = ws + stoff + (long)b0 * Cc; a.inb.rstd = ws + stoff + (long)B * Cc + (long)b0 * Cc;
                     a.inb.cond = cond ? ws + d.cond + (long)b0 * csb : nullptr; a.inb.cond_sb = csb; a.inb.cond_off = coff;
@@ -1451,7 +1458,7 @@
                     if (!keep_g) a.g[0].out = nullptr;
                     st.fused = true;
                 }
-                return avc_launch_conv(a, s, 0, p->tun);
+                return avc_launch_conv(a, s, 0, tun);
             };
             const bool was_fused = st.fused;
             if (ph == 0) {
@@ -1570,9 +1577,10 @@
         const float* dmuls = ws + (bh ? p->dmulsp : p->dmuls);
         const LayerP& Lh = p->layers[e.heads];
         RUN(wgrad_layer(c, Lh, ws + e.out[e.n], (long)C * Tb, Tb, 1, dmuls, (long)Co2 * Tb, Tb, 1, 1, B, Tb, Tb));
+        const avc_tuning enc_bwd_tun = in_fuse_tun(p, AVC_IN_FUSE_T128_ENC_BWD);
         auto dgrad_inb = [&](ConvArgs& a, bool keep_g, const float* y, const float* st, int T, float* dy) -> bool {
             bool fused = false;
-            if (a.Tout == T && avc_conv_inb_fusable(a, p->tun)) {
+            if (a.Tout == T && avc_conv_inb_fusable(a, enc_bwd_tun)) {
                 a.inb.dy = dy; a.inb.y = y; a.inb.mean = st; a.inb.rstd = st + (long)B * Cc;
                 a.inb.C = Cc; a.inb.relu = 1;
                 if (!keep_g) a.g[0].out = nullptr;
@@ -1585,7 +1593,7 @@
         {
             ConvArgs a = mk_dgrad(SL, Lh, ws, dmuls, (long)Co2 * Tb, Tb, 1, 1, B, Tb, Tb, gA, (long)C * Tb, Tb, 1);
             fused = dgrad_inb(a, true, ws + e.y2[e.n - 1], ws + e.st2[e.n - 1], e.T[e.n], dyA);
-            if (!dry) RUN(avc_launch_conv(a, s, 0, p->tun));
+            if (!dry) RUN(avc_launch_conv(a, s, 0, enc_bwd_tun));
         }
         for (int l = e.n - 1; l >= 0; --l) {
             const int Ti = e.T[l], T2 = e.T[l + 1], sub = e.c.subsample[l];
@@ -1596,7 +1604,7 @@
             {
                 ConvArgs a = mk_dgrad(SL, L2, ws, dyA, (long)C * T2, T2, 1, 1, B, T2, Ti, gB, (long)C * Ti, Ti, 1);
                 fused = dgrad_inb(a, false, ws + e.y1[l], ws + e.st1[l], Ti, dyB);
-                if (!dry) RUN(avc_launch_conv(a, s, 0, p->tun));
+                if (!dry) RUN(avc_launch_conv(a, s, 0, enc_bwd_tun));
             }
             RUN(wgrad_layer(c, L2, ws + e.a1[l], (long)C * Ti, Ti, 1, dyA, (long)C * T2, T2, 1, 1, B, Ti, T2));
             if (!dry && !fused) RUN(in_bwd(SL, gB, ws + e.y1[l], ws + e.st1[l], B, Cc, Ti, nullptr, 0, 0, dyB, nullptr, s, bh, NV));
@@ -1605,7 +1613,7 @@
                 ConvArgs a = mk_dgrad(SL, L1, ws, dyB, (long)C * Ti, Ti, 1, 1, B, Ti, Ti, gC, (long)C * Ti, Ti, 1);
                 set_res(a, gA, sub > 1 ? AVC_RES_POOLT : AVC_RES_IDENTITY, (long)C * T2, T2, 1, T2);
                 fused = dgrad_inb(a, true, l > 0 ? ws + e.y2[l - 1] : ws + e.h0, l > 0 ? ws + e.st2[l - 1] : ws + e.st0, Ti, dyA);
-                if (!dry) RUN(avc_launch_conv(a, s, 0, p->tun));
+                if (!dry) RUN(avc_launch_conv(a, s, 0, enc_bwd_tun));
             }
             RUN(wgrad_layer(c, L1, ws + e.out[l], (long)C * Ti, Ti, 1, dyB, (long)C * Ti, Ti, 1, 1, B, Ti, Ti));
             rot();
diff --git a/adaptive_voice_conversion_amd/csrc/ops_api.hip b/adaptive_voice_conversion_amd/csrc/ops_api.hip
--- a/adaptive_voice_conversion_amd/csrc/ops_api.hip
+++ b/adaptive_voice_conversion_amd/csrc/ops_api.hip
@@ -31,7 +31,7 @@
     t.dec_wgrad_wgs = 128;
     t.conv_walk = 0;
     t.conv_walk_min = 2;
-    t.conv_in_fuse = 1;
+    t.conv_in_fuse = 1 | AVC_IN_FUSE_T128_ENC_BWD;
     return t;
 }
 const avc_tuning& avc_default_tuning() {
@@ -39,7 +39,7 @@
     return t;
 }
 avc_tuning& avc_op_tuning() {
-    static thread_local avc_tuning t = make_default_tuning();
+    static thread_local avc_tuning t = [] { avc_tuning d = make_default_tuning(); d.conv_in_fuse = 1; return d; }();
     return t;
 }
 
@@ -273,6 +273,27 @@
     return avc_instnorm_bwd(g_out, y, mean, rstd, B, Cin, Tin, cond, cond_sb, cond_off, relu, dy_out, dcond, dcond_sb, dcond_off, stream);
 }
 
+struct OpInFuseScope {
+    long saved;
+    explicit OpInFuseScope(long v) : saved(avc_op_tuning().conv_in_fuse) { avc_op_tuning().conv_in_fuse = v; }
+    ~OpInFuseScope() { avc_op_tuning().conv_in_fuse = saved; }
+};
+int avc_conv1d_in_fwd_mode(const float* x, long sxb, long sxc, int sxt, int B, int Cin, int Tin, const float* wp, const float* bias, int Cout, int KS,
+                           int stride, int ops, float* y, const float* cond, long cond_sb, int cond_off, int relu, const float* res, int res_mode,
+                           int Tres, float* out, float* mean, float* rstd, int* fused, long in_fuse, void* stream) {
+    OpInFuseScope scope(in_fuse);
+    return avc_conv1d_in_fwd(x, sxb, sxc, sxt, B, Cin, Tin, wp, bias, Cout, KS, stride, ops, y, cond, cond_sb, cond_off, relu, res, res_mode, Tres, out,
+                             mean, rstd, fused, stream);
+}
+int avc_conv1d_dgrad_in_bwd_mode(const float* dy, long syb, long syc, int syt, int yps, int B, int Cout, int Tdy, const float* wpd, int Cin, int KS,
+                                 int stride, int Tin, float* g_out, const float* res, int res_mode, int Tres, const float* y, const float* mean,
+                                 const float* rstd, const float* cond, long cond_sb, int cond_off, int relu, float* dy_out, float* dcond,
+                                 long dcond_sb, int dcond_off, int* fused, long in_fuse, void* stream) {
+    OpInFuseScope scope(in_fuse);
+    return avc_conv1d_dgrad_in_bwd(dy, syb, syc, syt, yps, B, Cout, Tdy, wpd, Cin, KS, stride, Tin, g_out, res, res_mode, Tres, y, mean, rstd, cond,
+                                   cond_sb, cond_off, relu, dy_out, dcond, dcond_sb, dcond_off, fused, stream);
+}
+
 long avc_conv1d_wgrad_ws_floats(int B, int Cin, int Cout, int Tout, int KS) {
     long need = 0;
     for (int stride = 1; stride <= 2; ++stride) {
diff --git a/include/avc_hip.h b/include/avc_hip.h
--- a/include/avc_hip.h
+++ b/include/avc_hip.h
@@ -95,6 +95,11 @@
     long conv_in_fuse;
     long dbg_streams;
 } avc_tuning;
+#define AVC_IN_FUSE_T128_ENC_FWD 2
+#define AVC_IN_FUSE_T128_ENC_BWD 4
+#define AVC_IN_FUSE_T128_DEC_FWD 8
+#define AVC_IN_FUSE_T128_DEC_BWD 16
+#define AVC_IN_FUSE_T128_ALL 30
 void avc_tuning_init(avc_tuning* t);
 #define AVC_PLAN_X3 4
 #define AVC_PLAN_RAGGED 8
@@ -215,6 +220,13 @@
                             int stride, int Tin, float* g_out, const float* res, int res_mode, int Tres, const float* y, const float* mean,
                             const float* rstd, const float* cond, long cond_sb, int cond_off, int relu, float* dy_out, float* dcond,
                             long dcond_sb, int dcond_off, int* fused, void* stream);
+int avc_conv1d_in_fwd_mode(const float* x, long sxb, long sxc, int sxt, int B, int Cin, int Tin, const float* wp, const float* bias, int Cout, int KS,
+                           int stride, int ops, float* y, const float* cond, long cond_sb, int cond_off, int relu, const float* res, int res_mode,
+                           int Tres, float* out, float* mean, float* rstd, int* fused, long in_fuse, void* stream);
+int avc_conv1d_dgrad_in_bwd_mode(const float* dy, long syb, long syc, int syt, int yps, int B, int Cout, int Tdy, const float* wpd, int Cin, int KS,
+                                 int stride, int Tin, float* g_out, const float* res, int res_mode, int Tres, const float* y, const float* mean,
+                                 const float* rstd, const float* cond, long cond_sb, int cond_off, int relu, float* dy_out, float* dcond,
+                                 long dcond_sb, int dcond_off, int* fused, long in_fuse, void* stream);
 
 #ifdef __cplusplus
 }
```
